# wubinzzu/NeuRec

Hardware: AMD Instinct MI355X
Metric: BPR triplets/sec (LightGCN-gowalla) (higher is better)
Workload: dtype f32; 1 GPU; LightGCN on synthetic gowalla-shaped interactions (U=29858, I=40981, E=813886), 3 layers, dim 64, B=1024 per GPU, adj=pre, Adam lr=0.01 reg=1e-3; global_batch=1024, parallelism=single GPU

## Files before the change

include/neurec_hip.h:

```cpp
#ifndef NEUREC_HIP_H
#define NEUREC_HIP_H

#include <stddef.h>
#include <stdint.h>

#ifdef __cplusplus
extern "C" {
#endif

#define NRHIP_OK 0
#define NRHIP_ERR_ARG 1
#define NRHIP_ERR_UNSUPPORTED 2
#define NRHIP_ERR_HIP 3
#define NRHIP_ERR_WORKSPACE 4

#define NRHIP_ABI_VERSION 4
#define NRHIP_MAX_TOPK 128

int nrhip_abi_version(void);
const char* nrhip_last_error(void);
int nrhip_device_info(int* cu_count, int* clock_khz, size_t* hbm_bytes, char* name, int name_len);


int nrhip_eval_workspace_bytes(int rows, int top_k, size_t* bytes);
// ... 143 lines not shown
                           const int32_t* d_users, const int32_t* d_pos, const int32_t* d_neg, int batch,
                           float reg, float* d_G, float* d_work, float* d_loss2, const uint64_t* d_plan,
                           void* stream);
int nrhip_adam_dense_tf(float* d_var, float* d_m, float* d_v, float* d_grad, int64_t n,
                        float alpha, float beta1, float beta2, float eps, int clear_grad,
                        void* stream);

int nrhip_adam_dense_tf2(float* d_var, float* d_m, float* d_v, const float* d_grad_a,
                         const float* d_grad_b, int64_t n, float alpha, float beta1, float beta2,
                         float eps, void* stream);
int nrhip_adam_dense_tf_multi(int n_tensors, float* const* d_vars_host, float* const* d_ms_host,
                              float* const* d_vs_host, float* const* d_grads_host,
                              const int64_t* sizes_host, const int32_t* clear_grad_host, float alpha,
                              float beta1, float beta2, float eps, void* stream);
int nrhip_rows_div(const int32_t* d_rows, int n_listed, int d, const float* d_src, float denom,
                   float* d_dst, void* stream);
int nrhip_rows_clear(const int32_t* d_rows, int n_listed, int d, float* d_b0, float* d_b1,
                     float* d_b2, float* d_b3, uint8_t* d_flag, void* stream);

int nrhip_spmm_plan_bytes(int64_t n_rows, int64_t nnz, size_t* bytes);
int nrhip_spmm_plan_create(const int64_t* h_indptr, int64_t n_rows, int item_rows, int item_nnz,
                           int64_t split_row, void* d_plan_buf, size_t plan_bytes, void* stream,
                           void** plan_out);
int nrhip_spmm_plan_destroy(void* plan);
int nrhip_spmm_plan_info(const void* plan, int64_t* n_work_items, int64_t* n_split_rows);
int nrhip_spmm_workspace_bytes(const void* plan, int d, size_t* bytes);
int nrhip_spmm_csr(const void* plan, const int64_t* d_indptr, const int32_t* d_indices,
                   const float* d_vals, const float* d_X, int d, float* d_Y,
                   const float* d_addend, const float* d_sum_in, float* d_sum_out, void* d_ws,
                   size_t ws_bytes, void* stream);

int nrhip_spmm_csr_masked(const void* plan, const int64_t* d_indptr, const int32_t* d_indices,
                          const float* d_vals, const float* d_X, const uint8_t* d_x_row_nonzero,
                          const uint8_t* d_y_row_wanted, int d, float* d_Y, const float* d_addend,
                          const float* d_sum_in, float* d_sum_out, void* d_ws, size_t ws_bytes,
                          void* stream);
int nrhip_spmm_blocked_plan_bytes(int64_t n_rows, int64_t nnz, int d, size_t* bytes);
int nrhip_spmm_blocked_plan_create(const int64_t* h_indptr, const int32_t* h_indices,
                                   int64_t n_rows, int64_t split_row, int d, int64_t block_bytes,
                                   int n_workgroups, int waves_per_wg, int seg_len, int r_max,
                                   int p_max, void* d_plan_buf, size_t plan_bytes, void* stream,
                                   void** plan_out);
int nrhip_spmm_blocked_plan_destroy(void* plan);
int nrhip_spmm_blocked_plan_info(const void* plan, int* n_workgroups, int* n_phases,
                                 int64_t* n_entries, int64_t* n_split);
int nrhip_spmm_blocked_tune(int gathers_in_flight);
int nrhip_spmm_blocked_pack(void* plan, const int32_t* d_indices, const float* d_vals, void* stream);
int nrhip_spmm_blocked(const void* plan, const int32_t* d_indices, const float* d_vals,
                       const float* d_X, float* d_Y, const float* d_addend, const float* d_sum_in,
                       float* d_sum_out, const uint8_t* d_x_row_nonzero,
                       const uint8_t* d_y_row_wanted, void* stream);
int nrhip_spmm_plan_attach_blocked(void* plan, const void* blocked_plan, int d);

int nrhip_spmm_csr_adam(const void* plan, const int32_t* d_indices, const float* d_vals,
                        const float* d_X, int d, float* d_addend, float* d_grad_b, float* d_var,
                        float* d_m, float* d_v, float alpha, float beta1, float beta2, float eps,
                        int clear_consumed, uint8_t* d_row_flag, void* stream);
int nrhip_spmm_blocked_adam(const void* plan, const int32_t* d_indices, const float* d_vals,
                            const float* d_X, float* d_addend, float* d_grad_b, float* d_var,
                            float* d_m, float* d_v, float alpha, float beta1, float beta2,
                            float eps, int clear_consumed, uint8_t* d_row_flag, void* stream);
int nrhip_spmm_plan_has_blocked(const void* plan, int d);

int nrhip_spmm_csr_wanted_layers(const void* plan, const int32_t* d_indices, const float* d_vals,
                                 const float* d_X, int d, const float* d_sum_in,
                                 const float* d_layer_a, const float* d_layer_b, float* d_sum_out,
                                 const uint8_t* d_y_row_wanted, void* stream);
int nrhip_spmm_blocked_wanted_layers(const void* plan, const int32_t* d_indices, const float* d_vals,
                                     const float* d_X, const float* d_sum_in, const float* d_layer_a,
                                     const float* d_layer_b, float* d_sum_out,
                                     const uint8_t* d_y_row_wanted, void* stream);
int nrhip_spmm_csr_wanted_batch(const void* plan, const int32_t* d_indices, const float* d_vals,
                                const float* d_X, int d, const float* d_sum_in, const float* d_layer_a,
                                const float* d_layer_b, float* d_sum_out, const int32_t* d_users,
                                const int32_t* d_pos, const int32_t* d_neg, int batch, int n_users,
                                uint8_t* d_row_flag, int32_t* d_rows_out, void* stream);
int nrhip_spmm_blocked_wanted_batch(const void* plan, const int32_t* d_indices, const float* d_vals,
                                    const float* d_X, const float* d_sum_in, const float* d_layer_a,
                                    const float* d_layer_b, float* d_sum_out, const int32_t* d_users,
                                    const int32_t* d_pos, const int32_t* d_neg, int batch, int n_users,
                                    uint8_t* d_row_flag, int32_t* d_rows_out, void* stream);
int nrhip_spmm_plan_has_wanted(const void* plan, int d);
int nrhip_spmm_blocked_has_wanted(const void* blocked_plan);

int nrhip_spmm_csr_carry(const void* plan, const int64_t* d_indptr, const int32_t* d_indices, const float* d_vals,
                         const float* d_X, const float* d_X2, int x_split, int d, float* d_Yv, int has_carry,
                         const uint8_t* d_row_mask, void* stream);
int nrhip_spmm_chunks_finish(const int32_t* d_first_vrow, int64_t n_rows, const float* d_Yv, int d, float* d_Y,
                             const float* d_addend, const float* d_sum_in, float* d_sum_out,
                             const uint8_t* d_row_mask, void* stream);

int nrhip_partials_sum_rows(const float* d_parts, int world, int64_t n_rows, int d, float* d_Y, const float* d_addend,
                            const float* d_sum_in, float* d_sum_out, const uint8_t* d_row_mask, void* stream);

int nrhip_spmm_csr_rows(const int64_t* d_indptr, const int32_t* d_indices, const float* d_vals,
                        const float* d_X, int d, const int32_t* d_rows, int n_listed, float* d_Y,
                        const float* d_addend, const float* d_sum_in, float* d_sum_out,
                        void* stream);

int nrhip_lightgcn_bpr_grad(const float* d_Esum, const float* d_E0, int n_users, int d,
                            int n_layers, const int32_t* d_users, const int32_t* d_pos,
                            const int32_t* d_neg, int batch, float reg, float* d_Gstar,
                            float* d_Greg, float* d_work, float* d_loss2, const uint64_t* d_plan,
                            void* stream);

int nrhip_lightgcn_bpr_grad_h(const float* d_Esum, const float* d_E0, int n_users, int d,
                              int n_layers, const int32_t* d_users, const int32_t* d_pos,
                              const int32_t* d_neg, int batch, float reg, float* d_H,
                              float* d_Greg, float* d_work, float* d_loss2, const uint64_t* d_plan,
                              void* stream);

int nrhip_lightgcn_mark_batch(const int32_t* d_users, const int32_t* d_pos, const int32_t* d_neg,
                              int batch, int n_users, int32_t* d_rows_out, uint8_t* d_row_flag,
                              void* stream);

typedef struct nrhip_lightgcn_buffers {
  const void* plan;
  const void* plan_t;
  const int64_t* indptr;  const int32_t* indices;  const float* vals;
  const int64_t* indptr_t; const int32_t* indices_t; const float* vals_t;
  float* E0; float* m; float* v;
  float* Ea; float* Eb; float* Esum; float* Esum_rows;
  float* Gstar; float* Greg; float* H; float* Ga; float* Gb;
  int32_t* batch_rows;
  uint8_t* row_flag;
  float* terms;
  void* spmm_ws; size_t spmm_ws_bytes;
  int n_users; int n_nodes; int d; int n_layers; int max_batch;
  float reg;
} nrhip_lightgcn_buffers;
int nrhip_lightgcn_ctx_create(const nrhip_lightgcn_buffers* bufs, void** ctx_out);
int nrhip_lightgcn_ctx_destroy(void* ctx);
int nrhip_lightgcn_step(void* ctx, const int32_t* d_users, const int32_t* d_pos,
                        const int32_t* d_neg, int batch, const uint64_t* d_plan, float alpha,
                        float beta1, float beta2, float eps, float* d_loss2, void* stream);

int nrhip_lightgcn_step_colshard_fwd(void* ctx, const int32_t* d_users, const int32_t* d_pos, const int32_t* d_neg,
                                     int batch, float* d_partials, void* stream);
int nrhip_lightgcn_step_colshard_bwd(void* ctx, const int32_t* d_users, const int32_t* d_pos, const int32_t* d_neg,
                                     int batch, const uint64_t* d_plan, const float* d_given, float alpha,
                                     float beta1, float beta2, float eps, float* d_loss2, void* stream);
int nrhip_lightgcn_partial_dots(const float* d_Esum, const float* d_E0, int n_users, int d, int n_layers,
                                const int32_t* d_users, const int32_t* d_pos, const int32_t* d_neg, int batch,
                                float* d_out, void* stream);
int nrhip_partials_sum(const float* d_parts, int world, int n, float* d_given, void* stream);
int nrhip_lightgcn_bpr_grad_given(const float* d_Esum, const float* d_E0, int n_users, int d, int n_layers,
                                  const int32_t* d_users, const int32_t* d_pos, const int32_t* d_neg, int batch,
                                  float reg, float* d_Gstar, float* d_Greg, float* d_work, float* d_loss2,
                                  const uint64_t* d_plan, const float* d_given, int divided, void* stream);
int nrhip_lightgcn_step_grad(void* ctx, const int32_t* d_users, const int32_t* d_pos,
                             const int32_t* d_neg, int batch, const uint64_t* d_plan,
                             float* d_loss2, float* d_grad_out, void* stream);
int nrhip_lightgcn_step_apply(void* ctx, float* d_grad, float alpha, float beta1, float beta2,
                              float eps, void* stream);

typedef struct nrhip_mf_buffers {
  float* P; float* Q; float* mP; float* vP; float* mQ; float* vQ; float* GP; float* GQ;
  float* terms;
  int n_users; int n_items; int d; int max_batch;
  float reg;
  int32_t* last; int32_t* stamp; const float* alpha_tab; int alpha_len; int lazy_period;
  int32_t* tw; int32_t* inb;
} nrhip_mf_buffers;
int nrhip_mf_ctx_create(const nrhip_mf_buffers* bufs, void** ctx_out);
int nrhip_mf_ctx_destroy(void* ctx);
int nrhip_mf_step(void* ctx, const int32_t* d_users, const int32_t* d_pos, const int32_t* d_neg,
                  int batch, const uint64_t* d_plan, const uint64_t* d_next_plan, int next_batch,
                  int step_index, float alpha, float beta1, float beta2, float eps, float* d_loss2,
                  void* stream);
int nrhip_mf_steps(void* ctx, const int32_t* d_users, const int32_t* d_pos, const int32_t* d_neg,
                   int64_t n_total, int batch, const uint64_t* d_plans, int first_step_index,
                   const float* h_alpha, float beta1, float beta2, float eps, float* d_loss2,
                   float* d_terms_steps, void* stream);
int nrhip_loss_reduce_steps(const float* d_terms, int n_steps, int batch, int n_last, float reg, float* d_loss2,
                            void* stream);
int nrhip_mf_flush(void* ctx, int steps_done, float beta1, float beta2, float eps, void* stream);

int nrhip_ngcf_workspace_bytes(int64_t n_rows, size_t* bytes);
int nrhip_ngcf_layer_fwd(const float* d_ego, const float* d_S, const float* d_Wg,
                         const float* d_bg, const float* d_Wb, const float* d_bb, int64_t n_rows,
                         int d, float keep, uint8_t* d_mask, int mask_given, uint64_t seed,
                         uint64_t step, int layer, float* d_ego_out, float* d_out, int64_t ldo,
                         void* stream);
int nrhip_ngcf_layer_bwd(const float* d_ego, const float* d_S, const float* d_Wg,
                         const float* d_bg, const float* d_Wb, const float* d_bb, int64_t n_rows,
                         int d, float keep, const uint8_t* d_mask, const float* d_dout, int64_t ldo,
                         const float* d_dego_next, float* d_dS, float* d_dego_direct, float* d_dT1,
                         float* d_dT2, float* d_dWg, float* d_dbg, float* d_dWb, float* d_dbb,
                         void* d_ws, size_t ws_bytes, void* stream);

int nrhip_vae_encode(const int64_t* d_indptr, const int32_t* d_indices, const int32_t* d_rows,
                     int batch, int h, int z, const float* d_Wq0, const float* d_bq0,
                     const float* d_Wq1, const float* d_bq1, const float* d_Wp0,
                     const float* d_bp0, int act, float keep, const float* d_drop_given,
                     const float* d_eps_given, float is_training, uint64_t seed, uint64_t step,
                     float* d_h0val, float* d_H1, float* d_MU, float* d_LOGVAR, float* d_EPSSTD,
                     float* d_ZS, float* d_G1, float* d_KLb, void* stream);
int nrhip_add_row_bias(float* d_S, int64_t ld, int batch, int cols, const float* d_bias,
                       void* stream);
int nrhip_vae_workspace_bytes(int batch, int cols, size_t* bytes);
int nrhip_vae_decoder_loss_grad(float* d_S, int64_t ld, int batch, int cols, int h,
                                const float* d_bp1, const int64_t* d_indptr,
                                const int32_t* d_indices, const int32_t* d_rows,
                                const float* d_G1, const float* d_Wp1, float* d_nll,
                                float* d_dWp1, float* d_dbp1, float* d_dG1, void* d_ws,
                                size_t ws_bytes, void* stream);
int nrhip_vae_decoder_fused_workspace_bytes(int batch, int cols, size_t* bytes);
int nrhip_vae_decoder_fused(int batch, int cols, int h, const float* d_G1, const float* d_Wp1,
                            const float* d_bp1, const int64_t* d_indptr, const int32_t* d_indices,
                            const int32_t* d_rows, float* d_nll, float* d_dWp1, float* d_dbp1,
                            float* d_dG1, void* d_ws, size_t ws_bytes, float* d_dbg_logits, void* stream);
int nrhip_vae_mid_backward(int batch, int h, int z, int act, float anneal, const float* d_dG1,
                           const float* d_G1, const float* d_H1, const float* d_MU,
                           const float* d_LOGVAR, const float* d_EPSSTD, const float* d_ZS,
                           const float* d_Wp0, const float* d_Wq1, float* d_DA3, float* d_DH2,
                           float* d_DA1, float* d_dWp0, float* d_dbp0, float* d_dWq1,
                           float* d_dbq1, float* d_dbq0, void* stream);
int nrhip_vae_dwq0(const int64_t* d_indptr, const int32_t* d_indices, const int32_t* d_rows,
                   int batch, int h, const float* d_h0val, const float* d_DA1, float* d_dWq0,
                   void* stream);
int nrhip_axpy(float a, const float* d_x, float* d_y, int64_t n, void* stream);
// ... 200 lines not shown
```

neurec_amd/_lib.py:

```python
import ctypes as C
import os

from . import build as _build

_HERE = os.path.dirname(os.path.abspath(__file__))
LIB_PATH = os.path.join(_HERE, "libneurec_hip.so")

ERR_ARG, ERR_UNSUPPORTED, ERR_HIP, ERR_WORKSPACE = 1, 2, 3, 4


class NeuRecHipError(RuntimeError):
    """A HIP runtime failure or workspace error reported by the native library."""


def _load():
    if not os.path.isfile(LIB_PATH):
        raise ImportError(
            "libneurec_hip.so is not built (expected at %s). Run `python -m neurec_amd.build` "
            "(needs hipcc; the engine has no CPU fallback)." % LIB_PATH)
    if os.path.isfile(_build.STAMP) and not _build.is_current() and not os.environ.get("NEUREC_ALLOW_STALE_LIB"):
        raise ImportError(
            "libneurec_hip.so was built from other sources than neurec_amd/csrc now holds (digest in %s differs). "
            "Run `python -m neurec_amd.build`; NEUREC_ALLOW_STALE_LIB=1 loads it anyway." % _build.STAMP)
    try:
# ... 90 lines not shown
                ("M", C.c_void_p), ("mld", C.c_int64), ("eps", C.c_void_p), ("out", C.c_void_p), ("flags", C.c_void_p),
                ("sums", C.c_void_p), ("colsum_ws", C.c_void_p), ("colsum_ws_bytes", C.c_size_t)]


class EvalRedoArgs(C.Structure):
    _fields_ = [("ev", C.POINTER(EvalPrunedArgs)), ("n_flagged", C.c_int), ("reload_items", C.c_int),
                ("scores", C.c_void_p), ("lds", C.c_int64), ("slab_rows", C.c_int), ("rows", C.c_void_p),
                ("row_users", C.c_void_p), ("count", C.c_void_p), ("fixed", C.c_void_p), ("ws", C.c_void_p),
                ("ws_bytes", C.c_size_t)]


SIGNATURES = {
    "nrhip_device_info": [C.POINTER(i32), C.POINTER(i32), psz, C.c_char_p, i32],
    "nrhip_eval_workspace_bytes": [i32, i32, psz],
    "nrhip_mask_train": [p, i64, p, i32, i32, p, p, p],
    "nrhip_eval_scores": [p, i64, i32, i32, p, p, p, C.POINTER(i32), i32, i32, p, p, p, p, sz, p],
    "nrhip_eval_any_k_workspace_bytes": [i32, i32, i32, psz],
    "nrhip_eval_scores_any_k": [p, i64, i32, i32, p, p, p, C.POINTER(i32), i32, i32, p, p, p, sz, p],
    "nrhip_arg_topk": [p, i64, i32, i32, i32, p, p, p, sz, p],
    "nrhip_colsum_workspace_bytes": [i32, i32, psz],
    "nrhip_colsum_f64": [p, i64, i32, i32, p, p, sz, p],
    "nrhip_score_gemm_workspace_bytes": [i32, i32, i32, psz],
    "nrhip_score_gemm_prepare_items": [p, i64, i32, i32, p, sz, p],
    "nrhip_score_tilemax": [p, i64, p, i32, i32, i32, p, p, p, i64, p, sz, p],
    "nrhip_tile_strike_plan": [p, p, i32, i32, p, p, p, p, p, p, p, sz, p],
    "nrhip_score_tilemax_fix": [p, i64, i32, i32, p, p, i32, p, p, p, p, i32, i32, p, i64, p, sz, p],
    "nrhip_score_filter_workspace_bytes": [i32, i32, i32, psz],
    "nrhip_score_filter_kappa": [i32, p],
    "nrhip_score_filter_prepare_items": [p, i64, i32, i32, p, sz, i32, p],
    "nrhip_score_filter_tilemax": [p, i64, p, i32, i32, i32, p, i64, p, p, sz, i32, p],
    "nrhip_score_filter_i8_workspace_bytes": [i32, i32, i32, psz],
    "nrhip_score_filter_i8_prepare_items": [p, i64, i32, i32, p, sz, i32, p],
    "nrhip_score_filter_i8_tilemax": [p, i64, p, i32, i32, i32, p, i64, p, p, sz, i32, p],
    "nrhip_eval_tiles_workspace_bytes": [i32, i32, psz],
    "nrhip_eval_tiles": [p, i64, p, i64, p, i32, p, i32, i32, p, p, p, p, p, i32, i32, p, p, p, sz, p],
    "nrhip_eval_tiles_bounded_workspace_bytes": [i32, i32, i32, i32, psz],
    "nrhip_eval_tiles_bounded": [p, i64, p, i32, p, i64, p, i32, p, i32, i32, p, p, p, p, p, i32, i32, p, p, p, sz, p],
    "nrhip_eval_pruned": [C.POINTER(EvalPrunedArgs), p],
    "nrhip_eval_redo": [C.POINTER(EvalRedoArgs), p],
    "nrhip_vae_step": [C.POINTER(VaeStepArgs), p, i32, f32, f32, f32, u64, i32, i32, p],
    "nrhip_score_gemm_items_kmajor": [p, i32, i32, p, p],
    "nrhip_score_gemm": [p, i64, p, i32, i32, i32, p, i64, p, sz, p],
    "nrhip_sample_bpr_epoch": [p, p, p, i64, i32, i32, u64, u64, i32, i64, i64, p, p, p, p],
    "nrhip_sample_instances_epoch": [p, p, p, p, p, p, p, i64, i32, i32, i32, i32, u64, u64, i32, i64, i64, p, p, p, p, p, p],
    "nrhip_randint_choice_batch": [i32, i32, i64, p, p, p, i32, u64, u64, p, p],
    "nrhip_bpr_plan": [p, p, p, i64, i32, i32, p, p],
    "nrhip_bpr_mf_grad": [p, p, i32, i32, p, p, p, i32, f32, p, p, p, p, p, p],
    "nrhip_adam_sparse_tf": [p, p, p, p, i64, f32, f32, f32, f32, p],
    "nrhip_adam_dense_tf": [p, p, p, p, i64, f32, f32, f32, f32, i32, p],
    "nrhip_adam_dense_tf2": [p, p, p, p, p, i64, f32, f32, f32, f32, p],
    "nrhip_adam_dense_tf_multi": [i32, p, p, p, p, p, p, f32, f32, f32, f32, p],
    "nrhip_rows_div": [p, i32, i32, p, f32, p, p],
    "nrhip_rows_clear": [p, i32, i32, p, p, p, p, p, p],
    "nrhip_spmm_plan_bytes": [i64, i64, psz],
    "nrhip_spmm_plan_create": [p, i64, i32, i32, i64, p, sz, p, C.POINTER(p)],
    "nrhip_spmm_plan_destroy": [p],
    "nrhip_spmm_plan_info": [p, C.POINTER(i64), C.POINTER(i64)],
    "nrhip_spmm_workspace_bytes": [p, i32, psz],
    "nrhip_spmm_csr": [p, p, p, p, p, i32, p, p, p, p, p, sz, p],
    "nrhip_spmm_csr_masked": [p, p, p, p, p, p, p, i32, p, p, p, p, p, sz, p],
    "nrhip_spmm_csr_carry": [p, p, p, p, p, p, i32, i32, p, i32, p, p],
    "nrhip_spmm_chunks_finish": [p, i64, p, i32, p, p, p, p, p, p],
    "nrhip_partials_sum_rows": [p, i32, i64, i32, p, p, p, p, p, p],
    "nrhip_spmm_csr_rows": [p, p, p, p, i32, p, i32, p, p, p, p, p],
    "nrhip_lightgcn_mark_batch": [p, p, p, i32, i32, p, p, p],
    "nrhip_lightgcn_bpr_grad": [p, p, i32, i32, i32, p, p, p, i32, f32, p, p, p, p, p, p],
    "nrhip_lightgcn_bpr_grad_h": [p, p, i32, i32, i32, p, p, p, i32, f32, p, p, p, p, p, p],
    "nrhip_lightgcn_ctx_create": [C.POINTER(LightGCNBuffers), C.POINTER(p)],
    "nrhip_lightgcn_ctx_destroy": [p],
    "nrhip_lightgcn_step": [p, p, p, p, i32, p, f32, f32, f32, f32, p, p],
    "nrhip_lightgcn_step_grad": [p, p, p, p, i32, p, p, p, p],
    "nrhip_lightgcn_step_apply": [p, p, f32, f32, f32, f32, p],
    "nrhip_mf_ctx_create": [C.POINTER(MFBuffers), C.POINTER(p)],
    "nrhip_mf_ctx_destroy": [p],
    "nrhip_mf_step": [p, p, p, p, i32, p, p, i32, i32, f32, f32, f32, f32, p, p],
    "nrhip_mf_flush": [p, i32, f32, f32, f32, p],
    "nrhip_ngcf_ctx_create": [C.POINTER(NGCFBuffers), C.POINTER(p)],
    "nrhip_ngcf_ctx_destroy": [p],
    "nrhip_ngcf_forward": [p, C.c_uint64, C.c_uint64, i32, p],
    "nrhip_ngcf_step": [p, p, p, p, i32, p, C.c_uint64, C.c_uint64, i32, f32, f32, f32, f32, p, p],
    "nrhip_mf_steps": [p, p, p, p, i64, i32, p, i32, p, f32, f32, f32, p, p, p],
    "nrhip_loss_reduce_steps": [p, i32, i32, i32, f32, p, p],
    "nrhip_lightgcn_step_colshard_fwd": [p, p, p, p, i32, p, p],
    "nrhip_lightgcn_step_colshard_bwd": [p, p, p, p, i32, p, p, f32, f32, f32, f32, p, p],
    "nrhip_lightgcn_partial_dots": [p, p, i32, i32, i32, p, p, p, i32, p, p],
    "nrhip_partials_sum": [p, i32, i32, p, p],
    "nrhip_lightgcn_bpr_grad_given": [p, p, i32, i32, i32, p, p, p, i32, f32, p, p, p, p, p, p, i32, p],
    "nrhip_gemm_workspace_bytes": [i32, i32, i32, p],
    "nrhip_gemm_kmajor": [p, i64, p, i64, i32, i32, i32, p, i64, i32, p, i32, i32, p, sz, p],
    "nrhip_gemm_f32": [p, i64, i32, p, i64, i32, i32, i32, i32, p, i64, i32, p, i32, i32, p, sz, p],
    "nrhip_transpose2d": [p, i64, i32, i32, p, i64, p],
    "nrhip_ngcf_wide_forward": [C.POINTER(NGCFWideBuffers), i32, u64, u64, p],
    "nrhip_ngcf_wide_step": [C.POINTER(NGCFWideBuffers), p, p, p, i32, p, i32, u64, u64, f32, f32, f32, f32, p, p],
    "nrhip_vae_bag_fwd": [p, p, p, i32, i32, p, p, i32, f32, p, u64, u64, p, p, p],
    "nrhip_act_bwd": [p, p, i64, i32, p, p],
    "nrhip_vae_sample": [p, i32, i32, p, f32, u64, u64, p, p, p, p],
    "nrhip_vae_sample_bwd": [p, p, p, i32, i32, f32, p, p],
    "nrhip_vae_softmax_dlogits": [p, i64, i32, i32, p, p, p, p, p],
    "nrhip_vae_dwq0_wide": [p, p, p, i32, i32, p, p, p, p],
    "nrhip_colsum_rows": [p, i64, i32, i32, p, p, sz, p],
    "nrhip_ew_mul": [p, i64, p, i64, i64, i32, p, i64, p],
    "nrhip_ngcf_act_fwd": [p, p, i64, i64, i32, i32, f32, p, i32, u64, u64, i32, p, i64, p, i64, p],
    "nrhip_ngcf_act_bwd": [p, i64, p, i64, p, i64, p, p, i64, p, i64, i32, f32, p, p, p],
    "nrhip_lrelu_drop_fwd": [p, i64, i64, i32, i32, f32, p, i32, u64, u64, i32, i32, p, i64, p, i64, p],
    "nrhip_lrelu_drop_bwd": [p, i64, p, i64, p, i64, p, i64, i32, f32, i32, p, p],
    "nrhip_edge_dropout": [p, i64, f32, p, i32, u64, u64, p, p],
    "nrhip_gather_f32": [p, p, i64, p, p],
    "nrhip_ngcf_mix_bwd": [p, p, i64, p, p, i64, i64, i32, i32, p, p, p],
    "nrhip_route_batch": [p, p, p, i32, i32, i32, i32, i32, p, p, p, p, p, i32, p],
    "nrhip_route_owner_keys": [p, p, i32, p, p, i32, i32, i32, p, p, p],
    "nrhip_sort_u64_segments": [p, p, p, i32, i32, p],
    "nrhip_route_epoch": [p, p, p, i64, i32, i32, i32, i32, i32, i32, p, p, p, p, p, p, p, p],
    "nrhip_route_epoch_owner_keys": [p, p, p, i64, p, p, i32, i32, p, p, p, i32, i32, i64, p, p, p],
    "nrhip_bpr_mf_step_fused": [p, p, p, p, p, p, i32, f32, f32, f32, i32, i32, i32, p, p, p, i32, f32, p, p, p,
                                i32, p, i32, i32, p],
    "nrhip_bpr_mf_fused_flush": [p, p, p, p, p, i32, f32, f32, f32, i32, i64, p],
    "nrhip_adam_sparse_tf_lazy": [p, p, p, p, p, p, i64, i32, p, i32, p, i32, p, i32, i32, f32, f32, f32, p],
    "nrhip_bpr_mf_grad_lazy": [p, p, p, p, p, p, i32, f32, f32, f32, i32, i32, p, p, p, i32, f32, p, p, p,
                               p, p],
    "nrhip_ngcf_workspace_bytes": [i64, psz],
    "nrhip_ngcf_layer_fwd": [p, p, p, p, p, p, i64, i32, f32, p, i32, u64, u64, i32, p, p, i64, p],
    "nrhip_ngcf_layer_bwd": [p, p, p, p, p, p, i64, i32, f32, p, p, i64, p, p, p, p, p, p, p, p, p,
                             p, sz, p],
    "nrhip_spmm_blocked_plan_bytes": [i64, i64, i32, psz],
    "nrhip_spmm_blocked_pack": [p, p, p, p],
    "nrhip_spmm_blocked_plan_create": [p, p, i64, i64, i32, i64, i32, i32, i32, i32, i32, p, sz, p,
                                       C.POINTER(p)],
    "nrhip_spmm_blocked_plan_destroy": [p],
    "nrhip_spmm_blocked_plan_info": [p, p, p, p, p],
    "nrhip_spmm_blocked_tune": [i32],
    "nrhip_spmm_blocked": [p, p, p, p, p, p, p, p, p, p, p],
    "nrhip_spmm_plan_attach_blocked": [p, p, i32],
    "nrhip_spmm_plan_has_blocked": [p, i32],
    "nrhip_spmm_plan_has_wanted": [p, i32],
    "nrhip_spmm_blocked_has_wanted": [p],
    "nrhip_spmm_csr_wanted_layers": [p, p, p, p, i32, p, p, p, p, p, p],
    "nrhip_spmm_blocked_wanted_layers": [p, p, p, p, p, p, p, p, p, p],
    "nrhip_spmm_csr_wanted_batch": [p, p, p, p, i32, p, p, p, p, p, p, p, i32, i32, p, p, p],
    "nrhip_spmm_blocked_wanted_batch": [p, p, p, p, p, p, p, p, p, p, p, i32, i32, p, p, p],
    "nrhip_spmm_csr_adam": [p, p, p, p, i32, p, p, p, p, p, f32, f32, f32, f32, i32, p, p],
    "nrhip_spmm_blocked_adam": [p, p, p, p, p, p, p, p, p, f32, f32, f32, f32, i32, p, p],
    "nrhip_vae_encode": [p, p, p, i32, i32, i32, p, p, p, p, p, p, i32, f32, p, p, f32, u64, u64,
                         p, p, p, p, p, p, p, p, p],
    "nrhip_add_row_bias": [p, i64, i32, i32, p, p],
    "nrhip_vae_workspace_bytes": [i32, i32, psz],
    "nrhip_vae_decoder_loss_grad": [p, i64, i32, i32, i32, p, p, p, p, p, p, p, p, p, p, p, sz, p],
    "nrhip_vae_decoder_fused_workspace_bytes": [i32, i32, psz],
    "nrhip_vae_decoder_fused": [i32, i32, i32, p, p, p, p, p, p, p, p, p, p, p, sz, p, p],
    "nrhip_vae_mid_backward": [i32, i32, i32, i32, f32, p, p, p, p, p, p, p, p, p, p, p, p, p, p,
                               p, p, p, p],
    "nrhip_vae_dwq0": [p, p, p, i32, i32, p, p, p, p],
    "nrhip_axpy": [f32, p, p, i64, p],
    "nrhip_sumsq_accumulate": [p, i64, p, p],
    "nrhip_mean_f32": [p, i32, p, p],
    "nrhip_mean2_f32": [p, p, i32, p, p],
    "nrhip_pairwise_mf_grad": [p, p, i32, i32, p, p, p, i32, f32, i32, p, p, p, p, p, p],
    "nrhip_pointwise_mf_grad": [p, p, i32, i32, p, p, p, i32, f32, i32, p, p, p, p, p, p],
    "nrhip_gather_u8": [p, p, i64, p, p],
    "nrhip_mark_rows": [p, i32, i32, p, p],
    "nrhip_sort_u64": [p, i32, p],
    "nrhip_rows_sum_sorted": [p, i32, p, i32, p, i64, p, p],
    "nrhip_rows_sum_sorted2": [p, i32, p, i32, p, i64, p, p, i64, p, p],
    "nrhip_optimizer_rows_tf": [i32, p, p, p, p, p, i64, i32, f32, f32, f32, f32, p],
    "nrhip_optimizer_dense_tf": [i32, p, p, p, p, i64, f32, f32, f32, f32, i32, p],
    "nrhip_rows_gather": [p, i32, i32, p, p, i64, p],
    "nrhip_rows_gather_ld": [p, i32, i32, p, i64, p, i64, p],
    "nrhip_rows_gather2": [p, i32, i32, p, i64, p, i64, p, i64, p, i64, p],
    "nrhip_rows_scatter_add": [p, i32, i32, p, i64, p, p],
    "nrhip_scale": [p, f32, p, i64, p],
    "nrhip_add": [p, p, p, i64, p],
    "nrhip_div_scalar": [p, f32, p, i64, p],
    "nrhip_add2d": [p, i64, p, i64, p, i64, i64, i32, p],
    "nrhip_copy2d": [p, i64, p, i64, i64, i32, p],
    "nrhip_wrmf_chunk_plan": [p, i32, p, p, C.POINTER(i32)],
    "nrhip_wrmf_workspace_bytes": [i32, i32, psz],
    "nrhip_wrmf_gram": [p, i32, i32, p, p, sz, p],
    "nrhip_wrmf_solve": [p, p, i32, p, i32, p, i32, f32, f32, p, p, i32, p, p, sz, p],
}

for _name, _args in SIGNATURES.items():
    _fn = getattr(lib, _name)
    _fn.argtypes = _args
    _fn.restype = C.c_int
lib.nrhip_abi_version.argtypes = []
lib.nrhip_abi_version.restype = C.c_int
lib.nrhip_last_error.argtypes = []
lib.nrhip_last_error.restype = C.c_char_p

EXPORTED = sorted(list(SIGNATURES) + ["nrhip_abi_version", "nrhip_last_error"])

ABI_VERSION = 4
if lib.nrhip_abi_version() != ABI_VERSION:
    raise ImportError("libneurec_hip.so ABI version %d, expected %d"
                      % (lib.nrhip_abi_version(), ABI_VERSION))


def last_error():
    return lib.nrhip_last_error().decode("utf-8", "replace")


def check(rc):
    if rc == 0:
        return
    msg = last_error()
    if rc == ERR_ARG:
        raise ValueError(msg)
    if rc == ERR_UNSUPPORTED:
        raise NotImplementedError(msg)
    raise NeuRecHipError("libneurec_hip status %d: %s" % (rc, msg))


def call(name, *args):
    check(getattr(lib, name)(*args))


def is_stale():
    return not _build.is_current()
```

neurec_amd/build.py:

```python
import hashlib
import os
import subprocess
import sys
from concurrent.futures import ThreadPoolExecutor

HERE = os.path.dirname(os.path.abspath(__file__))
ROOT = os.path.dirname(HERE)
CSRC = os.path.join(HERE, "csrc")
OBJ_DIR = os.path.join(CSRC, "_obj")
LIB_PATH = os.path.join(HERE, "libneurec_hip.so")
STAMP = os.path.join(OBJ_DIR, "sources.sha256")

SOURCES = ["eval_select.hip", "score_gemm.hip", "sampler.hip", "spmm.hip", "bpr.hip", "adam.hip",
           "step.hip", "dense.hip", "vae.hip", "spmm_blocked.hip", "route.hip", "gemm.hip", "vae_wide.hip", "ngcf_wide.hip", "vae_fused.hip",
           "score_bf16.hip", "score_i8.hip", "eval_pipeline.hip", "wrmf.hip"]
FILE_FLAGS = {"score_i8.hip": ["-mllvm", "-amdgpu-mfma-vgpr-form"]}
EXP_SOURCES = ["experiments/gather_experiments.hip"]
EXP_LIB_PATH = os.path.join(HERE, "libneurec_exp.so")
HEADERS = ["nr_core.h", "nr_common.h", "spmm_blocked_plan.h"]

HIPCC = os.environ.get("HIPCC", "/opt/rocm/bin/hipcc")
FLAGS = ["-O3", "--offload-arch=gfx950", "-std=c++17", "-fPIC", "-ffp-contract=off",
         "-munsafe-fp-atomics", "-Wall", "-Wno-unused-function",
         "-I", CSRC, "-I", os.path.join(ROOT, "include")] + os.environ.get("NEUREC_HIPCC_EXTRA", "").split()


def _existing_sources():
    return [s for s in SOURCES if os.path.isfile(os.path.join(CSRC, s))]


def _digest():
    h = hashlib.sha256()
    for name in _existing_sources() + HEADERS:
        with open(os.path.join(CSRC, name), "rb") as f:
            h.update(name.encode())
            h.update(f.read())
    with open(os.path.join(ROOT, "include", "neurec_hip.h"), "rb") as f:
        h.update(f.read())
    h.update(" ".join(f.replace(ROOT, "<root>") for f in FLAGS).encode())
    h.update(repr(sorted(FILE_FLAGS.items())).encode())
    return h.hexdigest()


def is_current():
    if not (os.path.isfile(LIB_PATH) and os.path.isfile(STAMP)):
        return False
    with open(STAMP) as f:
        return f.read().strip() == _digest()


def build_extension(force=False, verbose=True):
    if not force and is_current():
        return LIB_PATH
    os.makedirs(OBJ_DIR, exist_ok=True)
    srcs = _existing_sources()

    def compile_one(src):
        obj = os.path.join(OBJ_DIR, src.replace(".hip", ".o"))
        cmd = [HIPCC] + FLAGS + FILE_FLAGS.get(src, []) + ["-c", os.path.join(CSRC, src), "-o", obj]
        r = subprocess.run(cmd, capture_output=True, text=True)
        if r.returncode != 0 and FILE_FLAGS.get(src):
            r2 = subprocess.run([HIPCC] + FLAGS + ["-c", os.path.join(CSRC, src), "-o", obj], capture_output=True, text=True)
            if r2.returncode == 0:
                sys.stderr.write("neurec_amd.build: %s compiled WITHOUT %s (not accepted by this hipcc)\n"
                                 % (src, " ".join(FILE_FLAGS[src])))
                r = r2
        return src, obj, r

    objs = []
    with ThreadPoolExecutor(max_workers=min(8, len(srcs))) as ex:
        for src, obj, r in ex.map(compile_one, srcs):
            if r.returncode != 0:
                raise RuntimeError("hipcc failed on %s:\n%s\n%s" % (src, r.stdout, r.stderr))
            if verbose and r.stderr.strip():
                sys.stderr.write(r.stderr)
            objs.append(obj)
    cmd = [HIPCC, "--offload-arch=gfx950", "-shared", "-fPIC", "-o", LIB_PATH] + objs
    r = subprocess.run(cmd, capture_output=True, text=True)
    if r.returncode != 0:
        raise RuntimeError("link failed:\n%s\n%s" % (r.stdout, r.stderr))
    with open(STAMP, "w") as f:
        f.write(_digest())
    if verbose:
        print("built", LIB_PATH)
    return LIB_PATH


def build_experiments(verbose=True):
    os.makedirs(OBJ_DIR, exist_ok=True)
    objs = []
    for src in EXP_SOURCES:
        obj = os.path.join(OBJ_DIR, os.path.basename(src).replace(".hip", ".o"))
        r = subprocess.run([HIPCC] + FLAGS + ["-c", os.path.join(CSRC, src), "-o", obj],
                           capture_output=True, text=True)
        if r.returncode != 0:
            raise RuntimeError("hipcc failed on %s:\n%s\n%s" % (src, r.stdout, r.stderr))
        objs.append(obj)
    r = subprocess.run([HIPCC, "--offload-arch=gfx950", "-shared", "-fPIC", "-o", EXP_LIB_PATH] + objs +
                       ["-L", HERE, "-lneurec_hip", "-Wl,-rpath,$ORIGIN"], capture_output=True, text=True)
    if r.returncode != 0:
        raise RuntimeError("link failed:\n%s\n%s" % (r.stdout, r.stderr))
    if verbose:
# ... 9 lines not shown
```

neurec_amd/colshard.py:

```python
import numpy as np
import torch

from . import engine as E
from .trainer import LightGCNEngine


class ColumnShardedLightGCN:
    def __init__(self, comm, adj_csr, n_users, n_items, embed, n_layers, lr, reg, max_batch, adj_t_csr=None,
                 rank=None, world=None, keep_order=False):
        self.comm = comm
        self.rank = comm.rank if rank is None else int(rank)
        self.world = comm.world if world is None else int(world)
        emb = np.asarray(embed, dtype=np.float32) if not isinstance(embed, torch.Tensor) else embed
        self.d = int(emb.shape[1])
        if self.d % self.world:
            raise ValueError("embed_size %d is not a multiple of the %d ranks" % (self.d, self.world))
        self.d_loc = self.d // self.world
        lo = self.rank * self.d_loc
        self.local = LightGCNEngine(adj_csr, n_users, n_items, emb[:, lo:lo + self.d_loc], n_layers, lr, reg,
                                    max_batch, adj_t_csr=adj_t_csr, keep_order=keep_order)
        dev = self.local.E0.device
        self.max_batch = int(max_batch)
        self._parts = torch.zeros(3 * self.max_batch, dtype=torch.float32, device=dev)
        self._given = torch.zeros(3 * self.max_batch, dtype=torch.float32, device=dev)
        self.exchange_bytes_per_step = None

    @property
    def adam(self):
        return self.local.adam

    def step(self, users, pos, neg, loss_out=None, plan=None):
        B = users.numel()
        if B > self.max_batch:
            raise ValueError("batch larger than max_batch")
        ctx, n = self.local._ctx, 3 * B
        ctx.lightgcn_step_colshard_fwd(users, pos, neg, self._parts)
        if self.comm.live and self.world == self.comm.world:
            allp = torch.empty((self.world, n), dtype=torch.float32, device=self._parts.device)
            self.comm.all_gather_rows(self._parts[:n], allp)
            E.partials_sum(allp, self.world, n, self._given)
            given = self._given
            self.exchange_bytes_per_step = self.world * n * 4
        else:
            given = self._parts
        ctx.lightgcn_step_colshard_bwd(users, pos, neg, self.local.adam, loss_out, plan, given)
        self.local.adam.advance()

    def final_embeddings(self):
        eu, ei = self.local.final_embeddings()
        if not (self.comm.live and self.world == self.comm.world):
            return eu, ei
        loc = torch.cat([eu, ei]).contiguous()
        allc = torch.empty((self.world,) + tuple(loc.shape), dtype=loc.dtype, device=loc.device)
        self.comm.all_gather_rows(loc, allc.view(self.world * loc.shape[0], loc.shape[1]))
        full = allc.permute(1, 0, 2).reshape(loc.shape[0], self.d).contiguous()
        U = self.local.n_users
        return full[:U], full[U:]

    def table(self):
        return self.local.E0[:, :self.d_loc]
```

neurec_amd/csrc/spmm.hip:

```cpp
#include "nr_common.h"
#include <limits.h>
#include <algorithm>
#include <stdlib.h>
#include <new>
#include <vector>

extern "C" int nrhip_spmm_blocked(const void* plan, const int32_t* d_indices, const float* d_vals,
                                  const float* d_X, float* d_Y, const float* d_addend,
                                  const float* d_sum_in, float* d_sum_out,
                                  const uint8_t* d_x_row_nonzero, const uint8_t* d_y_row_wanted,
                                  void* stream);

extern "C" int nrhip_spmm_blocked_wanted_layers(const void* plan, const int32_t* d_indices,
                                                const float* d_vals, const float* d_X,
                                                const float* d_sum_in, const float* d_layer_a,
                                                const float* d_layer_b, float* d_sum_out,
                                                const uint8_t* d_y_row_wanted, void* stream);
extern "C" int nrhip_spmm_blocked_wanted_batch(const void* plan, const int32_t* d_indices,
                                               const float* d_vals, const float* d_X,
                                               const float* d_sum_in, const float* d_layer_a,
                                               const float* d_layer_b, float* d_sum_out,
                                               const int32_t* d_users, const int32_t* d_pos,
                                               const int32_t* d_neg, int batch, int n_users,
                                               uint8_t* d_row_flag, int32_t* d_rows_out, void* stream);
extern "C" int nrhip_spmm_blocked_has_wanted(const void* plan);
extern "C" int nrhip_spmm_blocked_adam(const void* plan, const int32_t* d_indices,
                                       const float* d_vals, const float* d_X, float* d_addend,
                                       float* d_grad_b, float* d_var, float* d_m, float* d_v,
                                       float alpha, float beta1, float beta2, float eps,
                                       int clear_consumed, uint8_t* d_row_flag, void* stream);

namespace {

constexpr int kSegLen = 256;
constexpr int kItemRows = 32;
constexpr int kLegacyWaves = 4;
constexpr int kGather = 16;

struct SpmmPlan {
  int64_t n_rows, nnz;
  const void* blocked[5];
  int64_t n_items, n_hub_items, n_a_items, n_b_items;
  int item_rows, item_nnz;
  int32_t* item_row0;
  int32_t* item_nrows;
  int32_t* item_slot;
  int64_t* item_begin;
  int32_t* item_len;
  int64_t n_seg;
  int32_t* seg_row;
  int64_t* seg_begin;
  int32_t* seg_len;
  int32_t* seg_slot;
  int64_t n_multi_seg, n_multi_row;
  int32_t* multi_row;
  int32_t* multi_first;
  int32_t* multi_nseg;
};

inline int blocked_slot(int d) {
  return d == 16 ? 0 : d == 32 ? 1 : d == 64 ? 2 : d == 128 ? 3 : d == 256 ? 4 : -1;
}

struct PlanSizes {
  size_t max_seg, max_multi, max_item;
};
PlanSizes plan_sizes(int64_t n_rows, int64_t nnz) {
  PlanSizes s;
  s.max_seg = (size_t)(n_rows + nnz / kSegLen + 1);
  s.max_multi = (size_t)(nnz / kSegLen + 1);
  s.max_item = (size_t)(n_rows + nnz / kSegLen + 1);
  return s;
}
size_t plan_bytes_for(int64_t n_rows, int64_t nnz) {
  const PlanSizes s = plan_sizes(n_rows, nnz);
  return nr_align_up(s.max_seg * 4, 256) * 3 + nr_align_up(s.max_seg * 8, 256) +
         nr_align_up(s.max_multi * 4, 256) * 3 + nr_align_up(s.max_item * 4, 256) * 4 +
         nr_align_up(s.max_item * 8, 256);
}

template <int D, int G, bool MASKED>
__device__ __forceinline__ void gather_accumulate(int64_t b, int len, int lane,
                                                  const int32_t* __restrict__ indices,
                                                  const float* __restrict__ vals,
                                                  const float* __restrict__ X,
                                                  const uint8_t* __restrict__ col_mask,
                                                  float (&acc)[D / NR_WAVE]) {
  constexpr int CPL = D / NR_WAVE;
  for (int k0 = 0; k0 < len; k0 += NR_WAVE) {
    const int n = min(NR_WAVE, len - k0);
    int my_idx = 0;
    float my_val = 0.f;
    if (lane < n) {
      my_idx = indices[b + k0 + lane];
      my_val = vals[b + k0 + lane];
    }
    if constexpr (!MASKED) {
      for (int t0 = 0; t0 < n; t0 += G) {
        float a[G];
        float x[G][CPL];
#pragma unroll
        for (int u = 0; u < G; ++u) {
          const int tt = min(t0 + u, n - 1);
          const int col = __builtin_amdgcn_readlane(my_idx, tt);
          a[u] = __builtin_bit_cast(
              float, __builtin_amdgcn_readlane(__builtin_bit_cast(int, my_val), tt));
          const float* xr = X + (int64_t)col * D + lane;
#pragma unroll
// ... 658 lines not shown
  p->item_row0 = carve4(sz.max_item);
  p->item_nrows = carve4(sz.max_item);
  p->item_len = carve4(sz.max_item);
  p->item_slot = carve4(sz.max_item);
  p->item_begin = carve8(sz.max_item);
  hipStream_t st = (hipStream_t)stream;
  hipError_t e = hipSuccess;
  auto up = [&](void* dst, const void* src, size_t n) {
    if (n && e == hipSuccess) e = hipMemcpyAsync(dst, src, n, hipMemcpyHostToDevice, st);
  };
  up(p->seg_row, seg_row.data(), seg_row.size() * 4);
  up(p->seg_begin, seg_begin.data(), seg_begin.size() * 8);
  up(p->seg_len, seg_len.data(), seg_len.size() * 4);
  up(p->seg_slot, seg_slot.data(), seg_slot.size() * 4);
  up(p->multi_row, multi_row.data(), multi_row.size() * 4);
  up(p->multi_first, multi_first.data(), multi_first.size() * 4);
  up(p->multi_nseg, multi_nseg.data(), multi_nseg.size() * 4);
  up(p->item_row0, it_row0.data(), it_row0.size() * 4);
  up(p->item_nrows, it_nrows.data(), it_nrows.size() * 4);
  up(p->item_begin, it_begin.data(), it_begin.size() * 8);
  up(p->item_len, it_len.data(), it_len.size() * 4);
  up(p->item_slot, it_slot.data(), it_slot.size() * 4);
  if (e == hipSuccess) e = hipStreamSynchronize(st);
  if (e != hipSuccess) {
    delete p;
    nrhip_set_error("spmm_plan_create: upload failed: %s", hipGetErrorString(e));
    return NR_ERR_HIP;
  }
  *plan_out = p;
  return NR_OK;
}

int nrhip_spmm_plan_destroy(void* plan) {
  delete (SpmmPlan*)plan;
  return NR_OK;
}

int nrhip_spmm_plan_attach_blocked(void* plan, const void* blocked_plan, int d) {
  NR_REQUIRE(plan && blocked_slot(d) >= 0, NR_ERR_ARG,
             "spmm_plan_attach_blocked: null plan or dim %d not in (16, 32, 64, 128, 256)", d);
  ((SpmmPlan*)plan)->blocked[blocked_slot(d)] = blocked_plan;
  return NR_OK;
}

int nrhip_spmm_csr_adam(const void* plan, const int32_t* d_indices, const float* d_vals,
                        const float* d_X, int d, float* d_addend, float* d_grad_b, float* d_var,
                        float* d_m, float* d_v, float alpha, float beta1, float beta2, float eps,
                        int clear_consumed, uint8_t* d_row_flag, void* stream) {
  NR_REQUIRE(plan, NR_ERR_ARG, "spmm_csr_adam: null plan");
  const SpmmPlan* p = (const SpmmPlan*)plan;
  NR_REQUIRE(d == 64 && p->blocked[blocked_slot(64)], NR_ERR_UNSUPPORTED,
             "spmm_csr_adam: needs the d = 64 lane-group schedule");
  return nrhip_spmm_blocked_adam(p->blocked[blocked_slot(64)], d_indices, d_vals, d_X, d_addend, d_grad_b, d_var,
                                 d_m, d_v, alpha, beta1, beta2, eps, clear_consumed, d_row_flag,
                                 stream);
}

int nrhip_spmm_csr_wanted_layers(const void* plan, const int32_t* d_indices, const float* d_vals,
                                 const float* d_X, int d, const float* d_sum_in,
                                 const float* d_layer_a, const float* d_layer_b, float* d_sum_out,
                                 const uint8_t* d_y_row_wanted, void* stream) {
  NR_REQUIRE(plan, NR_ERR_ARG, "spmm_csr_wanted_layers: null plan");
  const SpmmPlan* p = (const SpmmPlan*)plan;
  NR_REQUIRE(d == 64 && p->blocked[blocked_slot(64)], NR_ERR_UNSUPPORTED,
             "spmm_csr_wanted_layers: needs the d = 64 lane-group schedule");
  return nrhip_spmm_blocked_wanted_layers(p->blocked[blocked_slot(64)], d_indices, d_vals, d_X, d_sum_in,
                                          d_layer_a, d_layer_b, d_sum_out, d_y_row_wanted, stream);
}

int nrhip_spmm_csr_wanted_batch(const void* plan, const int32_t* d_indices, const float* d_vals,
                                const float* d_X, int d, const float* d_sum_in, const float* d_layer_a,
                                const float* d_layer_b, float* d_sum_out, const int32_t* d_users,
                                const int32_t* d_pos, const int32_t* d_neg, int batch, int n_users,
                                uint8_t* d_row_flag, int32_t* d_rows_out, void* stream) {
  NR_REQUIRE(plan, NR_ERR_ARG, "spmm_csr_wanted_batch: null plan");
  const SpmmPlan* p = (const SpmmPlan*)plan;
  NR_REQUIRE(d == 64 && p->blocked[blocked_slot(64)], NR_ERR_UNSUPPORTED,
             "spmm_csr_wanted_batch: needs the d = 64 lane-group schedule");
  return nrhip_spmm_blocked_wanted_batch(p->blocked[blocked_slot(64)], d_indices, d_vals, d_X, d_sum_in,
                                         d_layer_a, d_layer_b, d_sum_out, d_users, d_pos, d_neg, batch,
                                         n_users, d_row_flag, d_rows_out, stream);
}

int nrhip_spmm_plan_has_wanted(const void* plan, int d) {
  if (!plan || d != 64) return 0;
  const SpmmPlan* p = (const SpmmPlan*)plan;
  return p->blocked[blocked_slot(64)] ? nrhip_spmm_blocked_has_wanted(p->blocked[blocked_slot(64)]) : 0;
}

int nrhip_spmm_plan_has_blocked(const void* plan, int d) {
  if (!plan) return 0;
  const SpmmPlan* p = (const SpmmPlan*)plan;
  const int slot = blocked_slot(d);
  return slot >= 0 && p->blocked[slot] != nullptr;
}

int nrhip_spmm_plan_info(const void* plan, int64_t* n_work_items, int64_t* n_split_rows) {
  NR_REQUIRE(plan, NR_ERR_ARG, "spmm_plan_info: null plan");
  const SpmmPlan* p = (const SpmmPlan*)plan;
  if (n_work_items) *n_work_items = p->n_items;
  if (n_split_rows) *n_split_rows = p->n_multi_row;
  return NR_OK;
}

int nrhip_spmm_workspace_bytes(const void* plan, int d, size_t* bytes) {
  NR_REQUIRE(plan && bytes && d >= 1, NR_ERR_ARG, "spmm_workspace_bytes: bad arguments");
  const SpmmPlan* p = (const SpmmPlan*)plan;
  *bytes = nr_align_up((size_t)(p->n_multi_seg + 1) * (size_t)d * sizeof(float), 256);
  return NR_OK;
}

static int spmm_dispatch(const char* who, const void* plan, const int64_t* d_indptr,
                         const int32_t* d_indices, const float* d_vals, const float* d_X, int d,
                         float* d_Y, const float* d_addend, const float* d_sum_in,
                         float* d_sum_out, const uint8_t* d_col_mask, const uint8_t* d_row_mask,
                         void* d_ws, size_t ws_bytes, void* stream) {
  NR_REQUIRE(plan && d_indptr && d_indices && d_vals && d_X && (d_Y || d_sum_out), NR_ERR_ARG,
             "%s: null pointer argument", who);
  NR_REQUIRE((d_sum_out == nullptr) || (d_sum_in != nullptr), NR_ERR_ARG,
             "%s: sum_out needs sum_in", who);
  const SpmmPlan* p = (const SpmmPlan*)plan;
  hipStream_t st = (hipStream_t)stream;
  const int bslot = blocked_slot(d);
  if (bslot >= 0 && p->blocked[bslot])
    return nrhip_spmm_blocked(p->blocked[bslot], d_indices, d_vals, d_X, d_Y, d_addend, d_sum_in,
                              d_sum_out, d_col_mask, d_row_mask, stream);
  if (d < 64)
    NR_REQUIRE(d_row_mask == nullptr, NR_ERR_UNSUPPORTED,
               "%s: row mask needs an embedding dim >= 64", who);
  if (p->n_multi_seg > 0)
    NR_REQUIRE(d_ws && ws_bytes >= (size_t)p->n_multi_seg * d * sizeof(float), NR_ERR_WORKSPACE,
               "%s: workspace too small for %lld split-row partials", who,
               (long long)p->n_multi_seg);
  float* part = (float*)d_ws;
  switch (d) {
    case 16: return launch_segs<16>(p, d_indices, d_vals, d_X, d_Y, d_addend, d_sum_in, d_sum_out, part, st);
    case 32: return launch_segs<32>(p, d_indices, d_vals, d_X, d_Y, d_addend, d_sum_in, d_sum_out, part, st);
    case 64: return launch_items<64, 4>(p, d_indptr, d_indices, d_vals, d_X, d_Y, d_addend, d_sum_in, d_sum_out, part, d_col_mask, d_row_mask, st);
    case 128: return launch_items<128, 2>(p, d_indptr, d_indices, d_vals, d_X, d_Y, d_addend, d_sum_in, d_sum_out, part, d_col_mask, d_row_mask, st);
    case 256: return launch_items<256, 1>(p, d_indptr, d_indices, d_vals, d_X, d_Y, d_addend, d_sum_in, d_sum_out, part, d_col_mask, d_row_mask, st);
    default:
      NR_REQUIRE(false, NR_ERR_UNSUPPORTED,
                 "%s: embedding dim %d not built (16, 32, 64, 128, 256)", who, d);
  }
  return NR_OK;
}

int nrhip_spmm_csr(const void* plan, const int64_t* d_indptr, const int32_t* d_indices,
                   const float* d_vals, const float* d_X, int d, float* d_Y,
                   const float* d_addend, const float* d_sum_in, float* d_sum_out, void* d_ws,
                   size_t ws_bytes, void* stream) {
  return spmm_dispatch("spmm_csr", plan, d_indptr, d_indices, d_vals, d_X, d, d_Y, d_addend,
                       d_sum_in, d_sum_out, nullptr, nullptr, d_ws, ws_bytes, stream);
}

int nrhip_spmm_csr_masked(const void* plan, const int64_t* d_indptr, const int32_t* d_indices,
                          const float* d_vals, const float* d_X, const uint8_t* d_x_row_nonzero,
                          const uint8_t* d_y_row_wanted, int d, float* d_Y, const float* d_addend,
                          const float* d_sum_in, float* d_sum_out, void* d_ws, size_t ws_bytes,
                          void* stream) {
  NR_REQUIRE(d_x_row_nonzero || d_y_row_wanted, NR_ERR_ARG, "spmm_csr_masked: no mask given");
  NR_REQUIRE(!(d_y_row_wanted && d_sum_out && d_sum_out == d_sum_in) || true, NR_ERR_ARG, "");
  return spmm_dispatch("spmm_csr_masked", plan, d_indptr, d_indices, d_vals, d_X, d, d_Y,
                       d_addend, d_sum_in, d_sum_out, d_x_row_nonzero, d_y_row_wanted, d_ws,
                       ws_bytes, stream);
}
// ... 80 lines not shown
```

neurec_amd/csrc/spmm_blocked.hip:

```cpp
#include "nr_common.h"
#include "spmm_blocked_plan.h"
#include <algorithm>
#include <new>
#include <cstdlib>
#include <initializer_list>
#include <vector>

namespace {

using nr_plan::kMaxLdsBytes;
using nr_plan::blocked_plan_bytes;
static_assert((int)nr_plan::kOk == NR_OK && (int)nr_plan::kErrArg == NR_ERR_ARG &&
              (int)nr_plan::kErrUnsupported == NR_ERR_UNSUPPORTED, "the planner returns the C ABI's status codes");

struct BlockedPlan : nr_plan::PlanArrays<int4> {
  int64_t n_rows, nnz, n_ent, n_cmb;
  int n_wg, n_phases;
  int seg, r_max, p_max, waves, d;
  const int32_t* pk_from_idx;
  const float* pk_from_val;
  int nnz_cap, ent_cap;
  int colmask_ok;
  int wanted_ok, w_ent_cap, w_nnz_cap, w_bitmap_words;
  int ww_ok, ww_ent_cap;
  int ww_lds_slots;
};


struct AdamEpilogue {
  float4* var; float4* m; float4* v; const float4* grad_b;
  float alpha, omb1, omb2, eps;
  float4* addend_rw; float4* grad_b_rw; uint8_t* flag_rw;
};


template <bool MASKED, bool ADAM, int LPR>
__device__ __forceinline__ void blocked_epilogue(const float4* s_acc, int r0, int nr, int tid, int nthreads,
                                                 float4* __restrict__ Y, const float4* __restrict__ addend,
                                                 const float4* sum_in, float4* sum_out,
                                                 const uint8_t* __restrict__ row_mask, const AdamEpilogue& ad,
                                                 const int32_t* s_rows = nullptr) {
  for (int i = tid; i < nr * LPR; i += nthreads) {
    const int row = s_rows ? s_rows[i / LPR] : r0 + i / LPR;
    if constexpr (MASKED) {
      if (row_mask && row_mask[row] == 0) continue;
    }
    const int64_t o = (int64_t)row * LPR + (i & (LPR - 1));
    float4 y = s_acc[i];
    bool flagged = true;
    if constexpr (ADAM) {
      if (ad.flag_rw) flagged = ad.flag_rw[row] != 0;
    }
    float4 hv = make_float4(0.f, 0.f, 0.f, 0.f);
    if (addend) {
      if (flagged) hv = addend[o];
      y.x = __fadd_rn(y.x, hv.x); y.y = __fadd_rn(y.y, hv.y);
      y.z = __fadd_rn(y.z, hv.z); y.w = __fadd_rn(y.w, hv.w);
    }
    if constexpr (ADAM) {
      float4 gb = make_float4(0.f, 0.f, 0.f, 0.f);
      if (flagged) gb = ad.grad_b[o];
      if (ad.addend_rw) {
        const float4 zero = make_float4(0.f, 0.f, 0.f, 0.f);
        if (hv.x != 0.f || hv.y != 0.f || hv.z != 0.f || hv.w != 0.f) ad.addend_rw[o] = zero;
        if (gb.x != 0.f || gb.y != 0.f || gb.z != 0.f || gb.w != 0.f) ad.grad_b_rw[o] = zero;
        if ((i & (LPR - 1)) == 0 && ad.flag_rw && flagged) ad.flag_rw[row] = 0;
      }
      float4 w = ad.var[o], mm = ad.m[o], vv = ad.v[o];
      nr::adam_dense_tf(__fadd_rn(y.x, gb.x), w.x, mm.x, vv.x, ad.alpha, ad.omb1, ad.omb2, ad.eps);
      nr::adam_dense_tf(__fadd_rn(y.y, gb.y), w.y, mm.y, vv.y, ad.alpha, ad.omb1, ad.omb2, ad.eps);
      nr::adam_dense_tf(__fadd_rn(y.z, gb.z), w.z, mm.z, vv.z, ad.alpha, ad.omb1, ad.omb2, ad.eps);
      nr::adam_dense_tf(__fadd_rn(y.w, gb.w), w.w, mm.w, vv.w, ad.alpha, ad.omb1, ad.omb2, ad.eps);
      ad.var[o] = w; ad.m[o] = mm; ad.v[o] = vv;
      continue;
    }
    if (Y) Y[o] = y;
    if (sum_out) {
      const float4 si = sum_in[o];
      sum_out[o] = make_float4(__fadd_rn(si.x, y.x), __fadd_rn(si.y, y.y), __fadd_rn(si.z, y.z),
                               __fadd_rn(si.w, y.w));
    }
  }
}

#ifdef NR_BLK_TIMELINE
__device__ unsigned long long g_blk_dbg[4096 * 24];
#define NR_BLK_STAMP(i) do { if (threadIdx.x == 0 && blockIdx.x < 4096) g_blk_dbg[blockIdx.x * 24 + (i)] = wall_clock64(); } while (0)
#define NR_BLK_WSTAMP() do { if ((threadIdx.x & 63) == 0 && blockIdx.x < 4096) g_blk_dbg[blockIdx.x * 24 + 8 + (threadIdx.x >> 6)] = wall_clock64(); } while (0)
extern "C" int nrhip_exp_blk_timeline(unsigned long long* h_out) {
  if (hipDeviceSynchronize() != hipSuccess) return NR_ERR_HIP;
  return hipMemcpyFromSymbol(h_out, HIP_SYMBOL(g_blk_dbg), sizeof(unsigned long long) * 4096 * 24) == hipSuccess ? NR_OK : NR_ERR_HIP;
}
#else
#define NR_BLK_STAMP(i) do {} while (0)
#define NR_BLK_WSTAMP() do {} while (0)
#endif

template <bool MASKED, int kWaves, int kG, int D, bool ADAM = false>
__global__ __launch_bounds__(kWaves* NR_WAVE) void spmm_blocked_kernel(
    const int32_t* __restrict__ wg_row0, const int32_t* __restrict__ wg_nrows,
    const int32_t* __restrict__ wg_ent_off, const int32_t* __restrict__ wg_cmb_off,
    const int4* __restrict__ ent, const int4* __restrict__ cmb, int n_phases,
    const int32_t* __restrict__ indices, const float* __restrict__ vals,
    const float4* __restrict__ X, float4* __restrict__ Y, const float4* __restrict__ addend,
    const float4* sum_in, float4* sum_out, const uint8_t* __restrict__ col_mask,
    const uint8_t* __restrict__ row_mask, int kRMax, AdamEpilogue ad, const int32_t* __restrict__ row_of,
    int kPMax) {
  constexpr int LPR = D / 4;
// ... 437 lines not shown
    for (int i = tid; i < 3 * bl.batch; i += 16 * NR_WAVE) {
      const int which = i / bl.batch, b = i - which * bl.batch;
      const int row = which == 0 ? bl.users[b] : bl.n_users + (which == 1 ? bl.pos[b] : bl.neg[b]);
      atomicOr(&s_bits[row >> 5], 1u << (row & 31));
      if (i % (int)gridDim.x == wg) {
        bl.row_flag[row] = 1;
        if (bl.rows_out) bl.rows_out[i] = row;
      }
    }
  }
  __syncthreads();
  auto is_wanted = [&](int row) -> bool {
    return by_batch ? ((s_bits[row >> 5] >> (row & 31)) & 1u) != 0u : row_mask[row] != 0;
  };
  for (int i = tid; i < ne; i += 16 * NR_WAVE) {
    const int4 e = w_ent[e0 + i];
    if (is_wanted(e.w)) {
      const int off = atomicAdd(&s_cursor, e.y);
      if (off + e.y <= nnz_cap) s_now[atomicAdd(&s_n_now, 1)] = make_int4(e.x, e.y | (off << 8), e.z, e.w);
      else s_later[atomicAdd(&s_n_later, 1)] = e;
    }
  }
  __syncthreads();
  while (true) {
    const int n_now = s_n_now, n_later = s_n_later;
    for (int k = wave; k < n_now; k += 16) {
      const int4 e = s_now[k];
      const int len = e.y & 0xFF, off = e.y >> 8;
      if (lane < len)
        s_iv[off + lane] = make_int2(indices[(uint32_t)e.z + lane], __float_as_int(vals[(uint32_t)e.z + lane]));
    }
    __syncthreads();
    for (int k = tid; k < n_now; k += 16 * NR_WAVE) {
      const int4 e = s_now[k];
      s_now[k] = make_int4(e.x, e.y & 0xFF, e.y >> 8, e.w | (1 << 30));
    }
    __syncthreads();
    staged_walk(s_now, s_iv, n_now, 0, X, Y, addend, sum_in, sum_out, s_part, kRMax, wave, g, c, chain);
    if (n_later == 0) break;
    __syncthreads();
    if (tid == 0) { s_n_now = 0; s_n_later = 0; s_cursor = 0; }
    __syncthreads();
    for (int k0 = 0; k0 < n_later; k0 += 16 * NR_WAVE) {
      const int k = k0 + tid;
      int4 e = make_int4(0, 0, 0, 0);
      if (k < n_later) e = s_later[k];
      __syncthreads();
      if (k < n_later) {
        const int off = atomicAdd(&s_cursor, e.y);
        if (off + e.y <= nnz_cap) s_now[atomicAdd(&s_n_now, 1)] = make_int4(e.x, e.y | (off << 8), e.z, e.w);
        else s_later[atomicAdd(&s_n_later, 1)] = e;
      }
      __syncthreads();
    }
  }
  if (c1 > c0) {
    __syncthreads();
    for (int ci = c0 + wave * 4 + g; ci < c1; ci += 64) {
      const int4 cm = w_cmb[ci];
      if (!is_wanted(cm.x)) continue;
      float4 acc = make_float4(0.f, 0.f, 0.f, 0.f);
      for (int sgm = 0; sgm < cm.z; ++sgm) {
        const float4 q = s_part[(size_t)(cm.y - kRMax + sgm) * RS + c];
        acc.x = __fadd_rn(acc.x, q.x); acc.y = __fadd_rn(acc.y, q.y);
        acc.z = __fadd_rn(acc.z, q.z); acc.w = __fadd_rn(acc.w, q.w);
      }
      masked_row_out(acc, (int64_t)cm.x * RS + c, addend, true, Y, sum_in, sum_out, &chain);
    }
  }
}

struct WantedEpi {
  float4* Y; const float4* addend; const float4* sum_in; float4* sum_out; LayerChain chain;
};
#ifdef NR_WW_TIMELINE
__device__ unsigned long long g_ww_dbg[256 * 8];
#define NR_WW_STAMP(i) do { if (threadIdx.x == 0 && blockIdx.x < 256) g_ww_dbg[blockIdx.x * 8 + (i)] = wall_clock64(); } while (0)
#define NR_WW_STAMP_END(i) do { __syncthreads(); NR_WW_STAMP(i); } while (0)
#else
#define NR_WW_STAMP(i)
#define NR_WW_STAMP_END(i)
#endif

__global__ __launch_bounds__(16 * NR_WAVE) void spmm_wanted_wave_kernel(
    const int32_t* __restrict__ ww_off, const int32_t* __restrict__ ww_choff,
    const int4* __restrict__ ww_ent, const int32_t* __restrict__ ww_gch, const int4* __restrict__ ww_hub,
    const int32_t* __restrict__ ww_lcoff, const int4* __restrict__ ww_lcmb,
    float* ww_part, unsigned* ww_cnt, const int32_t* __restrict__ indices,
    const float* __restrict__ vals, const float4* __restrict__ X, WantedEpi ep,
    const uint8_t* __restrict__ row_mask, BatchLists bl, int bitmap_words, int ent_cap, int lds_slots) {
  constexpr int RS = 16;
  extern __shared__ float4 s_mem[];
  float4* s_part = s_mem;
  int4* s_want = (int4*)(s_mem + (size_t)lds_slots * RS);
  uint32_t* s_bits = (uint32_t*)(s_want + ent_cap);
  __shared__ int s_n;
  const int tid = threadIdx.x, lane = tid & 63, wave = tid >> 6;
  const int c = lane & 15, g = lane >> 4;
  const int wg = blockIdx.x;
  const int e0 = ww_off[wg], ne = ww_off[wg + 1] - e0;
  const int h0 = ww_choff[wg], h1 = ww_choff[wg + 1];
  const int l0 = ww_lcoff[wg], l1 = ww_lcoff[wg + 1];
  NR_WW_STAMP(0);
  if (tid == 0) s_n = 0;
  const bool by_batch = bl.users != nullptr;
  if (by_batch) {
    for (int i = tid; i < bitmap_words; i += 16 * NR_WAVE) s_bits[i] = 0u;
    __syncthreads();
    for (int i = tid; i < bl.batch; i += 16 * NR_WAVE) {
      const int u = bl.users[i], p = bl.pos[i], q = bl.neg[i];
      const int ru = u, rp = bl.n_users + p, rq = bl.n_users + q;
      if (u >= 0) atomicOr(&s_bits[ru >> 5], 1u << (ru & 31));
      if (p >= 0) atomicOr(&s_bits[rp >> 5], 1u << (rp & 31));
      if (q >= 0) atomicOr(&s_bits[rq >> 5], 1u << (rq & 31));
    }
    const int total = 3 * bl.batch, per = (total + (int)gridDim.x - 1) / (int)gridDim.x;
    for (int i = wg * per + tid; i < min(total, (wg + 1) * per); i += 16 * NR_WAVE) {
      const int which = i / bl.batch, b = i - which * bl.batch;
      const int row = which == 0 ? bl.users[b] : bl.n_users + (which == 1 ? bl.pos[b] : bl.neg[b]);
      bl.row_flag[row] = 1;
      if (bl.rows_out) bl.rows_out[i] = row;
    }
  }
  __syncthreads();
  auto is_wanted = [&](int row) -> bool {
    return by_batch ? ((s_bits[row >> 5] >> (row & 31)) & 1u) != 0u : row_mask[row] != 0;
  };
  NR_WW_STAMP(1);
  for (int i = tid; i < ne; i += 16 * NR_WAVE) {
    const int4 e = ww_ent[e0 + i];
    if (is_wanted(e.w)) s_want[atomicAdd(&s_n, 1)] = e;
  }
  __syncthreads();
  NR_WW_STAMP(2);
  const int n = s_n;
  const float4 zero = make_float4(0.f, 0.f, 0.f, 0.f);
  int k = wave;
  int4 e = zero_int4();
  int col = 0;
  float val = 0.f;
  if (k < n) {
    e = s_want[k];
    if (lane < e.y) {
      col = indices[(uint32_t)e.z + lane];
      val = vals[(uint32_t)e.z + lane];
    }
  }
  while (k < n) {
    const int len = e.y, slot = e.x, row = e.w;
    float4 x[16];
#pragma unroll
    for (int j = 0; j < 16; ++j) {
      const int cj = __shfl(col, (g << 4) | j, NR_WAVE);
      x[j] = X[(int64_t)cj * RS + c];
    }
    const int64_t o = (int64_t)row * RS + c;
    const int64_t oe = slot == 0 ? o : (int64_t)c;
    float4 pre_si = zero, pre_a = zero, pre_b = zero;
    if (ep.sum_out) {
      pre_si = ep.sum_in[oe];
      if (ep.chain.a) pre_a = ep.chain.a[oe];
      if (ep.chain.b) pre_b = ep.chain.b[oe];
    }
    const int kn = k + 16;
    int4 en = zero_int4();
    int coln = 0;
    float valn = 0.f;
    if (kn < n) {
      en = s_want[kn];
      if (lane < en.y) {
        coln = indices[(uint32_t)en.z + lane];
        valn = vals[(uint32_t)en.z + lane];
      }
    }
#pragma unroll
    for (int j = 0; j < 16; ++j) {
      const float aj = __shfl(val, (g << 4) | j, NR_WAVE);
      x[j] = make_float4(__fmul_rn(aj, x[j].x), __fmul_rn(aj, x[j].y), __fmul_rn(aj, x[j].z), __fmul_rn(aj, x[j].w));
    }
    float4 acc = zero, carry = zero;
#pragma unroll
    for (int gg = 0; gg < 4; ++gg) {
      if (gg * 16 < len) {
        if (g == gg) {
          acc = carry;
#pragma unroll
          for (int j = 0; j < 16; ++j) {
            const float4 t = make_float4(__fadd_rn(acc.x, x[j].x), __fadd_rn(acc.y, x[j].y),
                                         __fadd_rn(acc.z, x[j].z), __fadd_rn(acc.w, x[j].w));
            if (gg * 16 + j < len) acc = t;
          }
        }
        const int src = (gg << 4) | c;
        carry = make_float4(__shfl(acc.x, src, NR_WAVE), __shfl(acc.y, src, NR_WAVE),
                            __shfl(acc.z, src, NR_WAVE), __shfl(acc.w, src, NR_WAVE));
      }
    }
    if (g == 0) {
      if (slot == 0) {
        float4 y = carry;
        if (ep.addend) {
          const float4 pre_add = ep.addend[o];
          y = make_float4(__fadd_rn(y.x, pre_add.x), __fadd_rn(y.y, pre_add.y), __fadd_rn(y.z, pre_add.z),
                          __fadd_rn(y.w, pre_add.w));
        }
        if (ep.Y) ep.Y[o] = y;
        if (ep.sum_out) {
          float4 si = pre_si;
          if (ep.chain.a)
            si = make_float4(__fadd_rn(si.x, pre_a.x), __fadd_rn(si.y, pre_a.y), __fadd_rn(si.z, pre_a.z),
                             __fadd_rn(si.w, pre_a.w));
          if (ep.chain.b)
            si = make_float4(__fadd_rn(si.x, pre_b.x), __fadd_rn(si.y, pre_b.y), __fadd_rn(si.z, pre_b.z),
                             __fadd_rn(si.w, pre_b.w));
          ep.sum_out[o] = make_float4(__fadd_rn(si.x, y.x), __fadd_rn(si.y, y.y), __fadd_rn(si.z, y.z),
                                      __fadd_rn(si.w, y.w));
        }
      } else if (slot < 0) {
        s_part[(size_t)(-slot - 1) * RS + c] = carry;
      } else {
        float* mine = ww_part + (size_t)(slot - 1) * 64 + c * 4;
        __hip_atomic_store(mine + 0, carry.x, __ATOMIC_RELAXED, __HIP_MEMORY_SCOPE_AGENT);
        __hip_atomic_store(mine + 1, carry.y, __ATOMIC_RELAXED, __HIP_MEMORY_SCOPE_AGENT);
        __hip_atomic_store(mine + 2, carry.z, __ATOMIC_RELAXED, __HIP_MEMORY_SCOPE_AGENT);
        __hip_atomic_store(mine + 3, carry.w, __ATOMIC_RELAXED, __HIP_MEMORY_SCOPE_AGENT);
      }
    }
    k = kn;
    e = en;
    col = coln;
    val = valn;
  }
  if (l1 > l0) {
    __syncthreads();
    for (int li = l0 + wave * 4 + g; li < l1; li += 64) {
      const int4 cm = ww_lcmb[li];
      if (!is_wanted(cm.x)) continue;
      float4 acc = zero;
      for (int sgm = 0; sgm < cm.z; ++sgm) {
        const float4 q = s_part[(size_t)(cm.y + sgm) * RS + c];
        acc.x = __fadd_rn(acc.x, q.x); acc.y = __fadd_rn(acc.y, q.y);
        acc.z = __fadd_rn(acc.z, q.z); acc.w = __fadd_rn(acc.w, q.w);
      }
      masked_row_out(acc, (int64_t)cm.x * RS + c, ep.addend, true, ep.Y, ep.sum_in, ep.sum_out, &ep.chain);
    }
  }
  NR_WW_STAMP_END(3);
  if (tid == 0 && blockIdx.x < 256) {
#ifdef NR_WW_TIMELINE
    g_ww_dbg[blockIdx.x * 8 + 6] = (unsigned long long)n;
    g_ww_dbg[blockIdx.x * 8 + 7] = (unsigned long long)(h1 - h0);
#endif
  }
  if (h1 > h0) {
    __builtin_amdgcn_fence(__ATOMIC_RELEASE, "workgroup");
    __builtin_amdgcn_s_waitcnt(0);
    __syncthreads();
    for (int hi = h0 + wave; hi < h1; hi += 16) {
      const int hub = ww_gch[hi];
      const int4 hd = ww_hub[hub];
      if (!is_wanted(hd.x)) continue;
      unsigned old = 0;
      if (lane == 0) old = __hip_atomic_fetch_add(&ww_cnt[hub], 1u, __ATOMIC_RELAXED, __HIP_MEMORY_SCOPE_AGENT);
      old = __builtin_amdgcn_readfirstlane(old);
      if (old != (unsigned)hd.w - 1u) continue;
      float4 sum = zero;
      for (int s0 = 0; s0 < hd.z; s0 += 16) {
        float4 q[16];
#pragma unroll
        for (int j = 0; j < 16; ++j) {
          const float* qp = ww_part + ((size_t)hd.y + min(s0 + j, hd.z - 1)) * 64 + c * 4;
          q[j].x = __hip_atomic_load(qp + 0, __ATOMIC_RELAXED, __HIP_MEMORY_SCOPE_AGENT);
          q[j].y = __hip_atomic_load(qp + 1, __ATOMIC_RELAXED, __HIP_MEMORY_SCOPE_AGENT);
          q[j].z = __hip_atomic_load(qp + 2, __ATOMIC_RELAXED, __HIP_MEMORY_SCOPE_AGENT);
          q[j].w = __hip_atomic_load(qp + 3, __ATOMIC_RELAXED, __HIP_MEMORY_SCOPE_AGENT);
        }
#pragma unroll
        for (int j = 0; j < 16; ++j)
          if (s0 + j < hd.z)
            sum = make_float4(__fadd_rn(sum.x, q[j].x), __fadd_rn(sum.y, q[j].y), __fadd_rn(sum.z, q[j].z),
                              __fadd_rn(sum.w, q[j].w));
      }
      if (g == 0)
        masked_row_out(sum, (int64_t)hd.x * RS + c, ep.addend, true, ep.Y, ep.sum_in, ep.sum_out, &ep.chain);
      if (lane == 0) __hip_atomic_store(&ww_cnt[hub], 0u, __ATOMIC_RELAXED, __HIP_MEMORY_SCOPE_AGENT);
    }
  }
  NR_WW_STAMP_END(4);
}

size_t wanted_lds_bytes(const BlockedPlan* p) {
  return (size_t)p->p_max * 256 + 2 * (size_t)p->w_ent_cap * 16 + (size_t)p->w_bitmap_words * 4 +
         (size_t)p->w_nnz_cap * 8;
}
int ww_bitmap_words(const BlockedPlan* p) { return (int)((p->n_rows + 127) / 128 * 4); }
size_t ww_lds_bytes(const BlockedPlan* p) {
  return (size_t)p->ww_lds_slots * 256 + (size_t)p->ww_ent_cap * 16 + (size_t)ww_bitmap_words(p) * 4 + 16;
}
size_t colmask_lds_bytes(const BlockedPlan* p) {
  return (size_t)p->p_max * 256 + (size_t)p->ent_cap * 16 + (size_t)p->nnz_cap * 8;
}

int launch_wanted_wave(const BlockedPlan* p, const int32_t* d_indices, const float* d_vals, const float* d_X,
                       float* d_Y, const float* d_addend, const float* d_sum_in, float* d_sum_out,
                       const uint8_t* d_y_row_wanted, LayerChain chain, BatchLists bl, hipStream_t st) {
  hipLaunchKernelGGL(spmm_wanted_wave_kernel, dim3((unsigned)p->n_wg), dim3(16 * NR_WAVE), ww_lds_bytes(p), st,
                     p->ww_off, p->ww_choff, p->ww_ent, p->ww_gch, p->ww_hub, p->ww_lcoff, p->ww_lcmb, p->ww_part,
                     p->ww_cnt, d_indices, d_vals, (const float4*)d_X,
                     WantedEpi{(float4*)d_Y, (const float4*)d_addend, (const float4*)d_sum_in,
                               (float4*)d_sum_out, chain},
                     d_y_row_wanted, bl, ww_bitmap_words(p), p->ww_ent_cap, p->ww_lds_slots);
  NR_LAUNCH_CHECK();
  return NR_OK;
}

int s_gathers_in_flight = 8;

__global__ __launch_bounds__(256) void row_order_pack_kernel(const uint32_t* __restrict__ src, const uint32_t* __restrict__ dst,
                                                             int64_t n_rows, const int32_t* __restrict__ indices,
                                                             const float* __restrict__ vals, int32_t* __restrict__ pk_idx,
                                                             float* __restrict__ pk_val) {
  const int c = threadIdx.x & 15;
  for (int64_t k = (int64_t)blockIdx.x * 16 + (threadIdx.x >> 4); k < n_rows; k += (int64_t)gridDim.x * 16) {
    const uint32_t s0 = src[k], d0 = dst[k], len = dst[k + 1] - d0;
    for (uint32_t j = c; j < len; j += 16) {
      pk_idx[d0 + j] = indices[s0 + j];
      pk_val[d0 + j] = vals[s0 + j];
    }
  }
}

static hipError_t allow_plan_lds(const BlockedPlan* p) {
  hipError_t e = hipSuccess;
  auto allow = [&](const void* fn, size_t lds) {
    if (e == hipSuccess) e = hipFuncSetAttribute(fn, hipFuncAttributeMaxDynamicSharedMemorySize, (int)lds);
  };
  const size_t lds = (size_t)(p->r_max + p->p_max) * p->d * 4 + (size_t)p->r_max * 4;
#define NR_ALLOW(DD)                                                                                                         \
  allow((const void*)spmm_blocked_kernel<false, 16, 8, DD>, lds); allow((const void*)spmm_blocked_kernel<true, 16, 8, DD>, lds); \
  allow((const void*)spmm_blocked_kernel<false, 16, 4, DD>, lds); allow((const void*)spmm_blocked_kernel<true, 16, 4, DD>, lds); \
  allow((const void*)spmm_blocked_kernel<false, 8, 8, DD>, lds); allow((const void*)spmm_blocked_kernel<true, 8, 8, DD>, lds);   \
  allow((const void*)spmm_blocked_kernel<false, 8, 4, DD>, lds); allow((const void*)spmm_blocked_kernel<true, 8, 4, DD>, lds)
  if (p->d == 16) { NR_ALLOW(16); } else if (p->d == 32) { NR_ALLOW(32); }
  else if (p->d == 64) {
    NR_ALLOW(64);
    allow((const void*)spmm_blocked_kernel<false, 16, 8, 64, true>, lds);
  }
  else if (p->d == 128) { NR_ALLOW(128); } else { NR_ALLOW(256); }
#undef NR_ALLOW
  if (p->wanted_ok) allow((const void*)spmm_wanted_rows_kernel, wanted_lds_bytes(p));
  if (p->ww_ok) allow((const void*)spmm_wanted_wave_kernel, ww_lds_bytes(p));
  if (p->colmask_ok)
    for (const void* fn : {(const void*)spmm_staged_masked_kernel<true, false>,
                           (const void*)spmm_staged_masked_kernel<false, true>,
                           (const void*)spmm_staged_masked_kernel<true, true>})
      allow(fn, colmask_lds_bytes(p));
  return e;
}

}

extern "C" {

int nrhip_spmm_blocked_plan_bytes(int64_t n_rows, int64_t nnz, int d, size_t* bytes) {
  NR_REQUIRE(bytes && n_rows >= 0 && nnz >= 0, NR_ERR_ARG, "spmm_blocked_plan_bytes: bad arguments");
  (void)d;
  *bytes = blocked_plan_bytes(n_rows, nnz);
  return NR_OK;
}

int nrhip_spmm_blocked_plan_create(const int64_t* h_indptr, const int32_t* h_indices,
                                   int64_t n_rows, int64_t split_row, int d, int64_t block_bytes,
                                   int n_workgroups, int waves_per_wg, int seg_len, int r_max,
                                   int p_max, void* d_plan_buf, size_t plan_bytes, void* stream,
                                   void** plan_out) {
  nr_plan::Options opt;
  nr_plan::Error err;
  int rc = nr_plan::resolve_options(d, waves_per_wg, seg_len, r_max, p_max, block_bytes, split_row, n_rows, &opt, &err);
  NR_REQUIRE(rc == NR_OK, rc, "%s", err.msg.c_str());
  NR_REQUIRE(h_indptr && h_indices && d_plan_buf && plan_out && n_rows > 0, NR_ERR_ARG,
             "spmm_blocked_plan_create: bad arguments");
  const int64_t nnz = h_indptr[n_rows] - h_indptr[0];
  NR_REQUIRE(h_indptr[0] == 0 && nnz < ((int64_t)1 << 32), NR_ERR_UNSUPPORTED,
             "spmm_blocked: indptr must start at 0 and hold < 2^32 non-zeros");
  const size_t need_bytes = blocked_plan_bytes(n_rows, nnz);
  NR_REQUIRE(plan_bytes >= need_bytes, NR_ERR_WORKSPACE,
             "spmm_blocked_plan_create: plan buffer %zu < %zu bytes", plan_bytes, need_bytes);
  int n_wg = n_workgroups;
  if (n_wg <= 0) {
    int dev = 0;
    hipDeviceProp_t prop;
    NR_CHECK_HIP(hipGetDevice(&dev));
    NR_CHECK_HIP(hipGetDeviceProperties(&prop, dev));
    n_wg = prop.multiProcessorCount * (16 / opt.waves);
  }
  rc = nr_plan::choose_workgroup_count(n_wg, n_workgroups <= 0, n_rows, &opt, &err);
  NR_REQUIRE(rc == NR_OK, rc, "%s", err.msg.c_str());
  const char* env = getenv("NEUREC_SPMM_MASKED_FAST");
  opt.masked_fast = !(env && env[0] == '0');
  env = getenv("NEUREC_SPMM_WANTED_WAVE");
  opt.wanted_wave = !(env && env[0] == '0');
  env = getenv("NEUREC_SPMM_WANTED_NNZ_CAP");
  opt.wanted_nnz_cap = env ? std::max(atoi(env), 1) : 0;

  nr_plan::Plan h;
  rc = nr_plan::build_plan(h_indptr, h_indices, n_rows, opt, &h, &err);
  NR_REQUIRE(rc == NR_OK, rc, "%s", err.msg.c_str());

  BlockedPlan* p = new (std::nothrow) BlockedPlan();
  NR_REQUIRE(p, NR_ERR_ARG, "spmm_blocked_plan_create: out of host memory");
  p->n_rows = n_rows; p->nnz = nnz; p->n_wg = h.n_wg; p->n_phases = h.n_phases;
  p->seg = opt.seg; p->r_max = opt.r_max; p->p_max = opt.p_max; p->waves = opt.waves; p->d = d;
  p->n_ent = (int64_t)h.ent.size(); p->n_cmb = (int64_t)h.cmb.size();
  p->nnz_cap = h.nnz_cap; p->ent_cap = h.ent_cap; p->colmask_ok = h.colmask_ok;
  p->wanted_ok = h.wanted_ok; p->w_ent_cap = h.w_ent_cap; p->w_nnz_cap = h.w_nnz_cap; p->w_bitmap_words = h.w_bitmap_words;
  p->ww_ok = h.ww_ok; p->ww_ent_cap = h.ww_ent_cap; p->ww_lds_slots = h.ww_lds_slots;
  std::vector<nr_plan::Section> sections = nr_plan::plan_sections(*p, h);
  const size_t used = nr_plan::carve_sections(&sections, d_plan_buf);
  if (used > plan_bytes) {
    delete p;
    nrhip_set_error("spmm_blocked_plan_create: plan needs %zu bytes, buffer has %zu", used, plan_bytes);
    return NR_ERR_WORKSPACE;
  }
  hipStream_t st = (hipStream_t)stream;
  hipError_t e = hipSuccess;
  for (const nr_plan::Section& s : sections) {
    if (e != hipSuccess) break;
    if (s.src && s.bytes) e = hipMemcpyAsync(s.addr, s.src, s.bytes, hipMemcpyHostToDevice, st);
    else if (s.zero) e = hipMemsetAsync(s.addr, 0, s.bytes + s.pad, st);
  }
  if (e == hipSuccess) e = hipStreamSynchronize(st);
  if (e == hipSuccess) e = allow_plan_lds(p);
  if (e != hipSuccess) {
    delete p;
    nrhip_set_error("spmm_blocked_plan_create: %s", hipGetErrorString(e));
    return NR_ERR_HIP;
  }
  *plan_out = p;
  return NR_OK;
}

int nrhip_spmm_blocked_pack(void* plan, const int32_t* d_indices, const float* d_vals, void* stream) {
  NR_REQUIRE(plan && d_indices && d_vals, NR_ERR_ARG, "spmm_blocked_pack: null pointer argument");
  BlockedPlan* p = (BlockedPlan*)plan;
  if (p->nnz > 0) {
    const unsigned blocks = (unsigned)std::min<int64_t>((p->n_rows + 15) / 16, 8192);
    hipLaunchKernelGGL(row_order_pack_kernel, dim3(blocks), dim3(256), 0, (hipStream_t)stream, p->pk_src, p->pk_dst,
                       p->n_rows, d_indices, d_vals, p->pk_idx, p->pk_val);
    NR_LAUNCH_CHECK();
  }
  p->pk_from_idx = d_indices;
  p->pk_from_val = d_vals;
  return NR_OK;
}

static int ensure_packed(const BlockedPlan* p, const int32_t* d_indices, const float* d_vals, void* stream) {
  if (p->pk_from_idx == d_indices && p->pk_from_val == d_vals) return NR_OK;
  return nrhip_spmm_blocked_pack((void*)p, d_indices, d_vals, stream);
}

#ifdef NR_WW_TIMELINE
int nrhip_ww_timeline(unsigned long long* h_out) {
  NR_CHECK_HIP(hipDeviceSynchronize());
  NR_CHECK_HIP(hipMemcpyFromSymbol(h_out, HIP_SYMBOL(g_ww_dbg), sizeof(unsigned long long) * 256 * 8));
  return NR_OK;
}
#endif

int nrhip_spmm_blocked_tune(int gathers_in_flight) {
  NR_REQUIRE(gathers_in_flight == 4 || gathers_in_flight == 8, NR_ERR_UNSUPPORTED,
             "spmm_blocked_tune: gathers in flight %d (4, 8)", gathers_in_flight);
  s_gathers_in_flight = gathers_in_flight;
  return NR_OK;
}

int nrhip_spmm_blocked_plan_destroy(void* plan) {
  delete (BlockedPlan*)plan;
  return NR_OK;
}

int nrhip_spmm_blocked_plan_info(const void* plan, int* n_workgroups, int* n_phases,
                                 int64_t* n_entries, int64_t* n_split) {
  NR_REQUIRE(plan, NR_ERR_ARG, "spmm_blocked_plan_info: null plan");
  const BlockedPlan* p = (const BlockedPlan*)plan;
  if (n_workgroups) *n_workgroups = p->n_wg;
  if (n_phases) *n_phases = p->n_phases;
  if (n_entries) *n_entries = p->n_ent;
  if (n_split) *n_split = p->n_cmb;
  return NR_OK;
}

int nrhip_spmm_blocked(const void* plan, const int32_t* d_indices, const float* d_vals,
                       const float* d_X, float* d_Y, const float* d_addend, const float* d_sum_in,
                       float* d_sum_out, const uint8_t* d_x_row_nonzero,
                       const uint8_t* d_y_row_wanted, void* stream) {
  NR_REQUIRE(plan && d_indices && d_vals && d_X && (d_Y || d_sum_out), NR_ERR_ARG,
             "spmm_blocked: null pointer argument");
  NR_REQUIRE((d_sum_out == nullptr) || (d_sum_in != nullptr), NR_ERR_ARG,
             "spmm_blocked: sum_out needs sum_in");
// ... 27 lines not shown
    if (d_x_row_nonzero && d_y_row_wanted) NR_STAGED(true, true);
    else if (d_x_row_nonzero) NR_STAGED(true, false);
    else NR_STAGED(false, true);
#undef NR_STAGED
    NR_LAUNCH_CHECK();
    return NR_OK;
  }
#define NR_BLK(M, W, GG, DD)                                                                       \
  hipLaunchKernelGGL((spmm_blocked_kernel<M, W, GG, DD>), grid, block, lds, st, p->wg_row0,        \
                     p->wg_nrows, p->wg_ent_off, p->wg_cmb_off, p->ent, p->cmb, p->n_phases,        \
                     p->pk_idx, p->pk_val, (const float4*)d_X, (float4*)d_Y, (const float4*)d_addend, \
                     (const float4*)d_sum_in, (float4*)d_sum_out, d_x_row_nonzero, d_y_row_wanted,  \
                     p->r_max, AdamEpilogue{}, p->row_of, p->p_max)
#define NR_BLK_D(DD)                                                                               \
  if (p->waves == 16) {                                                                            \
    if (masked) { if (gif == 4) NR_BLK(true, 16, 4, DD); else NR_BLK(true, 16, 8, DD); }           \
    else { if (gif == 4) NR_BLK(false, 16, 4, DD); else NR_BLK(false, 16, 8, DD); }                \
  } else {                                                                                         \
    if (masked) { if (gif == 4) NR_BLK(true, 8, 4, DD); else NR_BLK(true, 8, 8, DD); }             \
    else { if (gif == 4) NR_BLK(false, 8, 4, DD); else NR_BLK(false, 8, 8, DD); }                  \
  }
  if (p->d == 16) { NR_BLK_D(16) } else if (p->d == 32) { NR_BLK_D(32) } else if (p->d == 64) { NR_BLK_D(64) }
  else if (p->d == 128) { NR_BLK_D(128) } else { NR_BLK_D(256) }
#undef NR_BLK_D
#undef NR_BLK
  NR_LAUNCH_CHECK();
  return NR_OK;
}

int nrhip_spmm_blocked_wanted_layers(const void* plan, const int32_t* d_indices, const float* d_vals,
                                     const float* d_X, const float* d_sum_in, const float* d_layer_a,
                                     const float* d_layer_b, float* d_sum_out,
                                     const uint8_t* d_y_row_wanted, void* stream) {
  NR_REQUIRE(plan && d_indices && d_vals && d_X && d_sum_in && d_sum_out && d_y_row_wanted, NR_ERR_ARG,
             "spmm_blocked_wanted_layers: null pointer argument");
  NR_REQUIRE(d_layer_a || !d_layer_b, NR_ERR_ARG, "spmm_blocked_wanted_layers: layer_b without layer_a");
  const BlockedPlan* p = (const BlockedPlan*)plan;
  if (p->ww_ok)
    return launch_wanted_wave(p, d_indices, d_vals, d_X, nullptr, nullptr, d_sum_in, d_sum_out, d_y_row_wanted,
                              LayerChain{(const float4*)d_layer_a, (const float4*)d_layer_b}, BatchLists{},
                              (hipStream_t)stream);
  NR_REQUIRE(p->wanted_ok, NR_ERR_UNSUPPORTED, "spmm_blocked_wanted_layers: no wanted-rows schedule");
  hipLaunchKernelGGL(spmm_wanted_rows_kernel, dim3((unsigned)p->n_wg), dim3(p->waves * NR_WAVE),
                     wanted_lds_bytes(p), (hipStream_t)stream, p->w_ent_off, p->w_cmb_off, p->w_ent,
                     p->w_cmb, d_indices, d_vals, (const float4*)d_X, (float4*)nullptr,
                     (const float4*)nullptr, (const float4*)d_sum_in, (float4*)d_sum_out,
                     d_y_row_wanted, p->r_max, p->p_max, p->w_ent_cap, p->w_nnz_cap,
                     LayerChain{(const float4*)d_layer_a, (const float4*)d_layer_b}, BatchLists{},
                     p->w_bitmap_words);
  NR_LAUNCH_CHECK();
  return NR_OK;
}

int nrhip_spmm_blocked_wanted_batch(const void* plan, const int32_t* d_indices, const float* d_vals,
                                    const float* d_X, const float* d_sum_in, const float* d_layer_a,
                                    const float* d_layer_b, float* d_sum_out, const int32_t* d_users,
                                    const int32_t* d_pos, const int32_t* d_neg, int batch, int n_users,
                                    uint8_t* d_row_flag, int32_t* d_rows_out, void* stream) {
  NR_REQUIRE(plan && d_indices && d_vals && d_X && d_sum_in && d_sum_out && d_users && d_pos && d_neg &&
                 d_row_flag && batch >= 0 && n_users >= 0,
             NR_ERR_ARG, "spmm_blocked_wanted_batch: bad arguments");
  NR_REQUIRE(d_layer_a || !d_layer_b, NR_ERR_ARG, "spmm_blocked_wanted_batch: layer_b without layer_a");
  const BlockedPlan* p = (const BlockedPlan*)plan;
  if (batch == 0) return NR_OK;
  if (p->ww_ok)
    return launch_wanted_wave(p, d_indices, d_vals, d_X, nullptr, nullptr, d_sum_in, d_sum_out, nullptr,
                              LayerChain{(const float4*)d_layer_a, (const float4*)d_layer_b},
                              BatchLists{d_users, d_pos, d_neg, batch, n_users, d_row_flag, d_rows_out},
                              (hipStream_t)stream);
  NR_REQUIRE(p->wanted_ok && p->w_bitmap_words > 0, NR_ERR_UNSUPPORTED,
             "spmm_blocked_wanted_batch: no wanted-rows schedule with a row bit set");
  hipLaunchKernelGGL(spmm_wanted_rows_kernel, dim3((unsigned)p->n_wg), dim3(p->waves * NR_WAVE),
                     wanted_lds_bytes(p), (hipStream_t)stream, p->w_ent_off, p->w_cmb_off, p->w_ent,
                     p->w_cmb, d_indices, d_vals, (const float4*)d_X, (float4*)nullptr,
                     (const float4*)nullptr, (const float4*)d_sum_in, (float4*)d_sum_out,
                     (const uint8_t*)nullptr, p->r_max, p->p_max, p->w_ent_cap, p->w_nnz_cap,
                     LayerChain{(const float4*)d_layer_a, (const float4*)d_layer_b},
                     BatchLists{d_users, d_pos, d_neg, batch, n_users, d_row_flag, d_rows_out},
                     p->w_bitmap_words);
  NR_LAUNCH_CHECK();
  return NR_OK;
}

int nrhip_spmm_blocked_has_wanted(const void* plan) {
  if (plan && ((const BlockedPlan*)plan)->ww_ok) return 2;
  if (!plan || !((const BlockedPlan*)plan)->wanted_ok) return 0;
  return ((const BlockedPlan*)plan)->w_bitmap_words > 0 ? 2 : 1;
}

int nrhip_spmm_blocked_adam(const void* plan, const int32_t* d_indices, const float* d_vals,
                            const float* d_X, float* d_addend, float* d_grad_b, float* d_var,
                            float* d_m, float* d_v, float alpha, float beta1, float beta2,
                            float eps, int clear_consumed, uint8_t* d_row_flag, void* stream) {
  NR_REQUIRE(plan && d_indices && d_vals && d_X && d_grad_b && d_var && d_m && d_v, NR_ERR_ARG,
             "spmm_blocked_adam: null pointer argument");
  const BlockedPlan* p = (const BlockedPlan*)plan;
  NR_REQUIRE(p->d == 64 && p->waves == 16, NR_ERR_UNSUPPORTED,
             "spmm_blocked_adam: built for d = 64 schedules with 16 waves");
  NR_REQUIRE(d_X != d_var, NR_ERR_ARG, "spmm_blocked_adam: the operand must not be the updated table");
  const size_t lds = (size_t)(p->r_max + p->p_max) * p->d * 4 + (size_t)p->r_max * 4;
  NR_TRY(ensure_packed(p, d_indices, d_vals, stream));
  NR_REQUIRE(!clear_consumed || d_addend, NR_ERR_ARG, "spmm_blocked_adam: clear_consumed needs an addend");
  AdamEpilogue ad{(float4*)d_var, (float4*)d_m, (float4*)d_v, (const float4*)d_grad_b,
                  alpha, 1.0f - beta1, 1.0f - beta2, eps,
                  clear_consumed ? (float4*)d_addend : nullptr,
                  clear_consumed ? (float4*)d_grad_b : nullptr, clear_consumed ? d_row_flag : nullptr};
  hipLaunchKernelGGL((spmm_blocked_kernel<false, 16, 8, 64, true>), dim3((unsigned)p->n_wg),
                     dim3(16 * NR_WAVE), lds, (hipStream_t)stream, p->wg_row0, p->wg_nrows,
                     p->wg_ent_off, p->wg_cmb_off, p->ent, p->cmb, p->n_phases, p->pk_idx, p->pk_val,
                     (const float4*)d_X, (float4*)nullptr, (const float4*)d_addend,
                     (const float4*)nullptr, (float4*)nullptr, (const uint8_t*)nullptr,
                     (const uint8_t*)nullptr, p->r_max, ad, p->row_of, p->p_max);
  NR_LAUNCH_CHECK();
  return NR_OK;
}

}
```

neurec_amd/csrc/step.hip:

```cpp
#include "nr_common.h"
#include <algorithm>
#include "neurec_hip.h"
#include <new>

namespace {

struct LightGCNCtx {
  nrhip_lightgcn_buffers b;
};
struct NGCFCtx {
  nrhip_ngcf_buffers b;
};

struct MFCtx {
  nrhip_mf_buffers b;
  bool alpha_tail_const = false;
  const uint64_t* marked_plan = nullptr;
  int marked_step = 0;
};

constexpr int kAlphaTail = 256;

const float* alpha_window(const MFCtx* c, int step_index) {
  const nrhip_mf_buffers& b = c->b;
  if (step_index < b.alpha_len) return b.alpha_tab;
  if (!c->alpha_tail_const || b.lazy_period > 64) return nullptr;
  return b.alpha_tab - (step_index - (b.alpha_len - 1));
}

}

extern "C" int nrhip_spmm_csr_adam(const void* plan, const int32_t* d_indices, const float* d_vals,
                                   const float* d_X, int d, float* d_addend, float* d_grad_b,
                                   float* d_var, float* d_m, float* d_v, float alpha, float beta1,
                                   float beta2, float eps, int clear_consumed,
                                   uint8_t* d_row_flag, void* stream);
extern "C" int nrhip_spmm_plan_has_blocked(const void* plan, int d);
extern "C" int nrhip_spmm_plan_has_wanted(const void* plan, int d);
extern "C" int nrhip_spmm_csr_wanted_batch(const void* plan, const int32_t* d_indices,
                                           const float* d_vals, const float* d_X, int d,
                                           const float* d_sum_in, const float* d_layer_a,
                                           const float* d_layer_b, float* d_sum_out,
                                           const int32_t* d_users, const int32_t* d_pos,
                                           const int32_t* d_neg, int batch, int n_users,
                                           uint8_t* d_row_flag, int32_t* d_rows_out, void* stream);
extern "C" int nrhip_spmm_csr_wanted_layers(const void* plan, const int32_t* d_indices,
                                            const float* d_vals, const float* d_X, int d,
                                            const float* d_sum_in, const float* d_layer_a,
                                            const float* d_layer_b, float* d_sum_out,
                                            const uint8_t* d_y_row_wanted, void* stream);

extern "C" {

int nrhip_lightgcn_ctx_create(const nrhip_lightgcn_buffers* bufs, void** ctx_out) {
  NR_REQUIRE(bufs && ctx_out, NR_ERR_ARG, "lightgcn_ctx_create: null argument");
  const nrhip_lightgcn_buffers& b = *bufs;
  NR_REQUIRE(b.plan && b.plan_t && b.indptr && b.indices && b.vals && b.indptr_t && b.indices_t &&
                 b.vals_t && b.E0 && b.m && b.v && b.Ea && b.Eb && b.Esum && b.Esum_rows &&
                 b.Gstar && b.Greg && b.H && b.Ga && b.Gb && b.batch_rows && b.row_flag && b.terms,
             NR_ERR_ARG, "lightgcn_ctx_create: a buffer pointer is null");
  NR_REQUIRE(b.n_users > 0 && b.n_nodes > b.n_users && b.n_layers >= 0 && b.max_batch > 0,
             NR_ERR_ARG, "lightgcn_ctx_create: bad sizes");
  NR_REQUIRE(b.d == 16 || b.d == 32 || b.d == 64 || b.d == 128 || b.d == 256, NR_ERR_UNSUPPORTED,
             "lightgcn_ctx_create: embedding dim %d not built (16, 32, 64, 128, 256)", b.d);
  LightGCNCtx* c = new (std::nothrow) LightGCNCtx();
  NR_REQUIRE(c, NR_ERR_ARG, "lightgcn_ctx_create: out of host memory");
  c->b = b;
  *ctx_out = c;
  return NR_OK;
}

int nrhip_lightgcn_ctx_destroy(void* ctx) {
  delete (LightGCNCtx*)ctx;
  return NR_OK;
}

struct AdamArgs { float alpha, beta1, beta2, eps; };

static int lightgcn_fwd_bwd(const nrhip_lightgcn_buffers& b, const int32_t* d_users,
                            const int32_t* d_pos, const int32_t* d_neg, int batch,
                            const uint64_t* d_plan, float* d_loss2, void* stream,
                            const float** g_out, const AdamArgs* adam = nullptr,
                            bool* rearmed = nullptr, int phase = 0, float* d_partials = nullptr,
                            const float* d_given = nullptr) {
  const int L = b.n_layers, d = b.d;
  const bool skip = d >= 64;
  const int wanted_form = (skip && L > 0) ? nrhip_spmm_plan_has_wanted(b.plan, d) : 0;
  if (wanted_form != 2 && phase != 2)
    NR_TRY(nrhip_lightgcn_mark_batch(d_users, d_pos, d_neg, batch, b.n_users, b.batch_rows,
                                     b.row_flag, stream));
  const float* esum = b.E0;
  if (L > 0 && phase == 2) esum = b.Esum_rows;
  if (L > 0 && phase != 2) {
    const float* src = b.E0;
    const float* acc_in = b.E0;
    float* ping[2] = {b.Ea, b.Eb};
    const bool chain = wanted_form != 0;
    const float* layer[2] = {nullptr, nullptr};
    for (int k = 0; k < L - 1; ++k) {
      const bool keep_sum = !chain || k < L - 3;
      NR_TRY(nrhip_spmm_csr(b.plan, b.indptr, b.indices, b.vals, src, d, ping[k & 1], nullptr,
                            keep_sum ? acc_in : nullptr, keep_sum ? b.Esum : nullptr, b.spmm_ws,
                            b.spmm_ws_bytes, stream));
      src = ping[k & 1];
      if (keep_sum) acc_in = b.Esum;
      layer[0] = layer[1];
      layer[1] = src;
    }
    if (chain) {
      if (L - 1 == 1) { layer[0] = layer[1]; layer[1] = nullptr; }
      if (wanted_form == 2)
        NR_TRY(nrhip_spmm_csr_wanted_batch(b.plan, b.indices, b.vals, src, d, acc_in, layer[0], layer[1],
                                           b.Esum_rows, d_users, d_pos, d_neg, batch, b.n_users,
                                           b.row_flag, b.batch_rows, stream));
      else
        NR_TRY(nrhip_spmm_csr_wanted_layers(b.plan, b.indices, b.vals, src, d, acc_in, layer[0], layer[1],
                                            b.Esum_rows, b.row_flag, stream));
    } else if (skip)
      NR_TRY(nrhip_spmm_csr_masked(b.plan, b.indptr, b.indices, b.vals, src, nullptr, b.row_flag,
                                   d, nullptr, nullptr, acc_in, b.Esum_rows, b.spmm_ws,
                                   b.spmm_ws_bytes, stream));
    else
      NR_TRY(nrhip_spmm_csr(b.plan, b.indptr, b.indices, b.vals, src, d, nullptr, nullptr, acc_in,
                            b.Esum_rows, b.spmm_ws, b.spmm_ws_bytes, stream));
    esum = b.Esum_rows;
  }
  if (phase == 1)
    return nrhip_lightgcn_partial_dots(esum, b.E0, b.n_users, d, L, d_users, d_pos, d_neg, batch, d_partials,
                                       stream);
  if (((L + 1) & L) == 0) {
    if (d_given)
      NR_TRY(nrhip_lightgcn_bpr_grad_given(esum, b.E0, b.n_users, d, L, d_users, d_pos, d_neg, batch, b.reg, b.H,
                                           b.Greg, b.terms, d_loss2, d_plan, d_given, 1, stream));
    else
      NR_TRY(nrhip_lightgcn_bpr_grad_h(esum, b.E0, b.n_users, d, L, d_users, d_pos, d_neg, batch,
                                       b.reg, b.H, b.Greg, b.terms, d_loss2, d_plan, stream));
  } else {
    if (d_given)
      NR_TRY(nrhip_lightgcn_bpr_grad_given(esum, b.E0, b.n_users, d, L, d_users, d_pos, d_neg, batch, b.reg,
                                           b.Gstar, b.Greg, b.terms, d_loss2, d_plan, d_given, 0, stream));
    else
      NR_TRY(nrhip_lightgcn_bpr_grad(esum, b.E0, b.n_users, d, L, d_users, d_pos, d_neg, batch, b.reg,
                                     b.Gstar, b.Greg, b.terms, d_loss2, d_plan, stream));
    NR_TRY(nrhip_rows_div(b.batch_rows, 3 * batch, d, b.Gstar, (float)(L + 1), b.H, stream));
  }
  const float* g = b.H;
  float* gping[2] = {b.Ga, b.Gb};
  const bool fuse = adam && rearmed && L >= 2 && d == 64 && nrhip_spmm_plan_has_blocked(b.plan_t, d);
  for (int k = 0; k < L; ++k) {
    if (k == L - 1 && fuse) {
      const bool rearm = ((L + 1) & L) == 0;
      NR_TRY(nrhip_spmm_csr_adam(b.plan_t, b.indices_t, b.vals_t, g, d, b.H, b.Greg, b.E0, b.m, b.v,
                                 adam->alpha, adam->beta1, adam->beta2, adam->eps, rearm ? 1 : 0,
                                 b.row_flag, stream));
      *g_out = nullptr;
      if (rearm) *rearmed = true;
      return NR_OK;
    }
    if (k == 0 && skip)
      NR_TRY(nrhip_spmm_csr_masked(b.plan_t, b.indptr_t, b.indices_t, b.vals_t, g, b.row_flag,
                                   nullptr, d, gping[k & 1], b.H, nullptr, nullptr, b.spmm_ws,
                                   b.spmm_ws_bytes, stream));
    else
      NR_TRY(nrhip_spmm_csr(b.plan_t, b.indptr_t, b.indices_t, b.vals_t, g, d, gping[k & 1], b.H,
                            nullptr, nullptr, b.spmm_ws, b.spmm_ws_bytes, stream));
    g = gping[k & 1];
  }
  *g_out = g;
  return NR_OK;
}

static int lightgcn_check(void* ctx, const int32_t* u, const int32_t* p, const int32_t* n,
                          int batch) {
  NR_REQUIRE(ctx && u && p && n, NR_ERR_ARG, "lightgcn_step: null argument");
  const nrhip_lightgcn_buffers& b = ((LightGCNCtx*)ctx)->b;
  NR_REQUIRE(batch >= 0 && batch <= b.max_batch, NR_ERR_ARG,
             "lightgcn_step: batch %d outside 0..%d", batch, b.max_batch);
  return NR_OK;
}

int nrhip_lightgcn_step(void* ctx, const int32_t* d_users, const int32_t* d_pos,
                        const int32_t* d_neg, int batch, const uint64_t* d_plan, float alpha,
                        float beta1, float beta2, float eps, float* d_loss2, void* stream) {
  NR_TRY(lightgcn_check(ctx, d_users, d_pos, d_neg, batch));
  if (batch == 0) return NR_OK;
  const nrhip_lightgcn_buffers& b = ((LightGCNCtx*)ctx)->b;
  const float* g = nullptr;
  const AdamArgs adam{alpha, beta1, beta2, eps};
  bool rearmed = false;
  NR_TRY(lightgcn_fwd_bwd(b, d_users, d_pos, d_neg, batch, d_plan, d_loss2, stream, &g, &adam,
                          &rearmed));
  if (g)
    NR_TRY(nrhip_adam_dense_tf2(b.E0, b.m, b.v, g, b.Greg, (int64_t)b.n_nodes * b.d, alpha, beta1,
                                beta2, eps, stream));
  if (rearmed) return NR_OK;
  NR_TRY(nrhip_rows_clear(b.batch_rows, 3 * batch, b.d, b.Gstar, b.Greg, b.H, nullptr, b.row_flag,
                          stream));
  return NR_OK;
}

int nrhip_lightgcn_step_colshard_fwd(void* ctx, const int32_t* d_users, const int32_t* d_pos, const int32_t* d_neg,
                                     int batch, float* d_partials, void* stream) {
  NR_TRY(lightgcn_check(ctx, d_users, d_pos, d_neg, batch));
  NR_REQUIRE(d_partials, NR_ERR_ARG, "lightgcn_step_colshard_fwd: null output");
  if (batch == 0) return NR_OK;
  const float* g = nullptr;
  return lightgcn_fwd_bwd(((LightGCNCtx*)ctx)->b, d_users, d_pos, d_neg, batch, nullptr, nullptr, stream, &g,
                          nullptr, nullptr, 1, d_partials, nullptr);
}

int nrhip_lightgcn_step_colshard_bwd(void* ctx, const int32_t* d_users, const int32_t* d_pos, const int32_t* d_neg,
                                     int batch, const uint64_t* d_plan, const float* d_given, float alpha,
                                     float beta1, float beta2, float eps, float* d_loss2, void* stream) {
  NR_TRY(lightgcn_check(ctx, d_users, d_pos, d_neg, batch));
  NR_REQUIRE(d_given, NR_ERR_ARG, "lightgcn_step_colshard_bwd: null d_given");
  if (batch == 0) return NR_OK;
  const nrhip_lightgcn_buffers& b = ((LightGCNCtx*)ctx)->b;
  const float* g = nullptr;
  const AdamArgs adam{alpha, beta1, beta2, eps};
  bool rearmed = false;
  NR_TRY(lightgcn_fwd_bwd(b, d_users, d_pos, d_neg, batch, d_plan, d_loss2, stream, &g, &adam, &rearmed, 2, nullptr,
                          d_given));
  if (g)
    NR_TRY(nrhip_adam_dense_tf2(b.E0, b.m, b.v, g, b.Greg, (int64_t)b.n_nodes * b.d, alpha, beta1, beta2, eps,
                                stream));
  if (rearmed) return NR_OK;
  NR_TRY(nrhip_rows_clear(b.batch_rows, 3 * batch, b.d, b.Gstar, b.Greg, b.H, nullptr, b.row_flag, stream));
  return NR_OK;
}

int nrhip_lightgcn_step_grad(void* ctx, const int32_t* d_users, const int32_t* d_pos,
                             const int32_t* d_neg, int batch, const uint64_t* d_plan,
                             float* d_loss2, float* d_grad_out, void* stream) {
  NR_TRY(lightgcn_check(ctx, d_users, d_pos, d_neg, batch));
  NR_REQUIRE(d_grad_out, NR_ERR_ARG, "lightgcn_step_grad: null output");
  const nrhip_lightgcn_buffers& b = ((LightGCNCtx*)ctx)->b;
  const int64_t n = (int64_t)b.n_nodes * b.d;
  if (batch == 0) {
    NR_CHECK_HIP(hipMemsetAsync(d_grad_out, 0, n * sizeof(float), (hipStream_t)stream));
    return NR_OK;
  }
  const float* g = nullptr;
  NR_TRY(lightgcn_fwd_bwd(b, d_users, d_pos, d_neg, batch, d_plan, d_loss2, stream, &g));
  NR_TRY(nrhip_add(g, b.Greg, d_grad_out, n, stream));
  NR_TRY(nrhip_rows_clear(b.batch_rows, 3 * batch, b.d, b.Gstar, b.Greg, b.H, nullptr, b.row_flag,
                          stream));
  return NR_OK;
}

int nrhip_lightgcn_step_apply(void* ctx, float* d_grad, float alpha, float beta1, float beta2,
                              float eps, void* stream) {
  NR_REQUIRE(ctx && d_grad, NR_ERR_ARG, "lightgcn_step_apply: null argument");
  const nrhip_lightgcn_buffers& b = ((LightGCNCtx*)ctx)->b;
  return nrhip_adam_dense_tf(b.E0, b.m, b.v, d_grad, (int64_t)b.n_nodes * b.d, alpha, beta1, beta2,
                             eps, 0, stream);
}

int nrhip_mf_ctx_create(const nrhip_mf_buffers* bufs, void** ctx_out) {
  NR_REQUIRE(bufs && ctx_out, NR_ERR_ARG, "mf_ctx_create: null argument");
  const nrhip_mf_buffers& b = *bufs;
  NR_REQUIRE(b.P && b.Q && b.mP && b.vP && b.mQ && b.vQ && ((b.tw && b.inb) || (!b.tw && b.GP && b.GQ)) && b.terms, NR_ERR_ARG,
             "mf_ctx_create: a buffer pointer is null");
  NR_REQUIRE(b.n_users > 0 && b.n_items > 0 && b.d >= 1 && b.d <= 256 && b.max_batch > 0,
             NR_ERR_ARG, "mf_ctx_create: bad sizes");
  MFCtx* c = new (std::nothrow) MFCtx();
  NR_REQUIRE(c, NR_ERR_ARG, "mf_ctx_create: out of host memory");
  c->b = b;
  if (b.alpha_tab && b.alpha_len > kAlphaTail) {
    float tail[kAlphaTail];
    if (hipMemcpy(tail, b.alpha_tab + (b.alpha_len - kAlphaTail), sizeof(tail), hipMemcpyDeviceToHost) == hipSuccess) {
      c->alpha_tail_const = true;
      for (int k = 0; k < kAlphaTail; ++k) c->alpha_tail_const = c->alpha_tail_const && tail[k] == tail[kAlphaTail - 1];
    }
  }
  *ctx_out = c;
  return NR_OK;
}

int nrhip_mf_ctx_destroy(void* ctx) {
  delete (MFCtx*)ctx;
  return NR_OK;
}

}

static int mf_step_impl(void* ctx, const int32_t* d_users, const int32_t* d_pos, const int32_t* d_neg,
                        int batch, const uint64_t* d_plan, const uint64_t* d_next_plan, int next_batch,
                        int step_index, float alpha, float beta1, float beta2, float eps, float* d_loss2,
                        float* d_terms, void* stream) {
  NR_REQUIRE(ctx && d_users && d_pos && d_neg && d_loss2, NR_ERR_ARG, "mf_step: null argument");
  const nrhip_mf_buffers& b = ((MFCtx*)ctx)->b;
// ... 200 lines not shown
```

neurec_amd/engine.py:

```python
import ctypes as C
import os

import numpy as np
import torch

from . import _lib
from ._lib import call

NGCF_MAX_LAYERS = _lib.NGCF_MAX_LAYERS

METRIC_IDS = {"Precision": 1, "Recall": 2, "MAP": 3, "NDCG": 4, "MRR": 5}


def require_gpu():
    if not torch.cuda.is_available():
        raise RuntimeError("neurec_amd needs a ROCm GPU (MI355X / gfx950); no CPU path exists")
    return torch.device("cuda", torch.cuda.current_device())


def _stream():
    return C.c_void_p(torch.cuda.current_stream().cuda_stream)


def _ptr(t, dtype=None, allow_none=False):
# ... 857 lines not shown
    def matmul(self, X, out=None, addend=None, sum_in=None, sum_out=None, x_row_nonzero=None,
               y_row_wanted=None):
        d = X.shape[1]
        self.ensure_schedule(d)
        ws = self._workspace(d)
        if x_row_nonzero is None and y_row_wanted is None:
            call("nrhip_spmm_csr", self.plan, _ptr(self.indptr), _ptr(self.indices),
                 _ptr(self.vals), _ptr(X, torch.float32), d,
                 _ptr(out, torch.float32, allow_none=True), _ptr(addend, allow_none=True),
                 _ptr(sum_in, allow_none=True), _ptr(sum_out, allow_none=True), _ptr(ws),
                 ws.numel(), _stream())
        else:
            call("nrhip_spmm_csr_masked", self.plan, _ptr(self.indptr), _ptr(self.indices),
                 _ptr(self.vals), _ptr(X, torch.float32),
                 _ptr(x_row_nonzero, torch.uint8, allow_none=True),
                 _ptr(y_row_wanted, torch.uint8, allow_none=True), d,
                 _ptr(out, torch.float32, allow_none=True), _ptr(addend, allow_none=True),
                 _ptr(sum_in, allow_none=True), _ptr(sum_out, allow_none=True), _ptr(ws),
                 ws.numel(), _stream())
        return out

    def matmul_adam(self, X, addend, grad_b, var, m, v, st, row_flag=None):
        d = X.shape[1]
        if d != 64 or not self.ensure_schedule(64):
            return False
        call("nrhip_spmm_csr_adam", self.plan, _ptr(self.indices), _ptr(self.vals), _ptr(X, torch.float32), d,
             _ptr(addend, torch.float32), _ptr(grad_b, torch.float32), _ptr(var, torch.float32), _ptr(m), _ptr(v),
             float(st.alpha()), float(st.beta1), float(st.beta2), float(st.eps), 1 if row_flag is not None else 0,
             _ptr(row_flag, torch.uint8, allow_none=True), _stream())
        return True

    def matmul_rows(self, X, rows, out=None, addend=None, sum_in=None, sum_out=None):
        d = X.shape[1]
        call("nrhip_spmm_csr_rows", _ptr(self.indptr), _ptr(self.indices), _ptr(self.vals),
             _ptr(X, torch.float32), d, _ptr(rows, torch.int32), rows.numel(),
             _ptr(out, torch.float32, allow_none=True), _ptr(addend, allow_none=True),
             _ptr(sum_in, allow_none=True), _ptr(sum_out, allow_none=True), _stream())
        return out

    def algorithmic_bytes(self, d):
        return self.nnz * 8 + (self.n_rows + 1) * 4 + 2 * self.n_rows * d * 4

    def masked_bytes(self, d):
        return self.nnz * 8 + (self.n_rows + 1) * 4 + self.n_rows * d * 4

    def full_pass_kernel(self, d):
        if self.ensure_schedule(d):
            return "spmm_blocked_kernel<false, 16, 8, %d, false>" % d
        return "spmm_item_kernel<%d, ...>" % d


def add2d(x, y, out):
    call("nrhip_add2d", C.c_void_p(x.data_ptr()), x.stride(0), C.c_void_p(y.data_ptr()), y.stride(0),
         C.c_void_p(out.data_ptr()), out.stride(0), x.shape[0], x.shape[1], _stream())


def copy2d(x, out):
    call("nrhip_copy2d", C.c_void_p(x.data_ptr()), x.stride(0), C.c_void_p(out.data_ptr()),
         out.stride(0), x.shape[0], x.shape[1], _stream())


def ngcf_layer_fwd(ego, S, W, keep, mask, mask_given, seed, step, layer, ego_out, out_block):
    call("nrhip_ngcf_layer_fwd", _ptr(ego, torch.float32), _ptr(S, torch.float32), _ptr(W[0]),
         _ptr(W[1]), _ptr(W[2]), _ptr(W[3]), ego.shape[0], ego.shape[1], float(keep),
         _ptr(mask, torch.uint8), 1 if mask_given else 0, C.c_uint64(seed & (2**64 - 1)),
         C.c_uint64(step), int(layer), _ptr(ego_out, torch.float32),
         C.c_void_p(out_block.data_ptr()), out_block.stride(0), _stream())


def ngcf_layer_bwd(ego, S, W, keep, mask, dout_block, dego_next, dS, dego_direct, dT1, dT2, dW, ws):
    call("nrhip_ngcf_layer_bwd", _ptr(ego, torch.float32), _ptr(S, torch.float32), _ptr(W[0]),
         _ptr(W[1]), _ptr(W[2]), _ptr(W[3]), ego.shape[0], ego.shape[1], float(keep),
         _ptr(mask, torch.uint8), C.c_void_p(dout_block.data_ptr()), dout_block.stride(0),
         _ptr(dego_next, allow_none=True), _ptr(dS), _ptr(dego_direct), _ptr(dT1), _ptr(dT2),
         _ptr(dW[0]), _ptr(dW[1]), _ptr(dW[2]), _ptr(dW[3]), _ptr(ws), ws.numel(), _stream())


def ngcf_workspace(n_rows, device):
    nbytes = C.c_size_t(0)
    call("nrhip_ngcf_workspace_bytes", int(n_rows), C.byref(nbytes))
    return torch.empty(nbytes.value, dtype=torch.uint8, device=device)


class NativeStep:

    def __init__(self, kind, handle, owner):
        self.kind, self.handle, self.owner = kind, handle, owner

    @staticmethod
    def for_lightgcn(eng):
        b = _lib.LightGCNBuffers()
        eng.A.ensure_schedule(eng.d)
        eng.At.ensure_schedule(eng.d)
        ws = eng.A._workspace(eng.d)
        wst = eng.At._workspace(eng.d)
        ws = ws if ws.numel() >= wst.numel() else wst
        vals = dict(plan=eng.A.plan.value, plan_t=eng.At.plan.value, indptr=eng.A.indptr,
                    indices=eng.A.indices, vals=eng.A.vals, indptr_t=eng.At.indptr,
                    indices_t=eng.At.indices, vals_t=eng.At.vals, E0=eng.E0, m=eng.m, v=eng.v,
                    Ea=eng.Ea, Eb=eng.Eb, Esum=eng.Esum, Esum_rows=eng.Esum_rows, Gstar=eng.Gstar,
                    Greg=eng.Greg, H=eng.H, Ga=eng.Ga, Gb=eng.Gb, batch_rows=eng.batch_rows,
                    row_flag=eng.row_flag, terms=eng.terms, spmm_ws=ws)
        for k, t in vals.items():
            setattr(b, k, t if isinstance(t, int) else t.data_ptr())
        b.spmm_ws_bytes, b.n_users, b.n_nodes = ws.numel(), eng.n_users, eng.N
        b.d, b.n_layers, b.max_batch, b.reg = eng.d, eng.n_layers, eng.max_batch, eng.reg
        h = C.c_void_p(0)
        call("nrhip_lightgcn_ctx_create", C.byref(b), C.byref(h))
        ctx = NativeStep("lightgcn", h, eng)
        ctx._keep = (ws,)
        return ctx

    @staticmethod
    def for_ngcf(eng):
        b = _lib.NGCFBuffers()
        eng.A.ensure_schedule(eng.d)
        eng.At.ensure_schedule(eng.d)
        ws = eng.A._workspace(eng.d)
        wst = eng.At._workspace(eng.d)
        ws = ws if ws.numel() >= wst.numel() else wst
        b.plan, b.plan_t = eng.A.plan.value, eng.At.plan.value
        for k, t in dict(indptr=eng.A.indptr, indices=eng.A.indices, vals=eng.A.vals, indptr_t=eng.At.indptr,
                         indices_t=eng.At.indices, vals_t=eng.At.vals, spmm_ws=ws, E0=eng.E0, mE=eng.mE,
                         vE=eng.vE, gE0=eng.gE0, Out=eng.Out, dOut=eng.dOut, dS=eng.dS, dEd=eng.dEd, dT1=eng.dT1,
                         dT2=eng.dT2, terms=eng.terms, rows=eng.rows, flag=eng.flag, ws=eng.ws).items():
            setattr(b, k, t.data_ptr())
        b.spmm_ws_bytes, b.ws_bytes = ws.numel(), eng.ws.numel()
        b.dEgo[0], b.dEgo[1] = eng.dEgo[0].data_ptr(), eng.dEgo[1].data_ptr()
        for k in range(eng.L + 1):
            b.ego[k] = eng.ego[k].data_ptr()
        for k in range(eng.L):
            b.S[k], b.mask[k] = eng.S[k].data_ptr(), eng.mask[k].data_ptr()
            for j in range(4):
                b.W[k][j], b.gW[k][j] = eng.W[k][j].data_ptr(), eng.gW[k][j].data_ptr()
                b.mW[k][j], b.vW[k][j] = eng.mW[k][j].data_ptr(), eng.vW[k][j].data_ptr()
        b.n_users, b.n_nodes, b.d, b.n_layers = eng.n_users, eng.N, eng.d, eng.L
        b.max_batch, b.reg, b.keep = eng.max_batch, eng.reg, eng.keep
        h = C.c_void_p(0)
        call("nrhip_ngcf_ctx_create", C.byref(b), C.byref(h))
        ctx = NativeStep("ngcf", h, eng)
        ctx._keep = (ws,)
        return ctx

    def ngcf_forward(self, seed, step_counter, mask_given):
        call("nrhip_ngcf_forward", self.handle, C.c_uint64(seed & (2**64 - 1)), C.c_uint64(step_counter),
             1 if mask_given else 0, _stream())

    def ngcf_step(self, users, pos, neg, st, seed, step_counter, mask_given, loss2, plan=None):
        call("nrhip_ngcf_step", self.handle, self._idx(users), self._idx(pos), self._idx(neg), users.numel(),
             self._plan(plan, 3 * users.numel()), C.c_uint64(seed & (2**64 - 1)), C.c_uint64(step_counter),
             1 if mask_given else 0, float(st.alpha()), float(st.beta1), float(st.beta2), float(st.eps),
             _ptr(loss2, torch.float32), _stream())

    @staticmethod
    def for_mf(eng):
        b = _lib.MFBuffers()
        for k in ("_P", "_Q", "terms"):
            setattr(b, k.lstrip("_"), getattr(eng, k).data_ptr())
        for k in ("mP", "vP", "mQ", "vQ"):
            setattr(b, k, eng._views[k].data_ptr())
        if not getattr(eng, "fused", False):
            b.GP, b.GQ = eng.GP.data_ptr(), eng.GQ.data_ptr()
        b.n_users, b.n_items, b.d = eng._P.shape[0], eng._Q.shape[0], eng._P.shape[1]
        b.max_batch, b.reg = eng.max_batch, eng.reg
        if eng.lazy:
            b.alpha_tab = eng._alpha_tab.data_ptr()
            b.alpha_len, b.lazy_period = eng._alpha_tab.numel(), eng.lazy_period
            if eng.fused:
                b.tw, b.inb = eng._tw.data_ptr(), eng._inb.data_ptr()
            else:
                b.last, b.stamp = eng._last.data_ptr(), eng._stamp.data_ptr()
        h = C.c_void_p(0)
        call("nrhip_mf_ctx_create", C.byref(b), C.byref(h))
        return NativeStep("mf", h, eng)

    def __del__(self):
        try:
            if self.handle and self.handle.value:
                name = {"lightgcn": "nrhip_lightgcn_ctx_destroy", "ngcf": "nrhip_ngcf_ctx_destroy"}.get(
                    self.kind, "nrhip_mf_ctx_destroy")
                getattr(_lib.lib, name)(self.handle)
                self.handle = C.c_void_p(0)
        except Exception:
            pass

    @staticmethod
    def _idx(t):
        if t.dtype != torch.int32 or not t.is_cuda or not t.is_contiguous():
            raise TypeError("batch ids must be contiguous int32 device tensors")
        return C.c_void_p(t.data_ptr())

    @staticmethod
    def _plan(plan, n_occ):
        if plan is None:
            return C.c_void_p(0)
        if plan.dtype != torch.int64 or not plan.is_cuda or plan.numel() != n_occ:
            raise TypeError("batch plan must be the int64 device tensor of %d keys bpr_plan made" % n_occ)
        return C.c_void_p(plan.data_ptr())

    def lightgcn_step(self, users, pos, neg, st, loss2=None, plan=None):
        call("nrhip_lightgcn_step", self.handle, self._idx(users), self._idx(pos), self._idx(neg),
             users.numel(), self._plan(plan, 3 * users.numel()), float(st.alpha()), float(st.beta1),
             float(st.beta2), float(st.eps), _ptr(loss2, allow_none=True), _stream())

    def lightgcn_step_colshard_fwd(self, users, pos, neg, partials):
        call("nrhip_lightgcn_step_colshard_fwd", self.handle, self._idx(users), self._idx(pos), self._idx(neg),
             users.numel(), _ptr(partials, torch.float32), _stream())

    def lightgcn_step_colshard_bwd(self, users, pos, neg, st, loss2, plan, given):
        call("nrhip_lightgcn_step_colshard_bwd", self.handle, self._idx(users), self._idx(pos), self._idx(neg),
             users.numel(), self._plan(plan, 3 * users.numel()), _ptr(given, torch.float32), float(st.alpha()),
             float(st.beta1), float(st.beta2), float(st.eps), _ptr(loss2, torch.float32, allow_none=True), _stream())

    def lightgcn_step_grad(self, users, pos, neg, loss2, grad_out, plan=None):
        call("nrhip_lightgcn_step_grad", self.handle, self._idx(users), self._idx(pos),
             self._idx(neg), users.numel(), self._plan(plan, 3 * users.numel()),
             _ptr(loss2, allow_none=True), _ptr(grad_out, torch.float32), _stream())

    def lightgcn_step_apply(self, grad, st):
        call("nrhip_lightgcn_step_apply", self.handle, _ptr(grad, torch.float32),
             float(st.alpha()), float(st.beta1), float(st.beta2), float(st.eps), _stream())

    def mf_step(self, users, pos, neg, st, loss2, plan=None, next_plan=None):
        n_next = 0 if next_plan is None else next_plan.numel() // 3
        call("nrhip_mf_step", self.handle, self._idx(users), self._idx(pos), self._idx(neg),
             users.numel(), self._plan(plan, 3 * users.numel()), self._plan(next_plan, 3 * n_next), n_next,
             st.t + 1, float(st.alpha()), float(st.beta1), float(st.beta2), float(st.eps),
             _ptr(loss2, torch.float32), _stream())

    def mf_steps(self, users, pos, neg, batch, st, h_alpha, loss_steps, plans=None, terms_steps=None):
        n = users.numel()
        n_steps = (n + batch - 1) // batch
        if h_alpha.dtype != np.float32 or h_alpha.size < n_steps or not h_alpha.flags["C_CONTIGUOUS"]:
            raise TypeError("h_alpha: contiguous float32 host array of %d step sizes" % n_steps)
        if loss_steps.numel() < 2 * n_steps:
            raise ValueError("loss buffer holds %d floats, 2 per step = %d needed" % (loss_steps.numel(), 2 * n_steps))
        call("nrhip_mf_steps", self.handle, self._idx(users), self._idx(pos), self._idx(neg), n, int(batch),
             self._plan(plans, 3 * n), st.t + 1, h_alpha.ctypes.data_as(C.c_void_p), float(st.beta1),
             float(st.beta2), float(st.eps), _ptr(loss_steps, torch.float32),
             _ptr(terms_steps, torch.float32, allow_none=True), _stream())

    def mf_flush(self, st):
        call("nrhip_mf_flush", self.handle, st.t, float(st.beta1), float(st.beta2), float(st.eps),
             _stream())


def device_info():
    cu, clk, mem = C.c_int(0), C.c_int(0), C.c_size_t(0)
    name = C.create_string_buffer(128)
    call("nrhip_device_info", C.byref(cu), C.byref(clk), C.byref(mem), name, 128)
    return {"cu_count": cu.value, "clock_khz": clk.value, "hbm_bytes": mem.value,
            "name": name.value.decode()}


VAE_ACTS = {"tanh": 0, "sigmoid": 1, "relu": 2, "identity": 3}


def vae_encode(csr, rows, Wq0, bq0, Wq1, bq1, Wp0, bp0, act, keep, is_training, seed, step, bufs,
               drop_given=None, eps_given=None, h0val=None):
    h, z = Wq0.shape[1], Wp0.shape[0]
    call("nrhip_vae_encode", _ptr(csr.indptr), _ptr(csr.indices), _ptr(rows, torch.int32),
         rows.numel(), h, z, _ptr(Wq0, torch.float32), _ptr(bq0), _ptr(Wq1), _ptr(bq1), _ptr(Wp0),
         _ptr(bp0), VAE_ACTS[act], float(keep), _ptr(drop_given, torch.float32, allow_none=True),
         _ptr(eps_given, torch.float32, allow_none=True), float(is_training),
         C.c_uint64(seed & (2**64 - 1)), C.c_uint64(step), _ptr(h0val, torch.float32, allow_none=True),
         *[_ptr(b, torch.float32) for b in bufs], _stream())


def vae_step_native(eng, rows, anneal, keep, drop_given, eps_given, want_loss, apply):
    from ._lib import VaeStepArgs
    a = eng._step_args
    bufs = ("H1", "MU", "LOGVAR", "EPSSTD", "ZS", "G1", "KLb", "h0val", "nll", "dG1", "DA3", "DH2", "DA1", "stats",
            "regsum", "ws")
    key = tuple(t.data_ptr() for d in (eng.P, eng.G, eng.M, eng.V) for t in d.values()) + \
        tuple(getattr(eng, f).data_ptr() for f in bufs) + (eng.csr.indptr.data_ptr(), eng.csr.indices.data_ptr())
    if a is None or eng._step_key != key:
        eng._step_key = key
        a = VaeStepArgs()
        names = eng.NAMES
        for t in list(eng.P.values()) + list(eng.G.values()) + list(eng.M.values()) + list(eng.V.values()):
            _ptr(t, torch.float32)
        a.indptr, a.indices = eng.csr.indptr.data_ptr(), eng.csr.indices.data_ptr()
        a.n_items, a.h, a.z, a.act = eng.n_items, eng.h, eng.z, VAE_ACTS[eng.act]
        for k, n in enumerate(names):
            a.P[k], a.G[k], a.M[k], a.V[k] = (d[n].data_ptr() for d in (eng.P, eng.G, eng.M, eng.V))
            a.sizes[k] = eng.P[n].numel()
        for f in bufs:
            setattr(a, f, getattr(eng, f).data_ptr())
# ... 72 lines not shown
```

neurec_amd/trainer.py:

```python
import os
import numpy as np
import torch

from . import engine as E


class TripletBatch(tuple):
    plan = None
    next_plan = None

    def __new__(cls, users, pos, neg, plan=None, next_plan=None):
        self = super().__new__(cls, (users, pos, neg))
        self.plan, self.next_plan = plan, next_plan
        return self


class BprEpochSampler:

    def __init__(self, train_csr, n_items, neg_num=1, batch_size=1024, shuffle=True,
                 drop_last=False, seed=2018, rank=0, world=1, plan_users=None):
        if neg_num <= 0:
            raise ValueError("'neg_num' must be a positive integer.")
        if train_csr.nnz == 0:
            raise ValueError("'user_pos_dict' cannot be empty.")
        deg_max = int(np.diff(train_csr.h_indptr).max())
        if n_items <= deg_max:
            raise ValueError("The number of 'exclusion' is greater than 'high'.")
        self.csr, self.n_items, self.neg_num = train_csr, int(n_items), int(neg_num)
        self.batch_size, self.shuffle, self.drop_last = int(batch_size), bool(shuffle), drop_last
        self.seed, self.epoch = int(seed), 0
        self.row_of = train_csr.row_of()
        n = train_csr.nnz
        self.lo = (n * rank) // world
        self.hi = (n * (rank + 1)) // world
        self.n_local = self.hi - self.lo
        dev = train_csr.indptr.device
        self._users = torch.empty(max(self.n_local, 1), dtype=torch.int32, device=dev)
        self._pos = torch.empty(max(self.n_local, 1), dtype=torch.int32, device=dev)
        self._neg = torch.empty(max(self.n_local * self.neg_num, 1), dtype=torch.int32, device=dev)
        self.plan_users = None if plan_users is None else int(plan_users)
        self.plans = self.plan_users is not None and self.neg_num == 1
        self._plan = (torch.empty(max(3 * self.n_local, 1), dtype=torch.int64, device=dev)
                      if self.plans else None)

    def __len__(self):
        if self.drop_last:
            return self.n_local // self.batch_size
        return (self.n_local + self.batch_size - 1) // self.batch_size

    def sample_epoch(self):
        out = E.sample_bpr_epoch(self.csr, self.row_of, self.n_items, self.neg_num, self.seed,
                                 self.epoch, self.shuffle, self.lo, self.n_local,
                                 out=(self._users, self._pos, self._neg))
        self.epoch += 1
        if self.plans and self.n_local > 0:
            E.bpr_plan(out[0], out[1], out[2], self.batch_size, self.plan_users, out=self._plan)
        return out

    def epoch_stream(self):
        users, pos, neg = self.sample_epoch()
        n = self.n_local
        return (users[:n], pos[:n], neg[:n * self.neg_num],
                self._plan[:3 * n] if self.plans else None)

    def batches(self):
        users, pos, neg = self.sample_epoch()
        B = self.batch_size
        for k in range(len(self)):
            b, e = k * B, min((k + 1) * B, self.n_local)
            nb = neg[b * self.neg_num:e * self.neg_num]
            e2 = min((k + 2) * B, self.n_local)
            yield TripletBatch(users[b:e], pos[b:e],
                               nb if self.neg_num == 1 else nb.view(-1, self.neg_num),
                               self._plan[3 * b:3 * e] if self.plans else None,
                               self._plan[3 * e:3 * e2] if (self.plans and e2 > e) else None)


class MFEngine:

    ALPHA_STEPS = 1 << 20

    def __init__(self, user_table, item_table, lr, reg, max_batch, lazy=True, lazy_period=None, fused=None):
        dev = E.require_gpu()
        ut = torch.as_tensor(user_table, dtype=torch.float32)
        it = torch.as_tensor(item_table, dtype=torch.float32)
        nu, rows = ut.shape[0], ut.shape[0] + it.shape[0]
        self.lazy = bool(lazy)
        self.fused = self.lazy and (True if fused is None else bool(fused))
        self.lazy_period = int(lazy_period) if lazy_period is not None else (8 if self.fused else 16)
        if self.fused:
            self._w2 = torch.empty((2, rows, ut.shape[1]), dtype=torch.float32, device=dev)
            self._w2[0].copy_(torch.cat([ut, it]))
            self._w2[1].zero_()
            self._m2, self._v2 = torch.zeros_like(self._w2), torch.zeros_like(self._w2)
            self._table, self._m, self._v, self._g = self._w2[0], self._m2[0], self._v2[0], None
            self._tw = torch.tensor([0, -1], dtype=torch.int32, device=dev).repeat(rows, 1).contiguous()
            self._inb = torch.zeros(rows, dtype=torch.int32, device=dev)
            self.GP = self.GQ = None
        else:
            self._table = torch.cat([ut, it]).contiguous().to(dev)
            self._m, self._v, self._g = (torch.zeros_like(self._table) for _ in range(3))
            self.GP, self.GQ = self._g[:nu], self._g[nu:]
        self._P, self._Q = self._table[:nu], self._table[nu:]
        self._views = {"mP": self._m[:nu], "mQ": self._m[nu:], "vP": self._v[:nu], "vQ": self._v[nu:]}
        self.reg = float(reg)
        self.adam = E.AdamState(lr)
        self.terms = torch.empty(8 * max_batch, dtype=torch.float32, device=dev)
        self.max_batch = max_batch
        self._stale = False
        self._terms_steps = None
        self._alpha_host = None
        if self.lazy:
            self._alpha_np = self.adam.alpha_table(self.ALPHA_STEPS)
            self._alpha_tail_const = bool(self._alpha_np.size > 256 and
                                          np.all(self._alpha_np[-256:] == self._alpha_np[-1]))
            self._alpha_tab = torch.from_numpy(self._alpha_np).to(dev)
            if not self.fused:
                self._last = torch.zeros(rows, dtype=torch.int32, device=dev)
                self._stamp = torch.zeros(rows, dtype=torch.int32, device=dev)
        self._ctx = E.NativeStep.for_mf(self)

    def _check_step_sizes(self, upto):
        if self.lazy and upto >= self._alpha_tab.numel() and not self._alpha_tail_const:
            raise NotImplementedError("step %d is beyond the step-size table (%d entries) and the table's tail "
                                      "is not constant yet: enlarge MFEngine.ALPHA_STEPS" % (upto, self.ALPHA_STEPS))

    def flush(self):
        if self.lazy and self._stale:
            self._ctx.mf_flush(self.adam)
            self._stale = False

    P = property(lambda self: (self.flush(), self._P)[1])
    Q = property(lambda self: (self.flush(), self._Q)[1])
    mP = property(lambda self: (self.flush(), self._views["mP"])[1])
    mQ = property(lambda self: (self.flush(), self._views["mQ"])[1])
    vP = property(lambda self: (self.flush(), self._views["vP"])[1])
    vQ = property(lambda self: (self.flush(), self._views["vQ"])[1])

    def step(self, users, pos, neg, loss_out, plan=None, next_plan=None):
        self._check_step_sizes(self.adam.t + 2)
        self._ctx.mf_step(users, pos, neg, self.adam, loss_out, plan, next_plan if self.lazy else None)
        self.adam.advance()
        self._stale = True

    def run_batches(self, users, pos, neg, batch, loss_steps, plans=None):
        n = users.numel()
        n_steps = (n + batch - 1) // batch
        self._check_step_sizes(self.adam.t + n_steps + 1)
        if batch > self.max_batch:
            raise ValueError("batch larger than max_batch")
        if n_steps == 0:
            return 0
        t = self.adam.t
        if self.lazy:
            idx = np.minimum(np.arange(t + 1, t + 1 + n_steps), self._alpha_np.size - 1)
            h_alpha = np.ascontiguousarray(self._alpha_np[idx])
        else:
# ... 46 lines not shown
        self.GP, self.GQ = torch.zeros_like(self.P), torch.zeros_like(self.Q)
        self.reg, self.lr, self.momentum = float(reg), float(lr), float(momentum)
        self.adam = E.AdamState(lr)
        self.terms = torch.empty(8 * max_batch, dtype=torch.float32, device=dev)
        self.max_batch = max_batch
        self.flagP = torch.zeros(self.P.shape[0], dtype=torch.uint8, device=dev)
        self.flagQ = torch.zeros(self.Q.shape[0], dtype=torch.uint8, device=dev)
        init = {"adam": 0.0, "gd": None, "adagrad": 1e-8, "rmsprop": 1.0, "momentum": 0.0}[learner]
        mk = lambda t, v: None if v is None else torch.full_like(t, v)
        self.s0P, self.s0Q = mk(self.P, init), mk(self.Q, init)
        two = learner in ("adam", "rmsprop")
        self.s1P, self.s1Q = (mk(self.P, 0.0), mk(self.Q, 0.0)) if two else (None, None)

    def _apply(self, var, s0, s1, grad, flag):
        if self.learner == "adam":
            E.adam_sparse(var, s0, s1, grad, self.adam)
        elif self.learner == "rmsprop":
            E.optimizer_rows("rmsprop", var, s0, s1, grad, flag, self.lr, 0.9, 0.0, 1e-10)
        elif self.learner == "momentum":
            E.optimizer_rows("momentum", var, s0, None, grad, flag, self.lr, self.momentum)
        else:
            E.optimizer_rows(self.learner, var, s0, None, grad, flag, self.lr)

    def step(self, users, items, third, loss_out):
        if users.numel() > self.max_batch:
            raise ValueError("batch larger than max_batch")
        if self.pairwise:
            E.pairwise_mf_grad(self.P, self.Q, users, items, third, self.reg, self.loss, self.GP,
                               self.GQ, self.terms, loss_out)
        else:
            E.pointwise_mf_grad(self.P, self.Q, users, items, third, self.reg, self.loss, self.GP,
                                self.GQ, self.terms, loss_out)
        if self.learner != "adam":
            E.mark_rows(users, self.flagP)
            E.mark_rows(items, self.flagQ)
            if self.pairwise:
                E.mark_rows(third, self.flagQ)
        self._apply(self.P, self.s0P, self.s1P, self.GP, self.flagP)
        self._apply(self.Q, self.s0Q, self.s1Q, self.GQ, self.flagQ)
        self.adam.advance()


class LightGCNEngine:

    def __init__(self, adj_csr, n_users, n_items, embed, n_layers, lr, reg, max_batch,
                 adj_t_csr=None, keep_order=False):
        dev = E.require_gpu()
        self.n_users, self.n_items, self.n_layers = int(n_users), int(n_items), int(n_layers)
        self.N = self.n_users + self.n_items
        if adj_t_csr is None and not isinstance(adj_csr, E.SpmmCSR):
            from .graph import is_symmetric, transpose_csr
            if not is_symmetric(adj_csr):
                adj_t_csr = transpose_csr(adj_csr)
        self.A = adj_csr if isinstance(adj_csr, E.SpmmCSR) else \
            E.SpmmCSR.from_scipy(adj_csr, split_row=n_users, keep_order=keep_order)
        if adj_t_csr is None:
            self.At = self.A
        else:
            self.At = adj_t_csr if isinstance(adj_t_csr, E.SpmmCSR) else E.SpmmCSR.from_scipy(adj_t_csr, split_row=n_users)
        emb = torch.as_tensor(embed, dtype=torch.float32)
        assert emb.shape[0] == self.N
        self.d_real = int(emb.shape[1])
        fits = [w for w in (16, 32, 64, 128, 256) if w >= self.d_real]
        if not fits:
            raise NotImplementedError("LightGCN embed_size %d > 256 is not built" % self.d_real)
        self.d = fits[0]
        self.E0 = torch.zeros((self.N, self.d), dtype=torch.float32, device=dev)
        self.E0[:, :self.d_real] = emb.to(dev)
        z = lambda: torch.zeros_like(self.E0)
        self.m, self.v = z(), z()
        self.Ea, self.Eb = z(), z()
        self.Esum = z()
        self.Gstar, self.Greg = z(), z()
        self.H, self.Ga, self.Gb = z(), z(), z()
        self.reg = float(reg)
        self.adam = E.AdamState(lr)
        self.terms = torch.empty(8 * max_batch, dtype=torch.float32, device=dev)
        self.max_batch = max_batch
        self.Esum_rows = z()
        self.batch_rows = torch.zeros(3 * max_batch, dtype=torch.int32, device=dev)
        self.row_flag = torch.zeros(self.N, dtype=torch.uint8, device=dev)
        self.Gsync = None
        self._ctx = E.NativeStep.for_lightgcn(self)

    def propagate(self):
        if self.n_layers == 0:
            self.Esum.copy_(self.E0)
            return self.Esum
        src, acc_in = self.E0, self.E0
        bufs = (self.Ea, self.Eb)
        for k in range(self.n_layers):
            out = None if k == self.n_layers - 1 else bufs[k % 2]
            self.A.matmul(src, out=out, sum_in=acc_in, sum_out=self.Esum)
            src, acc_in = out, self.Esum
        return self.Esum

    def final_embeddings(self):
        self.propagate()
        Estar = torch.empty_like(self.Esum)
        E.div_scalar(self.Esum, float(self.n_layers + 1), Estar)
        if self.d_real != self.d:
            Estar = Estar[:, :self.d_real].contiguous()
        return Estar[:self.n_users], Estar[self.n_users:]

    def step(self, users, pos, neg, loss_out=None, grad_sync=None, plan=None):
        if grad_sync is None:
            self._ctx.lightgcn_step(users, pos, neg, self.adam, loss_out, plan)
        else:
            if self.Gsync is None:
                self.Gsync = torch.zeros_like(self.E0)
            self._ctx.lightgcn_step_grad(users, pos, neg, loss_out, self.Gsync, plan)
            grad_sync(self.Gsync)
            self._ctx.lightgcn_step_apply(self.Gsync, self.adam)
        self.adam.advance()

    def step_reference(self, users, pos, neg, loss_out=None, grad_sync=None, plan=None):
        B = users.numel()
        if B > self.max_batch:
            raise ValueError("batch larger than max_batch")
        L = self.n_layers
        rows = self.batch_rows[:3 * B]
        E.lightgcn_mark_batch(users, pos, neg, self.n_users, rows, self.row_flag)
        if L == 0:
            esum = self.E0
        else:
            src, acc_in = self.E0, self.E0
            bufs = (self.Ea, self.Eb)
            for k in range(L - 1):
                self.A.matmul(src, out=bufs[k % 2], sum_in=acc_in, sum_out=self.Esum)
                src, acc_in = bufs[k % 2], self.Esum
            if self.d >= 64:
                self.A.matmul(src, sum_in=acc_in, sum_out=self.Esum_rows, y_row_wanted=self.row_flag)
            else:
                self.A.matmul(src, sum_in=acc_in, sum_out=self.Esum_rows)
            esum = self.Esum_rows
        E.lightgcn_bpr_grad(esum, self.E0, self.n_users, L, users, pos, neg, self.reg,
                            self.Gstar, self.Greg, self.terms, loss_out, plan)
        E.rows_div(rows, self.Gstar, float(L + 1), self.H)
        g = self.H
        bufs = (self.Ga, self.Gb)
        for k in range(L):
            self.At.matmul(g, out=bufs[k % 2], addend=self.H,
                           x_row_nonzero=self.row_flag if (k == 0 and self.d >= 64) else None)
            g = bufs[k % 2]
        if grad_sync is not None and self.Gsync is None:
            self.Gsync = torch.zeros_like(self.E0)
        if grad_sync is None:
            E.adam_dense2(self.E0, self.m, self.v, g, self.Greg, self.adam)
        else:
            E.add(g, self.Greg, self.Gsync)
            grad_sync(self.Gsync)
            E.adam_dense(self.E0, self.m, self.v, self.Gsync, self.adam, clear_grad=False)
        E.rows_clear(rows, self.d, (self.Gstar, self.Greg, self.H), self.row_flag)
        self.adam.advance()

    def step_bytes(self):
        L, nd4 = self.n_layers, self.N * self.d * 4
        full, masked = self.A.algorithmic_bytes(self.d), self.A.masked_bytes(self.d)
        if L == 0:
            return 7 * nd4
        head = self.max_batch * (11 * self.d * 4 + 12)
        fwd = (L - 1) * full + masked
        bwd = masked + max(L - 2, 0) * full if L >= 2 else 0
        last = self.A.nnz * 8 + (self.N + 1) * 4 + nd4 + 6 * nd4
        return fwd + head + bwd + last

    def step_bytes_survey(self):
        nd4 = self.N * self.d * 4
        return 2 * self.n_layers * self.A.algorithmic_bytes(self.d) + 7 * nd4 + 6 * self.max_batch * self.d * 4


class FullRankEvaluator:

    def __init__(self, train_csr, test_csr, metric_ids, top_k, batch_rows=2048, overlap=True,
                 pruned=True, search=None, extra_tiles=2):
        self.search = str(search or os.environ.get("NEUREC_EVAL_SEARCH", "int8"))
        if self.search not in ("bf16", "int8", "fp32"):
            raise ValueError("search must be 'bf16', 'int8' or 'fp32', got %r" % (self.search,))
        self.extra_tiles = int(extra_tiles)
        self.int8_retry = 8
        self._int8_pause = 0
        self.int8_extra_tiles = 4
        self.native_loop = True
        self.pruned = bool(pruned)
        self.train, self.test = train_csr, test_csr
        self.metric_ids = [int(m) for m in metric_ids]
        self.top_k = int(top_k)
        self.batch_rows = int(batch_rows)
        self.overlap = bool(overlap)
        self._side = None
# ... 458 lines not shown
```

Measured before the change: 5.255 million triplets/s.

## Precompute per-epoch hop schedules for batch-wanted SpMM rows

Builds, once per epoch, a device-side schedule of the wanted rows and their sublists for every batch, derived from the epoch's batch plans. The LightGCN step then runs a planned hop kernel that reads this schedule instead of discovering and ordering wanted rows inside each step. The aim is to take per-step row marking and scheduling work off the critical path. In exchange it adds an epoch-level planning kernel, extra device memory, and a batch-index consistency check that ties steps to the epoch stream.

```diff
diff --git a/include/neurec_hip.h b/include/neurec_hip.h
--- a/include/neurec_hip.h
+++ b/include/neurec_hip.h
@@ -249,6 +249,28 @@
                                     uint8_t* d_row_flag, int32_t* d_rows_out, void* stream);
 int nrhip_spmm_plan_has_wanted(const void* plan, int d);
 int nrhip_spmm_blocked_has_wanted(const void* blocked_plan);
+int nrhip_spmm_plan_has_wanted_planned(const void* plan, int d);
+int nrhip_spmm_blocked_has_wanted_planned(const void* blocked_plan);
+int nrhip_spmm_wanted_epoch_plan_bytes(const void* plan, int d, int batch, int64_t n_batches, size_t* bytes,
+                                       int* stride);
+int nrhip_spmm_blocked_wanted_epoch_plan_bytes(const void* blocked_plan, int batch, int64_t n_batches, size_t* bytes,
+                                               int* stride);
+int nrhip_spmm_wanted_epoch_plan(const void* plan, int d, const int64_t* d_indptr, const uint64_t* d_plans, int batch,
+                                 int64_t n_batches, int last_len, void* d_sched, size_t sched_bytes, void* stream);
+int nrhip_spmm_blocked_wanted_epoch_plan(const void* blocked_plan, const int64_t* d_indptr, const uint64_t* d_plans,
+                                         int batch, int64_t n_batches, int last_len, void* d_sched, size_t sched_bytes,
+                                         void* stream);
+int nrhip_spmm_csr_wanted_planned(const void* plan, const int32_t* d_indices, const float* d_vals, const float* d_X,
+                                  int d, const float* d_sum_in, const float* d_layer_a, const float* d_layer_b,
+                                  float* d_sum_out, const int32_t* d_users, const int32_t* d_pos, const int32_t* d_neg,
+                                  int batch, int n_users, uint8_t* d_row_flag, int32_t* d_rows_out,
+                                  const void* d_batch_sched, int stride, void* stream);
+int nrhip_spmm_blocked_wanted_planned(const void* blocked_plan, const int32_t* d_indices, const float* d_vals,
+                                      const float* d_X, const float* d_sum_in, const float* d_layer_a,
+                                      const float* d_layer_b, float* d_sum_out, const int32_t* d_users,
+                                      const int32_t* d_pos, const int32_t* d_neg, int batch, int n_users,
+                                      uint8_t* d_row_flag, int32_t* d_rows_out, const void* d_batch_sched, int stride,
+                                      void* stream);
 
 int nrhip_spmm_csr_carry(const void* plan, const int64_t* d_indptr, const int32_t* d_indices, const float* d_vals,
                          const float* d_X, const float* d_X2, int x_split, int d, float* d_Yv, int has_carry,
@@ -301,9 +323,15 @@
 int nrhip_lightgcn_step(void* ctx, const int32_t* d_users, const int32_t* d_pos,
                         const int32_t* d_neg, int batch, const uint64_t* d_plan, float alpha,
                         float beta1, float beta2, float eps, float* d_loss2, void* stream);
+int nrhip_lightgcn_step_planned(void* ctx, const int32_t* d_users, const int32_t* d_pos, const int32_t* d_neg,
+                                int batch, const uint64_t* d_plan, const void* d_hop_sched, int hop_stride,
+                                float alpha, float beta1, float beta2, float eps, float* d_loss2, void* stream);
 
 int nrhip_lightgcn_step_colshard_fwd(void* ctx, const int32_t* d_users, const int32_t* d_pos, const int32_t* d_neg,
                                      int batch, float* d_partials, void* stream);
+int nrhip_lightgcn_step_colshard_fwd_planned(void* ctx, const int32_t* d_users, const int32_t* d_pos,
+                                             const int32_t* d_neg, int batch, const void* d_hop_sched, int hop_stride,
+                                             float* d_partials, void* stream);
 int nrhip_lightgcn_step_colshard_bwd(void* ctx, const int32_t* d_users, const int32_t* d_pos, const int32_t* d_neg,
                                      int batch, const uint64_t* d_plan, const float* d_given, float alpha,
                                      float beta1, float beta2, float eps, float* d_loss2, void* stream);
diff --git a/neurec_amd/_lib.py b/neurec_amd/_lib.py
--- a/neurec_amd/_lib.py
+++ b/neurec_amd/_lib.py
@@ -196,6 +196,8 @@
     "nrhip_mf_steps": [p, p, p, p, i64, i32, p, i32, p, f32, f32, f32, p, p, p],
     "nrhip_loss_reduce_steps": [p, i32, i32, i32, f32, p, p],
     "nrhip_lightgcn_step_colshard_fwd": [p, p, p, p, i32, p, p],
+    "nrhip_lightgcn_step_colshard_fwd_planned": [p, p, p, p, i32, p, i32, p, p],
+    "nrhip_lightgcn_step_planned": [p, p, p, p, i32, p, p, i32, f32, f32, f32, f32, p, p],
     "nrhip_lightgcn_step_colshard_bwd": [p, p, p, p, i32, p, p, f32, f32, f32, f32, p, p],
     "nrhip_lightgcn_partial_dots": [p, p, i32, i32, i32, p, p, p, i32, p, p],
     "nrhip_partials_sum": [p, i32, i32, p, p],
@@ -248,6 +250,14 @@
     "nrhip_spmm_plan_has_blocked": [p, i32],
     "nrhip_spmm_plan_has_wanted": [p, i32],
     "nrhip_spmm_blocked_has_wanted": [p],
+    "nrhip_spmm_plan_has_wanted_planned": [p, i32],
+    "nrhip_spmm_blocked_has_wanted_planned": [p],
+    "nrhip_spmm_wanted_epoch_plan_bytes": [p, i32, i32, i64, psz, C.POINTER(i32)],
+    "nrhip_spmm_blocked_wanted_epoch_plan_bytes": [p, i32, i64, psz, C.POINTER(i32)],
+    "nrhip_spmm_wanted_epoch_plan": [p, i32, p, p, i32, i64, i32, p, sz, p],
+    "nrhip_spmm_blocked_wanted_epoch_plan": [p, p, p, i32, i64, i32, p, sz, p],
+    "nrhip_spmm_csr_wanted_planned": [p, p, p, p, i32, p, p, p, p, p, p, p, i32, i32, p, p, p, i32, p],
+    "nrhip_spmm_blocked_wanted_planned": [p, p, p, p, p, p, p, p, p, p, p, i32, i32, p, p, p, i32, p],
     "nrhip_spmm_csr_wanted_layers": [p, p, p, p, i32, p, p, p, p, p, p],
     "nrhip_spmm_blocked_wanted_layers": [p, p, p, p, p, p, p, p, p, p],
     "nrhip_spmm_csr_wanted_batch": [p, p, p, p, i32, p, p, p, p, p, p, p, i32, i32, p, p, p],
diff --git a/neurec_amd/build.py b/neurec_amd/build.py
--- a/neurec_amd/build.py
+++ b/neurec_amd/build.py
@@ -17,7 +17,7 @@
 FILE_FLAGS = {"score_i8.hip": ["-mllvm", "-amdgpu-mfma-vgpr-form"]}
 EXP_SOURCES = ["experiments/gather_experiments.hip"]
 EXP_LIB_PATH = os.path.join(HERE, "libneurec_exp.so")
-HEADERS = ["nr_core.h", "nr_common.h", "spmm_blocked_plan.h"]
+HEADERS = ["nr_core.h", "nr_common.h", "spmm_blocked_plan.h", "spmm_wanted_plan.h"]
 
 HIPCC = os.environ.get("HIPCC", "/opt/rocm/bin/hipcc")
 FLAGS = ["-O3", "--offload-arch=gfx950", "-std=c++17", "-fPIC", "-ffp-contract=off",
diff --git a/neurec_amd/colshard.py b/neurec_amd/colshard.py
--- a/neurec_amd/colshard.py
+++ b/neurec_amd/colshard.py
@@ -34,7 +34,8 @@
         if B > self.max_batch:
             raise ValueError("batch larger than max_batch")
         ctx, n = self.local._ctx, 3 * B
-        ctx.lightgcn_step_colshard_fwd(users, pos, neg, self._parts)
+        hop = self.local._hop.for_batch(plan, B) if self.local._hop is not None else None
+        ctx.lightgcn_step_colshard_fwd(users, pos, neg, self._parts, hop=hop)
         if self.comm.live and self.world == self.comm.world:
             allp = torch.empty((self.world, n), dtype=torch.float32, device=self._parts.device)
             self.comm.all_gather_rows(self._parts[:n], allp)
diff --git a/neurec_amd/csrc/spmm.hip b/neurec_amd/csrc/spmm.hip
--- a/neurec_amd/csrc/spmm.hip
+++ b/neurec_amd/csrc/spmm.hip
@@ -24,6 +24,18 @@
                                                const int32_t* d_neg, int batch, int n_users,
                                                uint8_t* d_row_flag, int32_t* d_rows_out, void* stream);
 extern "C" int nrhip_spmm_blocked_has_wanted(const void* plan);
+extern "C" int nrhip_spmm_blocked_has_wanted_planned(const void* plan);
+extern "C" int nrhip_spmm_blocked_wanted_epoch_plan_bytes(const void* plan, int batch, int64_t n_batches, size_t* bytes,
+                                                          int* stride);
+extern "C" int nrhip_spmm_blocked_wanted_epoch_plan(const void* plan, const int64_t* d_indptr, const uint64_t* d_plans,
+                                                    int batch, int64_t n_batches, int last_len, void* d_sched,
+                                                    size_t sched_bytes, void* stream);
+extern "C" int nrhip_spmm_blocked_wanted_planned(const void* plan, const int32_t* d_indices, const float* d_vals,
+                                                 const float* d_X, const float* d_sum_in, const float* d_layer_a,
+                                                 const float* d_layer_b, float* d_sum_out, const int32_t* d_users,
+                                                 const int32_t* d_pos, const int32_t* d_neg, int batch, int n_users,
+                                                 uint8_t* d_row_flag, int32_t* d_rows_out, const void* d_batch_sched,
+                                                 int stride, void* stream);
 extern "C" int nrhip_spmm_blocked_adam(const void* plan, const int32_t* d_indices,
                                        const float* d_vals, const float* d_X, float* d_addend,
                                        float* d_grad_b, float* d_var, float* d_m, float* d_v,
@@ -848,6 +860,40 @@
                                          n_users, d_row_flag, d_rows_out, stream);
 }
 
+int nrhip_spmm_plan_has_wanted_planned(const void* plan, int d) {
+  if (!plan || d != 64) return 0;
+  const SpmmPlan* p = (const SpmmPlan*)plan;
+  return p->blocked[blocked_slot(64)] ? nrhip_spmm_blocked_has_wanted_planned(p->blocked[blocked_slot(64)]) : 0;
+}
+
+int nrhip_spmm_wanted_epoch_plan_bytes(const void* plan, int d, int batch, int64_t n_batches, size_t* bytes,
+                                       int* stride) {
+  NR_REQUIRE(nrhip_spmm_plan_has_wanted_planned(plan, d), NR_ERR_UNSUPPORTED,
+             "spmm_wanted_epoch_plan_bytes: no planned batch-rows hop for this matrix and width");
+  return nrhip_spmm_blocked_wanted_epoch_plan_bytes(((const SpmmPlan*)plan)->blocked[blocked_slot(64)], batch, n_batches,
+                                                    bytes, stride);
+}
+
+int nrhip_spmm_wanted_epoch_plan(const void* plan, int d, const int64_t* d_indptr, const uint64_t* d_plans, int batch,
+                                 int64_t n_batches, int last_len, void* d_sched, size_t sched_bytes, void* stream) {
+  NR_REQUIRE(nrhip_spmm_plan_has_wanted_planned(plan, d), NR_ERR_UNSUPPORTED,
+             "spmm_wanted_epoch_plan: no planned batch-rows hop for this matrix and width");
+  return nrhip_spmm_blocked_wanted_epoch_plan(((const SpmmPlan*)plan)->blocked[blocked_slot(64)], d_indptr, d_plans,
+                                              batch, n_batches, last_len, d_sched, sched_bytes, stream);
+}
+
+int nrhip_spmm_csr_wanted_planned(const void* plan, const int32_t* d_indices, const float* d_vals, const float* d_X,
+                                  int d, const float* d_sum_in, const float* d_layer_a, const float* d_layer_b,
+                                  float* d_sum_out, const int32_t* d_users, const int32_t* d_pos, const int32_t* d_neg,
+                                  int batch, int n_users, uint8_t* d_row_flag, int32_t* d_rows_out,
+                                  const void* d_batch_sched, int stride, void* stream) {
+  NR_REQUIRE(nrhip_spmm_plan_has_wanted_planned(plan, d), NR_ERR_UNSUPPORTED,
+             "spmm_csr_wanted_planned: no planned batch-rows hop for this matrix and width");
+  return nrhip_spmm_blocked_wanted_planned(((const SpmmPlan*)plan)->blocked[blocked_slot(64)], d_indices, d_vals, d_X,
+                                           d_sum_in, d_layer_a, d_layer_b, d_sum_out, d_users, d_pos, d_neg, batch,
+                                           n_users, d_row_flag, d_rows_out, d_batch_sched, stride, stream);
+}
+
 int nrhip_spmm_plan_has_wanted(const void* plan, int d) {
   if (!plan || d != 64) return 0;
   const SpmmPlan* p = (const SpmmPlan*)plan;
diff --git a/neurec_amd/csrc/spmm_blocked.hip b/neurec_amd/csrc/spmm_blocked.hip
--- a/neurec_amd/csrc/spmm_blocked.hip
+++ b/neurec_amd/csrc/spmm_blocked.hip
@@ -1,5 +1,6 @@
 #include "nr_common.h"
 #include "spmm_blocked_plan.h"
+#include "spmm_wanted_plan.h"
 #include <algorithm>
 #include <new>
 #include <cstdlib>
@@ -24,6 +25,8 @@
   int wanted_ok, w_ent_cap, w_nnz_cap, w_bitmap_words;
   int ww_ok, ww_ent_cap;
   int ww_lds_slots;
+  int wp_ok, n_hubs;
+  nr_wplan::SlotProfile wp_profile;
 };
 
 
@@ -627,6 +630,127 @@
 #define NR_WW_STAMP_END(i)
 #endif
 
+template <class Between>
+__device__ __forceinline__ float4 ww_sublist_sum(int col, float val, int len, const float4* __restrict__ X, int c,
+                                                 int g, Between between) {
+  constexpr int RS = 16;
+  const float4 zero = make_float4(0.f, 0.f, 0.f, 0.f);
+  float4 x[16];
+#pragma unroll
+  for (int j = 0; j < 16; ++j) {
+    const int cj = __shfl(col, (g << 4) | j, NR_WAVE);
+    x[j] = X[(int64_t)cj * RS + c];
+  }
+  between();
+#pragma unroll
+  for (int j = 0; j < 16; ++j) {
+    const float aj = __shfl(val, (g << 4) | j, NR_WAVE);
+    x[j] = make_float4(__fmul_rn(aj, x[j].x), __fmul_rn(aj, x[j].y), __fmul_rn(aj, x[j].z), __fmul_rn(aj, x[j].w));
+  }
+  float4 acc = zero, carry = zero;
+#pragma unroll
+  for (int gg = 0; gg < 4; ++gg) {
+    if (gg * 16 < len) {
+      if (g == gg) {
+        acc = carry;
+#pragma unroll
+        for (int j = 0; j < 16; ++j) {
+          const float4 t = make_float4(__fadd_rn(acc.x, x[j].x), __fadd_rn(acc.y, x[j].y),
+                                       __fadd_rn(acc.z, x[j].z), __fadd_rn(acc.w, x[j].w));
+          if (gg * 16 + j < len) acc = t;
+        }
+      }
+      const int src = (gg << 4) | c;
+      carry = make_float4(__shfl(acc.x, src, NR_WAVE), __shfl(acc.y, src, NR_WAVE),
+                          __shfl(acc.z, src, NR_WAVE), __shfl(acc.w, src, NR_WAVE));
+    }
+  }
+  return carry;
+}
+
+struct WwPre { float4 si, a, b; };
+__device__ __forceinline__ WwPre ww_prefetch(const WantedEpi& ep, int64_t oe) {
+  const float4 zero = make_float4(0.f, 0.f, 0.f, 0.f);
+  WwPre p{zero, zero, zero};
+  if (ep.sum_out) {
+    p.si = ep.sum_in[oe];
+    if (ep.chain.a) p.a = ep.chain.a[oe];
+    if (ep.chain.b) p.b = ep.chain.b[oe];
+  }
+  return p;
+}
+
+__device__ __forceinline__ void ww_sublist_out(float4 carry, int slot, int64_t o, int c, const WwPre& pre,
+                                               const WantedEpi& ep, float4* lds_dst, float* ww_part) {
+  if (slot == 0) {
+    float4 y = carry;
+    if (ep.addend) {
+      const float4 pre_add = ep.addend[o];
+      y = make_float4(__fadd_rn(y.x, pre_add.x), __fadd_rn(y.y, pre_add.y), __fadd_rn(y.z, pre_add.z),
+                      __fadd_rn(y.w, pre_add.w));
+    }
+    if (ep.Y) ep.Y[o] = y;
+    if (ep.sum_out) {
+      float4 si = pre.si;
+      if (ep.chain.a)
+        si = make_float4(__fadd_rn(si.x, pre.a.x), __fadd_rn(si.y, pre.a.y), __fadd_rn(si.z, pre.a.z),
+                         __fadd_rn(si.w, pre.a.w));
+      if (ep.chain.b)
+        si = make_float4(__fadd_rn(si.x, pre.b.x), __fadd_rn(si.y, pre.b.y), __fadd_rn(si.z, pre.b.z),
+                         __fadd_rn(si.w, pre.b.w));
+      ep.sum_out[o] = make_float4(__fadd_rn(si.x, y.x), __fadd_rn(si.y, y.y), __fadd_rn(si.z, y.z),
+                                  __fadd_rn(si.w, y.w));
+    }
+  } else if (slot < 0) {
+    lds_dst[c] = carry;
+  } else {
+    float* mine = ww_part + (size_t)(slot - 1) * 64 + c * 4;
+    __hip_atomic_store(mine + 0, carry.x, __ATOMIC_RELAXED, __HIP_MEMORY_SCOPE_AGENT);
+    __hip_atomic_store(mine + 1, carry.y, __ATOMIC_RELAXED, __HIP_MEMORY_SCOPE_AGENT);
+    __hip_atomic_store(mine + 2, carry.z, __ATOMIC_RELAXED, __HIP_MEMORY_SCOPE_AGENT);
+    __hip_atomic_store(mine + 3, carry.w, __ATOMIC_RELAXED, __HIP_MEMORY_SCOPE_AGENT);
+  }
+}
+
+__device__ __forceinline__ void ww_chunk_done(int hub, const int4 hd, unsigned* ww_cnt, const float* ww_part,
+                                              const WantedEpi& ep, int lane, int c, int g) {
+  constexpr int RS = 16;
+  unsigned old = 0;
+  if (lane == 0) old = __hip_atomic_fetch_add(&ww_cnt[hub], 1u, __ATOMIC_RELAXED, __HIP_MEMORY_SCOPE_AGENT);
+  old = __builtin_amdgcn_readfirstlane(old);
+  if (old != (unsigned)hd.w - 1u) return;
+  float4 sum = make_float4(0.f, 0.f, 0.f, 0.f);
+  for (int s0 = 0; s0 < hd.z; s0 += 16) {
+    float4 q[16];
+#pragma unroll
+    for (int j = 0; j < 16; ++j) {
+      const float* qp = ww_part + ((size_t)hd.y + min(s0 + j, hd.z - 1)) * 64 + c * 4;
+      q[j].x = __hip_atomic_load(qp + 0, __ATOMIC_RELAXED, __HIP_MEMORY_SCOPE_AGENT);
+      q[j].y = __hip_atomic_load(qp + 1, __ATOMIC_RELAXED, __HIP_MEMORY_SCOPE_AGENT);
+      q[j].z = __hip_atomic_load(qp + 2, __ATOMIC_RELAXED, __HIP_MEMORY_SCOPE_AGENT);
+      q[j].w = __hip_atomic_load(qp + 3, __ATOMIC_RELAXED, __HIP_MEMORY_SCOPE_AGENT);
+    }
+#pragma unroll
+    for (int j = 0; j < 16; ++j)
+      if (s0 + j < hd.z)
+        sum = make_float4(__fadd_rn(sum.x, q[j].x), __fadd_rn(sum.y, q[j].y), __fadd_rn(sum.z, q[j].z),
+                          __fadd_rn(sum.w, q[j].w));
+  }
+  if (g == 0)
+    masked_row_out(sum, (int64_t)hd.x * RS + c, ep.addend, true, ep.Y, ep.sum_in, ep.sum_out, &ep.chain);
+  if (lane == 0) __hip_atomic_store(&ww_cnt[hub], 0u, __ATOMIC_RELAXED, __HIP_MEMORY_SCOPE_AGENT);
+}
+
+__device__ __forceinline__ void ww_publish_batch(const BatchLists& bl, int wg, int n_wg, int tid) {
+  const int total = 3 * bl.batch, per = (total + n_wg - 1) / n_wg;
+  for (int i = wg * per + tid; i < min(total, (wg + 1) * per); i += 16 * NR_WAVE) {
+    const int which = i / bl.batch, b = i - which * bl.batch;
+    const int row = which == 0 ? bl.users[b] : bl.n_users + (which == 1 ? bl.pos[b] : bl.neg[b]);
+    bl.row_flag[row] = 1;
+    if (bl.rows_out) bl.rows_out[i] = row;
+  }
+}
+
 __global__ __launch_bounds__(16 * NR_WAVE) void spmm_wanted_wave_kernel(
     const int32_t* __restrict__ ww_off, const int32_t* __restrict__ ww_choff,
     const int4* __restrict__ ww_ent, const int32_t* __restrict__ ww_gch, const int4* __restrict__ ww_hub,
@@ -659,13 +783,7 @@
       if (p >= 0) atomicOr(&s_bits[rp >> 5], 1u << (rp & 31));
       if (q >= 0) atomicOr(&s_bits[rq >> 5], 1u << (rq & 31));
     }
-    const int total = 3 * bl.batch, per = (total + (int)gridDim.x - 1) / (int)gridDim.x;
-    for (int i = wg * per + tid; i < min(total, (wg + 1) * per); i += 16 * NR_WAVE) {
-      const int which = i / bl.batch, b = i - which * bl.batch;
-      const int row = which == 0 ? bl.users[b] : bl.n_users + (which == 1 ? bl.pos[b] : bl.neg[b]);
-      bl.row_flag[row] = 1;
-      if (bl.rows_out) bl.rows_out[i] = row;
-    }
+    ww_publish_batch(bl, wg, (int)gridDim.x, tid);
   }
   __syncthreads();
   auto is_wanted = [&](int row) -> bool {
@@ -693,84 +811,24 @@
   }
   while (k < n) {
     const int len = e.y, slot = e.x, row = e.w;
-    float4 x[16];
-#pragma unroll
-    for (int j = 0; j < 16; ++j) {
-      const int cj = __shfl(col, (g << 4) | j, NR_WAVE);
-      x[j] = X[(int64_t)cj * RS + c];
-    }
     const int64_t o = (int64_t)row * RS + c;
-    const int64_t oe = slot == 0 ? o : (int64_t)c;
-    float4 pre_si = zero, pre_a = zero, pre_b = zero;
-    if (ep.sum_out) {
-      pre_si = ep.sum_in[oe];
-      if (ep.chain.a) pre_a = ep.chain.a[oe];
-      if (ep.chain.b) pre_b = ep.chain.b[oe];
-    }
+    WwPre pre;
     const int kn = k + 16;
     int4 en = zero_int4();
     int coln = 0;
     float valn = 0.f;
-    if (kn < n) {
-      en = s_want[kn];
-      if (lane < en.y) {
-        coln = indices[(uint32_t)en.z + lane];
-        valn = vals[(uint32_t)en.z + lane];
-      }
-    }
-#pragma unroll
-    for (int j = 0; j < 16; ++j) {
-      const float aj = __shfl(val, (g << 4) | j, NR_WAVE);
-      x[j] = make_float4(__fmul_rn(aj, x[j].x), __fmul_rn(aj, x[j].y), __fmul_rn(aj, x[j].z), __fmul_rn(aj, x[j].w));
-    }
-    float4 acc = zero, carry = zero;
-#pragma unroll
-    for (int gg = 0; gg < 4; ++gg) {
-      if (gg * 16 < len) {
-        if (g == gg) {
-          acc = carry;
-#pragma unroll
-          for (int j = 0; j < 16; ++j) {
-            const float4 t = make_float4(__fadd_rn(acc.x, x[j].x), __fadd_rn(acc.y, x[j].y),
-                                         __fadd_rn(acc.z, x[j].z), __fadd_rn(acc.w, x[j].w));
-            if (gg * 16 + j < len) acc = t;
-          }
+    const float4 carry = ww_sublist_sum(col, val, len, X, c, g, [&]() {
+      pre = ww_prefetch(ep, slot == 0 ? o : (int64_t)c);
+      if (kn < n) {
+        en = s_want[kn];
+        if (lane < en.y) {
+          coln = indices[(uint32_t)en.z + lane];
+          valn = vals[(uint32_t)en.z + lane];
         }
-        const int src = (gg << 4) | c;
-        carry = make_float4(__shfl(acc.x, src, NR_WAVE), __shfl(acc.y, src, NR_WAVE),
-                            __shfl(acc.z, src, NR_WAVE), __shfl(acc.w, src, NR_WAVE));
-      }
-    }
-    if (g == 0) {
-      if (slot == 0) {
-        float4 y = carry;
-        if (ep.addend) {
-          const float4 pre_add = ep.addend[o];
-          y = make_float4(__fadd_rn(y.x, pre_add.x), __fadd_rn(y.y, pre_add.y), __fadd_rn(y.z, pre_add.z),
-                          __fadd_rn(y.w, pre_add.w));
-        }
-        if (ep.Y) ep.Y[o] = y;
-        if (ep.sum_out) {
-          float4 si = pre_si;
-          if (ep.chain.a)
-            si = make_float4(__fadd_rn(si.x, pre_a.x), __fadd_rn(si.y, pre_a.y), __fadd_rn(si.z, pre_a.z),
-                             __fadd_rn(si.w, pre_a.w));
-          if (ep.chain.b)
-            si = make_float4(__fadd_rn(si.x, pre_b.x), __fadd_rn(si.y, pre_b.y), __fadd_rn(si.z, pre_b.z),
-                             __fadd_rn(si.w, pre_b.w));
-          ep.sum_out[o] = make_float4(__fadd_rn(si.x, y.x), __fadd_rn(si.y, y.y), __fadd_rn(si.z, y.z),
-                                      __fadd_rn(si.w, y.w));
-        }
-      } else if (slot < 0) {
-        s_part[(size_t)(-slot - 1) * RS + c] = carry;
-      } else {
-        float* mine = ww_part + (size_t)(slot - 1) * 64 + c * 4;
-        __hip_atomic_store(mine + 0, carry.x, __ATOMIC_RELAXED, __HIP_MEMORY_SCOPE_AGENT);
-        __hip_atomic_store(mine + 1, carry.y, __ATOMIC_RELAXED, __HIP_MEMORY_SCOPE_AGENT);
-        __hip_atomic_store(mine + 2, carry.z, __ATOMIC_RELAXED, __HIP_MEMORY_SCOPE_AGENT);
-        __hip_atomic_store(mine + 3, carry.w, __ATOMIC_RELAXED, __HIP_MEMORY_SCOPE_AGENT);
-      }
-    }
+      }
+    });
+    if (g == 0)
+      ww_sublist_out(carry, slot, o, c, pre, ep, s_part + (size_t)(slot < 0 ? -slot - 1 : 0) * RS, ww_part);
     k = kn;
     e = en;
     col = coln;
@@ -805,33 +863,153 @@
       const int hub = ww_gch[hi];
       const int4 hd = ww_hub[hub];
       if (!is_wanted(hd.x)) continue;
-      unsigned old = 0;
-      if (lane == 0) old = __hip_atomic_fetch_add(&ww_cnt[hub], 1u, __ATOMIC_RELAXED, __HIP_MEMORY_SCOPE_AGENT);
-      old = __builtin_amdgcn_readfirstlane(old);
-      if (old != (unsigned)hd.w - 1u) continue;
-      float4 sum = zero;
-      for (int s0 = 0; s0 < hd.z; s0 += 16) {
-        float4 q[16];
-#pragma unroll
-        for (int j = 0; j < 16; ++j) {
-          const float* qp = ww_part + ((size_t)hd.y + min(s0 + j, hd.z - 1)) * 64 + c * 4;
-          q[j].x = __hip_atomic_load(qp + 0, __ATOMIC_RELAXED, __HIP_MEMORY_SCOPE_AGENT);
-          q[j].y = __hip_atomic_load(qp + 1, __ATOMIC_RELAXED, __HIP_MEMORY_SCOPE_AGENT);
-          q[j].z = __hip_atomic_load(qp + 2, __ATOMIC_RELAXED, __HIP_MEMORY_SCOPE_AGENT);
-          q[j].w = __hip_atomic_load(qp + 3, __ATOMIC_RELAXED, __HIP_MEMORY_SCOPE_AGENT);
+      ww_chunk_done(hub, hd, ww_cnt, ww_part, ep, lane, c, g);
+    }
+  }
+  NR_WW_STAMP_END(4);
+}
+
+constexpr int kWpThreads = 1024;
+
+__global__ __launch_bounds__(kWpThreads) void spmm_wanted_epoch_plan_kernel(
+    const uint64_t* __restrict__ plans, int batch, int n_batches, int last_len, const int64_t* __restrict__ indptr,
+    const int4* __restrict__ ww_hub, int n_hubs, int n2, int stride, int4* __restrict__ sched) {
+  extern __shared__ uint32_t s_wp[];
+  uint32_t* s_key = s_wp;
+  int* s_off = (int*)(s_wp + n2);
+  __shared__ int s_scan[kWpThreads];
+  __shared__ int s_nhub, s_nrows;
+  const int tid = threadIdx.x, b = blockIdx.x;
+  const int n = 3 * (b == n_batches - 1 ? last_len : batch);
+  const uint64_t* keys = plans + 3 * (size_t)b * batch;
+  int4* items = sched + (size_t)b * stride;
+  if (tid == 0) { s_nhub = 0; s_nrows = 0; }
+  for (int i = tid; i < n2; i += kWpThreads) {
+    uint32_t k = ~0u;
+    if (i < n) {
+      const int32_t row = (int32_t)(keys[i] >> 32);
+      const int32_t prev = i > 0 ? (int32_t)(keys[i - 1] >> 32) : -1;
+      if (row != prev) k = nr_wplan::sort_key(indptr[row + 1] - indptr[row], row);
+    }
+    s_key[i] = k;
+  }
+  __syncthreads();
+  for (int k = 2; k <= n2; k <<= 1)
+    for (int j = k >> 1; j > 0; j >>= 1) {
+      for (int i = tid; i < n2; i += kWpThreads) {
+        const int p = i ^ j;
+        if (p > i) {
+          const uint32_t x = s_key[i], y = s_key[p];
+          if ((x > y) == ((i & k) == 0)) { s_key[i] = y; s_key[p] = x; }
         }
-#pragma unroll
-        for (int j = 0; j < 16; ++j)
-          if (s0 + j < hd.z)
-            sum = make_float4(__fadd_rn(sum.x, q[j].x), __fadd_rn(sum.y, q[j].y), __fadd_rn(sum.z, q[j].z),
-                              __fadd_rn(sum.w, q[j].w));
-      }
-      if (g == 0)
-        masked_row_out(sum, (int64_t)hd.x * RS + c, ep.addend, true, ep.Y, ep.sum_in, ep.sum_out, &ep.chain);
-      if (lane == 0) __hip_atomic_store(&ww_cnt[hub], 0u, __ATOMIC_RELAXED, __HIP_MEMORY_SCOPE_AGENT);
-    }
-  }
-  NR_WW_STAMP_END(4);
+      }
+      __syncthreads();
+    }
+  const int per = n2 / kWpThreads;
+  int sum = 0, hubs = 0, rows = 0;
+  for (int j = tid * per; j < (tid + 1) * per; ++j) {
+    const uint32_t k = s_key[j];
+    s_off[j] = sum;
+    if (k != ~0u) {
+      const int32_t row = nr_wplan::key_row(k);
+      const int64_t len = indptr[row + 1] - indptr[row];
+      sum += nr_wplan::slots_of(len);
+      hubs += nr_wplan::is_hub(len) ? 1 : 0;
+      ++rows;
+    }
+  }
+  s_scan[tid] = sum;
+  if (hubs) atomicAdd(&s_nhub, hubs);
+  if (rows) atomicAdd(&s_nrows, rows);
+  __syncthreads();
+  for (int off = 1; off < kWpThreads; off <<= 1) {
+    const int v = tid >= off ? s_scan[tid - off] : 0;
+    __syncthreads();
+    s_scan[tid] += v;
+    __syncthreads();
+  }
+  const int before = s_scan[tid] - sum, total = s_scan[kWpThreads - 1];
+  for (int j = tid * per; j < (tid + 1) * per; ++j) s_off[j] += before;
+  __syncthreads();
+  const int cap = stride - 1;
+  const int n_hub_rows = s_nhub;
+  for (int j = 0; j < n_hub_rows; ++j) {
+    const int32_t row = nr_wplan::key_row(s_key[j]);
+    const int64_t first = indptr[row], len = indptr[row + 1] - first;
+    int lo = 0, hi = n_hubs - 1;
+    while (lo < hi) {
+      const int mid = (lo + hi) >> 1;
+      if (ww_hub[mid].x < row) lo = mid + 1; else hi = mid;
+    }
+    const int part0 = ww_hub[lo].y, sl = nr_wplan::slots_of(len), o = s_off[j];
+    for (int s = tid; s < sl; s += kWpThreads)
+      if (o + s < cap) {
+        const nr_plan::Int4 it = nr_wplan::item_of(row, first, len, s, lo, part0);
+        items[1 + o + s] = make_int4(it.x, it.y, it.z, it.w);
+      }
+  }
+  for (int j = n_hub_rows + tid; j < n2; j += kWpThreads) {
+    const uint32_t k = s_key[j];
+    if (k == ~0u) continue;
+    const int32_t row = nr_wplan::key_row(k);
+    const int64_t first = indptr[row], len = indptr[row + 1] - first;
+    const int sl = nr_wplan::slots_of(len), o = s_off[j];
+    for (int s = 0; s < sl; ++s)
+      if (o + s < cap) {
+        const nr_plan::Int4 it = nr_wplan::item_of(row, first, len, s, 0, 0);
+        items[1 + o + s] = make_int4(it.x, it.y, it.z, it.w);
+      }
+  }
+  for (int i = 1 + min(total, cap) + tid; i < stride; i += kWpThreads) items[i] = make_int4(0, 0, 0, -1);
+  if (tid == 0) items[0] = make_int4(min(total, cap), s_nrows, 0, 0);
+}
+
+__global__ __launch_bounds__(16 * NR_WAVE) void spmm_wanted_planned_kernel(
+    const int4* __restrict__ items, const int4* __restrict__ ww_hub, float* ww_part, unsigned* ww_cnt,
+    const int32_t* __restrict__ indices, const float* __restrict__ vals, const float4* __restrict__ X, WantedEpi ep,
+    BatchLists bl) {
+  constexpr int RS = 16;
+  __shared__ float4 s_part[16 * RS];
+  const int tid = threadIdx.x, lane = tid & 63, wave = tid >> 6;
+  const int c = lane & 15, g = lane >> 4;
+  const int wg = blockIdx.x;
+  const int n_items = items[0].x;
+  ww_publish_batch(bl, wg, (int)gridDim.x, tid);
+  if (wg * 16 >= n_items) return;
+  const int idx = wg * 16 + wave;
+  const int4 it = idx < n_items ? items[1 + idx] : make_int4(0, 0, 0, -1);
+  const int slot = it.x, len = it.y & 255, hub = (it.y >> 8) - 1, row = it.w;
+  const int64_t o = (int64_t)row * RS + c;
+  const bool head = slot < 0 && ((-slot - 1) & 15) == 0;
+  int4 hd = zero_int4();
+  WwPre pre;
+  if (row >= 0) {
+    int col = 0;
+    float val = 0.f;
+    if (lane < len) {
+      col = indices[(uint32_t)it.z + lane];
+      val = vals[(uint32_t)it.z + lane];
+    }
+    if (hub >= 0) hd = ww_hub[hub];
+    const float4 carry = ww_sublist_sum(col, val, len, X, c, g,
+                                        [&]() { pre = ww_prefetch(ep, (slot == 0 || head) ? o : (int64_t)c); });
+    if (g == 0) ww_sublist_out(carry, slot, o, c, pre, ep, s_part + wave * RS, ww_part);
+  }
+  __builtin_amdgcn_fence(__ATOMIC_RELEASE, "workgroup");
+  __builtin_amdgcn_s_waitcnt(0);
+  __syncthreads();
+  if (row < 0) return;
+  if (head && g == 0) {
+    const int ns = (-slot - 1) >> 4;
+    float4 acc = make_float4(0.f, 0.f, 0.f, 0.f);
+    for (int sgm = 0; sgm < ns; ++sgm) {
+      const float4 q = s_part[(wave + sgm) * RS + c];
+      acc.x = __fadd_rn(acc.x, q.x); acc.y = __fadd_rn(acc.y, q.y);
+      acc.z = __fadd_rn(acc.z, q.z); acc.w = __fadd_rn(acc.w, q.w);
+    }
+    ww_sublist_out(acc, 0, o, c, pre, ep, nullptr, nullptr);
+  }
+  if (hub >= 0) ww_chunk_done(hub, hd, ww_cnt, ww_part, ep, lane, c, g);
 }
 
 size_t wanted_lds_bytes(const BlockedPlan* p) {
@@ -960,6 +1138,10 @@
   p->nnz_cap = h.nnz_cap; p->ent_cap = h.ent_cap; p->colmask_ok = h.colmask_ok;
   p->wanted_ok = h.wanted_ok; p->w_ent_cap = h.w_ent_cap; p->w_nnz_cap = h.w_nnz_cap; p->w_bitmap_words = h.w_bitmap_words;
   p->ww_ok = h.ww_ok; p->ww_ent_cap = h.ww_ent_cap; p->ww_lds_slots = h.ww_lds_slots;
+  env = getenv("NEUREC_SPMM_WANTED_PLANNED");
+  p->n_hubs = (int)h.ww_hub.size();
+  p->wp_ok = h.ww_ok && opt.seg == nr_wplan::kSeg && n_rows <= nr_wplan::kMaxRows && !(env && env[0] == '0');
+  if (p->wp_ok) p->wp_profile = nr_wplan::slot_profile(h_indptr, n_rows);
   std::vector<nr_plan::Section> sections = nr_plan::plan_sections(*p, h);
   const size_t used = nr_plan::carve_sections(&sections, d_plan_buf);
   if (used > plan_bytes) {
@@ -1153,6 +1335,69 @@
   return NR_OK;
 }
 
+int nrhip_spmm_blocked_has_wanted_planned(const void* plan) {
+  return plan && ((const BlockedPlan*)plan)->wp_ok ? 1 : 0;
+}
+
+int nrhip_spmm_blocked_wanted_epoch_plan_bytes(const void* plan, int batch, int64_t n_batches, size_t* bytes,
+                                               int* stride) {
+  NR_REQUIRE(plan && bytes && stride && batch >= 1 && n_batches >= 0, NR_ERR_ARG,
+             "spmm_blocked_wanted_epoch_plan_bytes: bad arguments");
+  const BlockedPlan* p = (const BlockedPlan*)plan;
+  NR_REQUIRE(p->wp_ok, NR_ERR_UNSUPPORTED, "spmm_blocked_wanted_epoch_plan_bytes: no planned form for this plan");
+  NR_REQUIRE(3 * (int64_t)batch <= nr_wplan::kMaxKeys, NR_ERR_UNSUPPORTED,
+             "spmm_blocked_wanted_epoch_plan_bytes: batch %d > %d", batch, nr_wplan::kMaxKeys / 3);
+  const int64_t st = nr_wplan::stride_of(p->wp_profile, batch);
+  NR_REQUIRE(st < ((int64_t)1 << 24), NR_ERR_UNSUPPORTED, "spmm_blocked_wanted_epoch_plan_bytes: %lld items per batch",
+             (long long)st);
+  *stride = (int)st;
+  *bytes = (size_t)st * 16 * (size_t)n_batches;
+  return NR_OK;
+}
+
+int nrhip_spmm_blocked_wanted_epoch_plan(const void* plan, const int64_t* d_indptr, const uint64_t* d_plans, int batch,
+                                         int64_t n_batches, int last_len, void* d_sched, size_t sched_bytes,
+                                         void* stream) {
+  NR_REQUIRE(plan && d_indptr && d_plans && d_sched && batch >= 1 && n_batches >= 1 && last_len >= 1 &&
+                 last_len <= batch && n_batches < ((int64_t)1 << 30),
+             NR_ERR_ARG, "spmm_blocked_wanted_epoch_plan: bad arguments");
+  const BlockedPlan* p = (const BlockedPlan*)plan;
+  size_t need = 0;
+  int stride = 0;
+  NR_TRY(nrhip_spmm_blocked_wanted_epoch_plan_bytes(plan, batch, n_batches, &need, &stride));
+  NR_REQUIRE(sched_bytes >= need, NR_ERR_WORKSPACE, "spmm_blocked_wanted_epoch_plan: buffer %zu < %zu bytes",
+             sched_bytes, need);
+  int n2 = kWpThreads;
+  while (n2 < 3 * batch) n2 <<= 1;
+  hipLaunchKernelGGL(spmm_wanted_epoch_plan_kernel, dim3((unsigned)n_batches), dim3(kWpThreads), (size_t)n2 * 8,
+                     (hipStream_t)stream, d_plans, batch, (int)n_batches, last_len, d_indptr, p->ww_hub, p->n_hubs, n2,
+                     stride, (int4*)d_sched);
+  NR_LAUNCH_CHECK();
+  return NR_OK;
+}
+
+int nrhip_spmm_blocked_wanted_planned(const void* plan, const int32_t* d_indices, const float* d_vals,
+                                      const float* d_X, const float* d_sum_in, const float* d_layer_a,
+                                      const float* d_layer_b, float* d_sum_out, const int32_t* d_users,
+                                      const int32_t* d_pos, const int32_t* d_neg, int batch, int n_users,
+                                      uint8_t* d_row_flag, int32_t* d_rows_out, const void* d_batch_sched, int stride,
+                                      void* stream) {
+  NR_REQUIRE(plan && d_indices && d_vals && d_X && d_sum_in && d_sum_out && d_users && d_pos && d_neg &&
+                 d_row_flag && d_batch_sched && batch >= 1 && n_users >= 0 && stride > 1 && (stride - 1) % 16 == 0,
+             NR_ERR_ARG, "spmm_blocked_wanted_planned: bad arguments");
+  NR_REQUIRE(d_layer_a || !d_layer_b, NR_ERR_ARG, "spmm_blocked_wanted_planned: layer_b without layer_a");
+  const BlockedPlan* p = (const BlockedPlan*)plan;
+  NR_REQUIRE(p->wp_ok, NR_ERR_UNSUPPORTED, "spmm_blocked_wanted_planned: no planned form for this plan");
+  hipLaunchKernelGGL(spmm_wanted_planned_kernel, dim3((unsigned)((stride - 1) / 16)), dim3(16 * NR_WAVE), 0,
+                     (hipStream_t)stream, (const int4*)d_batch_sched, p->ww_hub, p->ww_part, p->ww_cnt, d_indices,
+                     d_vals, (const float4*)d_X,
+                     WantedEpi{nullptr, nullptr, (const float4*)d_sum_in, (float4*)d_sum_out,
+                               LayerChain{(const float4*)d_layer_a, (const float4*)d_layer_b}},
+                     BatchLists{d_users, d_pos, d_neg, batch, n_users, d_row_flag, d_rows_out});
+  NR_LAUNCH_CHECK();
+  return NR_OK;
+}
+
 int nrhip_spmm_blocked_has_wanted(const void* plan) {
   if (plan && ((const BlockedPlan*)plan)->ww_ok) return 2;
   if (!plan || !((const BlockedPlan*)plan)->wanted_ok) return 0;
diff --git a/neurec_amd/csrc/spmm_wanted_plan.h b/neurec_amd/csrc/spmm_wanted_plan.h
--- /dev/null
+++ b/neurec_amd/csrc/spmm_wanted_plan.h
@@ -0,0 +1,115 @@
+#pragma once
+#include <stdint.h>
+#include <algorithm>
+#include <vector>
+
+#include "spmm_blocked_plan.h"
+
+#ifdef __HIPCC__
+#define NR_WP_HD __host__ __device__ __forceinline__
+#else
+#define NR_WP_HD inline
+#endif
+
+namespace nr_wplan {
+
+constexpr int kSeg = 64;
+constexpr int kChunk = nr_plan::kWaveChunk;
+constexpr int kWaves = 16;
+constexpr int kMaxKeys = 16384;
+constexpr int64_t kMaxRows = (int64_t)1 << 19;
+
+NR_WP_HD int segments_of(int64_t len) { return len <= kSeg ? 1 : (int)((len + kSeg - 1) / kSeg); }
+NR_WP_HD bool is_hub(int64_t len) { return len > (int64_t)kSeg * kChunk; }
+NR_WP_HD int slots_of(int64_t len) {
+  const int ns = segments_of(len);
+  if (ns > kChunk) return (ns + kChunk - 1) / kChunk * kChunk;
+  return ns <= 1 ? 1 : ns <= 2 ? 2 : ns <= 4 ? 4 : 8;
+}
+NR_WP_HD uint32_t sort_key(int64_t len, int32_t row) {
+  const int sl = slots_of(len);
+  const uint32_t cls = sl >= 8 ? 0u : sl == 4 ? 1u : sl == 2 ? 2u : 3u;
+  const uint32_t c = (uint32_t)(len < 1023 ? len : 1023);
+  return (cls << 29) | ((1023u - c) << 19) | (uint32_t)row;
+}
+NR_WP_HD int32_t key_row(uint32_t key) { return (int32_t)(key & ((1u << 19) - 1u)); }
+NR_WP_HD int seg_len(int64_t len, int sg) {
+  const int64_t left = len - (int64_t)sg * kSeg;
+  return (int)(left < 0 ? 0 : left < kSeg ? left : kSeg);
+}
+
+NR_WP_HD nr_plan::Int4 item_pad() { return nr_plan::Int4{0, 0, 0, -1}; }
+NR_WP_HD nr_plan::Int4 item_short(int32_t row, int64_t first, int64_t len) {
+  return nr_plan::Int4{0, (int32_t)len, (int32_t)(uint32_t)first, row};
+}
+NR_WP_HD nr_plan::Int4 item_lds(int32_t row, int64_t first, int64_t len, int sg) {
+  return nr_plan::Int4{-(1 + sg + 16 * segments_of(len)), seg_len(len, sg),
+                       (int32_t)(uint32_t)(first + (int64_t)sg * kSeg), row};
+}
+NR_WP_HD nr_plan::Int4 item_hub(int32_t row, int64_t first, int64_t len, int sg, int hub_index, int part0) {
+  return nr_plan::Int4{1 + part0 + sg, seg_len(len, sg) | ((sg % kChunk == 0) ? (hub_index + 1) << 8 : 0),
+                       (int32_t)(uint32_t)(first + (int64_t)sg * kSeg), row};
+}
+NR_WP_HD nr_plan::Int4 item_of(int32_t row, int64_t first, int64_t len, int s, int hub_index, int part0) {
+  const int ns = segments_of(len);
+  if (s >= ns) return item_pad();
+  if (ns == 1) return item_short(row, first, len);
+  if (ns <= kChunk) return item_lds(row, first, len, s);
+  return item_hub(row, first, len, s, hub_index, part0);
+}
+
+
+struct SlotProfile { std::vector<int32_t> big_desc; int64_t n_rows = 0; };
+inline SlotProfile slot_profile(const int64_t* indptr, int64_t n_rows) {
+  SlotProfile p;
+  p.n_rows = n_rows;
+  for (int64_t r = 0; r < n_rows; ++r) {
+    const int s = slots_of(indptr[r + 1] - indptr[r]);
+    if (s > 1) p.big_desc.push_back(s);
+  }
+  std::sort(p.big_desc.begin(), p.big_desc.end(), [](int32_t a, int32_t b) { return a > b; });
+  return p;
+}
+inline int64_t items_bound(const SlotProfile& p, int batch) {
+  const int64_t k = std::min<int64_t>(3 * (int64_t)batch, p.n_rows);
+  const int64_t nb = std::min<int64_t>(k, (int64_t)p.big_desc.size());
+  int64_t sum = k - nb;
+  for (int64_t i = 0; i < nb; ++i) sum += p.big_desc[(size_t)i];
+  return sum;
+}
+inline int64_t stride_of(const SlotProfile& p, int batch) {
+  return 1 + (items_bound(p, batch) + kWaves - 1) / kWaves * kWaves;
+}
+
+inline int64_t plan_batch(const int64_t* indptr, const std::vector<nr_plan::Int4>& hubs, const uint64_t* keys,
+                          int n_keys, int64_t stride, nr_plan::Int4* out) {
+  std::vector<uint32_t> sk;
+  for (int i = 0; i < n_keys; ++i) {
+    const int32_t row = (int32_t)(keys[i] >> 32);
+    if (i > 0 && (int32_t)(keys[i - 1] >> 32) == row) continue;
+    sk.push_back(sort_key(indptr[row + 1] - indptr[row], row));
+  }
+  std::sort(sk.begin(), sk.end());
+  for (int64_t i = 0; i < stride; ++i) out[i] = nr_plan::Int4{0, 0, 0, 0};
+  int64_t n = 0;
+  for (uint32_t k : sk) {
+    const int32_t row = key_row(k);
+    const int64_t first = indptr[row], len = indptr[row + 1] - first;
+    const int sl = slots_of(len);
+    int hub = -1, part0 = 0;
+    if (is_hub(len)) {
+      auto it = std::lower_bound(hubs.begin(), hubs.end(), row, [](const nr_plan::Int4& h, int32_t r) { return h.x < r; });
+      if (it == hubs.end() || it->x != row) return -1;
+      hub = (int)(it - hubs.begin());
+      part0 = it->y;
+    }
+    if (n + sl > stride - 1) return -1;
+    for (int s = 0; s < sl; ++s) out[1 + n + s] = item_of(row, first, len, s, hub, part0);
+    n += sl;
+  }
+  for (int64_t i = 1 + n; i < stride; ++i) out[i] = item_pad();
+  out[0] = nr_plan::Int4{(int32_t)n, (int32_t)sk.size(), 0, 0};
+  return n;
+}
+
+}
diff --git a/neurec_amd/csrc/step.hip b/neurec_amd/csrc/step.hip
--- a/neurec_amd/csrc/step.hip
+++ b/neurec_amd/csrc/step.hip
@@ -44,6 +44,13 @@
                                            const int32_t* d_users, const int32_t* d_pos,
                                            const int32_t* d_neg, int batch, int n_users,
                                            uint8_t* d_row_flag, int32_t* d_rows_out, void* stream);
+extern "C" int nrhip_spmm_plan_has_wanted_planned(const void* plan, int d);
+extern "C" int nrhip_spmm_csr_wanted_planned(const void* plan, const int32_t* d_indices, const float* d_vals,
+                                             const float* d_X, int d, const float* d_sum_in, const float* d_layer_a,
+                                             const float* d_layer_b, float* d_sum_out, const int32_t* d_users,
+                                             const int32_t* d_pos, const int32_t* d_neg, int batch, int n_users,
+                                             uint8_t* d_row_flag, int32_t* d_rows_out, const void* d_batch_sched,
+                                             int stride, void* stream);
 extern "C" int nrhip_spmm_csr_wanted_layers(const void* plan, const int32_t* d_indices,
                                             const float* d_vals, const float* d_X, int d,
                                             const float* d_sum_in, const float* d_layer_a,
@@ -82,7 +89,7 @@
                             const uint64_t* d_plan, float* d_loss2, void* stream,
                             const float** g_out, const AdamArgs* adam = nullptr,
                             bool* rearmed = nullptr, int phase = 0, float* d_partials = nullptr,
-                            const float* d_given = nullptr) {
+                            const float* d_given = nullptr, const void* d_hop_sched = nullptr, int hop_stride = 0) {
   const int L = b.n_layers, d = b.d;
   const bool skip = d >= 64;
   const int wanted_form = (skip && L > 0) ? nrhip_spmm_plan_has_wanted(b.plan, d) : 0;
@@ -109,7 +116,11 @@
     }
     if (chain) {
       if (L - 1 == 1) { layer[0] = layer[1]; layer[1] = nullptr; }
-      if (wanted_form == 2)
+      if (wanted_form == 2 && d_hop_sched)
+        NR_TRY(nrhip_spmm_csr_wanted_planned(b.plan, b.indices, b.vals, src, d, acc_in, layer[0], layer[1],
+                                             b.Esum_rows, d_users, d_pos, d_neg, batch, b.n_users, b.row_flag,
+                                             b.batch_rows, d_hop_sched, hop_stride, stream));
+      else if (wanted_form == 2)
         NR_TRY(nrhip_spmm_csr_wanted_batch(b.plan, b.indices, b.vals, src, d, acc_in, layer[0], layer[1],
                                            b.Esum_rows, d_users, d_pos, d_neg, batch, b.n_users,
                                            b.row_flag, b.batch_rows, stream));
@@ -199,6 +210,28 @@
   return NR_OK;
 }
 
+int nrhip_lightgcn_step_planned(void* ctx, const int32_t* d_users, const int32_t* d_pos, const int32_t* d_neg,
+                                int batch, const uint64_t* d_plan, const void* d_hop_sched, int hop_stride,
+                                float alpha, float beta1, float beta2, float eps, float* d_loss2, void* stream) {
+  NR_TRY(lightgcn_check(ctx, d_users, d_pos, d_neg, batch));
+  if (batch == 0) return NR_OK;
+  const nrhip_lightgcn_buffers& b = ((LightGCNCtx*)ctx)->b;
+  NR_REQUIRE(d_hop_sched && b.n_layers > 0 && nrhip_spmm_plan_has_wanted_planned(b.plan, b.d) &&
+                 nrhip_spmm_plan_has_wanted(b.plan, b.d) == 2,
+             NR_ERR_UNSUPPORTED, "lightgcn_step_planned: no planned batch-rows hop for this context");
+  const float* g = nullptr;
+  const AdamArgs adam{alpha, beta1, beta2, eps};
+  bool rearmed = false;
+  NR_TRY(lightgcn_fwd_bwd(b, d_users, d_pos, d_neg, batch, d_plan, d_loss2, stream, &g, &adam, &rearmed, 0, nullptr,
+                          nullptr, d_hop_sched, hop_stride));
+  if (g)
+    NR_TRY(nrhip_adam_dense_tf2(b.E0, b.m, b.v, g, b.Greg, (int64_t)b.n_nodes * b.d, alpha, beta1, beta2, eps,
+                                stream));
+  if (rearmed) return NR_OK;
+  NR_TRY(nrhip_rows_clear(b.batch_rows, 3 * batch, b.d, b.Gstar, b.Greg, b.H, nullptr, b.row_flag, stream));
+  return NR_OK;
+}
+
 int nrhip_lightgcn_step_colshard_fwd(void* ctx, const int32_t* d_users, const int32_t* d_pos, const int32_t* d_neg,
                                      int batch, float* d_partials, void* stream) {
   NR_TRY(lightgcn_check(ctx, d_users, d_pos, d_neg, batch));
@@ -207,6 +240,21 @@
   const float* g = nullptr;
   return lightgcn_fwd_bwd(((LightGCNCtx*)ctx)->b, d_users, d_pos, d_neg, batch, nullptr, nullptr, stream, &g,
                           nullptr, nullptr, 1, d_partials, nullptr);
+}
+
+int nrhip_lightgcn_step_colshard_fwd_planned(void* ctx, const int32_t* d_users, const int32_t* d_pos,
+                                             const int32_t* d_neg, int batch, const void* d_hop_sched, int hop_stride,
+                                             float* d_partials, void* stream) {
+  NR_TRY(lightgcn_check(ctx, d_users, d_pos, d_neg, batch));
+  NR_REQUIRE(d_partials, NR_ERR_ARG, "lightgcn_step_colshard_fwd_planned: null output");
+  if (batch == 0) return NR_OK;
+  const nrhip_lightgcn_buffers& b = ((LightGCNCtx*)ctx)->b;
+  NR_REQUIRE(d_hop_sched && b.n_layers > 0 && nrhip_spmm_plan_has_wanted_planned(b.plan, b.d) &&
+                 nrhip_spmm_plan_has_wanted(b.plan, b.d) == 2,
+             NR_ERR_UNSUPPORTED, "lightgcn_step_colshard_fwd_planned: no planned batch-rows hop for this context");
+  const float* g = nullptr;
+  return lightgcn_fwd_bwd(b, d_users, d_pos, d_neg, batch, nullptr, nullptr, stream, &g, nullptr, nullptr, 1,
+                          d_partials, nullptr, d_hop_sched, hop_stride);
 }
 
 int nrhip_lightgcn_step_colshard_bwd(void* ctx, const int32_t* d_users, const int32_t* d_pos, const int32_t* d_neg,
diff --git a/neurec_amd/engine.py b/neurec_amd/engine.py
--- a/neurec_amd/engine.py
+++ b/neurec_amd/engine.py
@@ -963,6 +963,44 @@
     return torch.empty(nbytes.value, dtype=torch.uint8, device=device)
 
 
+class EpochHopSchedule:
+
+    def __init__(self, A, d):
+        self.A, self.d = A, int(d)
+        self.ok = bool(_lib.lib.nrhip_spmm_plan_has_wanted_planned(A.plan, self.d)) and \
+            _lib.lib.nrhip_spmm_plan_has_wanted(A.plan, self.d) == 2
+        self.key, self.buf, self.stride, self.batch, self.n_batches, self.last_len = None, None, 0, 0, 0, 0
+
+    def for_batch(self, plan, n_triplets):
+        stream = getattr(plan, "epoch_plans", None) if plan is not None else None
+        if not self.ok or stream is None:
+            return None
+        plans, batch, epoch = stream
+        if 3 * batch > 16384:
+            return None
+        key = (plans.data_ptr(), plans.numel(), int(batch), int(epoch))
+        if key != self.key:
+            self._build(plans, int(batch))
+            self.key = key
+        k = int(plan.batch_index)
+        if not (0 <= k < self.n_batches) or n_triplets != (self.last_len if k == self.n_batches - 1 else self.batch):
+            raise ValueError("batch %d of %d triplets is not a batch of its epoch stream" % (k, n_triplets))
+        return self.buf.data_ptr() + k * self.stride * 16, self.stride
+
+    def _build(self, plans, batch):
+        n = plans.numel() // 3
+        n_batches = (n + batch - 1) // batch
+        nbytes, stride = C.c_size_t(0), C.c_int(0)
+        call("nrhip_spmm_wanted_epoch_plan_bytes", self.A.plan, self.d, batch, n_batches, C.byref(nbytes),
+             C.byref(stride))
+        if self.buf is None or self.buf.numel() < nbytes.value:
+            self.buf = torch.empty(nbytes.value, dtype=torch.uint8, device=plans.device)
+        self.stride, self.batch, self.n_batches = stride.value, batch, n_batches
+        self.last_len = n - (n_batches - 1) * batch
+        call("nrhip_spmm_wanted_epoch_plan", self.A.plan, self.d, _ptr(self.A.indptr), _ptr(plans, torch.int64), batch,
+             n_batches, self.last_len, _ptr(self.buf), self.buf.numel(), _stream())
+
+
 class NativeStep:
 
     def __init__(self, kind, handle, owner):
@@ -1079,12 +1117,21 @@
             raise TypeError("batch plan must be the int64 device tensor of %d keys bpr_plan made" % n_occ)
         return C.c_void_p(plan.data_ptr())
 
-    def lightgcn_step(self, users, pos, neg, st, loss2=None, plan=None):
+    def lightgcn_step(self, users, pos, neg, st, loss2=None, plan=None, hop=None):
+        if hop is not None:
+            call("nrhip_lightgcn_step_planned", self.handle, self._idx(users), self._idx(pos), self._idx(neg),
+                 users.numel(), self._plan(plan, 3 * users.numel()), C.c_void_p(hop[0]), hop[1], float(st.alpha()),
+                 float(st.beta1), float(st.beta2), float(st.eps), _ptr(loss2, allow_none=True), _stream())
+            return
         call("nrhip_lightgcn_step", self.handle, self._idx(users), self._idx(pos), self._idx(neg),
              users.numel(), self._plan(plan, 3 * users.numel()), float(st.alpha()), float(st.beta1),
              float(st.beta2), float(st.eps), _ptr(loss2, allow_none=True), _stream())
 
-    def lightgcn_step_colshard_fwd(self, users, pos, neg, partials):
+    def lightgcn_step_colshard_fwd(self, users, pos, neg, partials, hop=None):
+        if hop is not None:
+            call("nrhip_lightgcn_step_colshard_fwd_planned", self.handle, self._idx(users), self._idx(pos),
+                 self._idx(neg), users.numel(), C.c_void_p(hop[0]), hop[1], _ptr(partials, torch.float32), _stream())
+            return
         call("nrhip_lightgcn_step_colshard_fwd", self.handle, self._idx(users), self._idx(pos), self._idx(neg),
              users.numel(), _ptr(partials, torch.float32), _stream())
 
diff --git a/neurec_amd/trainer.py b/neurec_amd/trainer.py
--- a/neurec_amd/trainer.py
+++ b/neurec_amd/trainer.py
@@ -66,13 +66,17 @@
     def batches(self):
         users, pos, neg = self.sample_epoch()
         B = self.batch_size
+        epoch_plans = (self._plan[:3 * self.n_local], B, self.epoch) if self.plans else None
         for k in range(len(self)):
             b, e = k * B, min((k + 1) * B, self.n_local)
             nb = neg[b * self.neg_num:e * self.neg_num]
             e2 = min((k + 2) * B, self.n_local)
+            plan = None
+            if self.plans:
+                plan = self._plan[3 * b:3 * e]
+                plan.epoch_plans, plan.batch_index = epoch_plans, k
             yield TripletBatch(users[b:e], pos[b:e],
-                               nb if self.neg_num == 1 else nb.view(-1, self.neg_num),
-                               self._plan[3 * b:3 * e] if self.plans else None,
+                               nb if self.neg_num == 1 else nb.view(-1, self.neg_num), plan,
                                self._plan[3 * e:3 * e2] if (self.plans and e2 > e) else None)
 
 
@@ -285,6 +289,7 @@
         self.row_flag = torch.zeros(self.N, dtype=torch.uint8, device=dev)
         self.Gsync = None
         self._ctx = E.NativeStep.for_lightgcn(self)
+        self._hop = E.EpochHopSchedule(self.A, self.d) if self.n_layers > 0 else None
 
     def propagate(self):
         if self.n_layers == 0:
@@ -308,7 +313,8 @@
 
     def step(self, users, pos, neg, loss_out=None, grad_sync=None, plan=None):
         if grad_sync is None:
-            self._ctx.lightgcn_step(users, pos, neg, self.adam, loss_out, plan)
+            hop = self._hop.for_batch(plan, users.numel()) if self._hop is not None else None
+            self._ctx.lightgcn_step(users, pos, neg, self.adam, loss_out, plan, hop=hop)
         else:
             if self.Gsync is None:
                 self.Gsync = torch.zeros_like(self.E0)
```

Measured after the change: 5.412 million triplets/s (median of 6 runs). 1.03x the previous value.
